# lppllppl920/SAGE-SLAM

Hardware: AMD Instinct MI355X
Metric: M residuals/sec (+ LM iters/sec), 64-keyframe feature-metric BA @128x160 (higher is better)
Workload: dtype f32; 1 GPU; 64-keyframe window, 128x160x16 feature pyramids (L=4), 32-dim depth code, dense sampling N=16128, 186 links = 372 photometric + 372 geometric directed edges; parallelism=single GPU, collective=none, accepted_steps=988

## Files before the change

### include/sage_ba.h

```cpp
#ifndef SAGE_BA_H_
#define SAGE_BA_H_

#include <stddef.h>
#include <stdint.h>

#ifdef __cplusplus
extern "C" {
#endif

#define SAGE_MAX_LEVELS 8
#define SAGE_POSE_FLOATS 12

#define SAGE_OK 0
#define SAGE_E_INVALID (-1)
#define SAGE_E_UNSUPPORTED (-2)
#define SAGE_E_NOT_PSD (-3)
#define SAGE_E_STATE (-4)
#define SAGE_E_NO_OVERLAP (-5)

typedef struct SageCamera
{
  float fx, fy, cx, cy, w, h;
} SageCamera;

// ... 9 lines not shown

const char *sage_version(void);
const char *sage_error_string(int code);

typedef struct SageWorkspace SageWorkspace;
int sage_workspace_create(void *hip_stream, SageWorkspace **out);
void sage_workspace_destroy(SageWorkspace *ws);


int sage_photometric_jac_error_calculate(
    SageWorkspace *ws, float *AtA_dev, float *Atb_dev, float *error_host, float *num_inliers_host,
    const float *R10_dev, const float *t10_dev, const float *R0_dev, const float *t0_dev,
    const float *R1_dev, const float *t1_dev,
    const float *bias0_dev, const float *basis0_dev, const float *code0_dev, const float *mask1_dev,
    const int64_t *loc1d_dev, const float *homo_dev,
    const float *feat0_dev, const float *feat1_dev, const float *grad1_dev,
    float scale0, const SagePyramid *pyr, float eps, const float *weights_host,
    int N, int FS, int CS);

int sage_photometric_error_calculate(
    SageWorkspace *ws, float *error_host, float *num_inliers_host,
    const float *R10_dev, const float *t10_dev,
    const float *bias0_dev, const float *basis0_dev, const float *code0_dev, const float *mask1_dev,
    const int64_t *loc1d_dev, const float *homo_dev,
    const float *feat0_dev, const float *feat1_dev,
    float scale0, const SagePyramid *pyr, float eps, const float *weights_host,
    int N, int FS, int CS);

int sage_tracker_photo_jac_error_calculate(
    SageWorkspace *ws, int dof, float *AtA_dev, float *Atb_dev, float *error_host, float *num_inliers_host,
    const float *R_dev, const float *t_dev, const float *mask1_dev,
    const float *dpts0_dev, const float *homo_dev, const float *feat0s_dev,
    const float *feat1_dev, const float *grad1_dev,
    const SagePyramid *pyr, float scale0, float eps, const float *weights_dev, int N, int FS);

int sage_tracker_photo_error_calculate(
    SageWorkspace *ws, float *error_host, float *num_inliers_host,
    const float *R_dev, const float *t_dev, const float *mask1_dev,
    const float *dpts0_dev, const float *homo_dev, const float *feat0s_dev, const float *feat1_dev,
    const SagePyramid *pyr, float eps, const float *weights_dev, int N, int FS);

int sage_geometric_jac_error_calculate(
    SageWorkspace *ws, float *AtA_dev, float *Atb_dev, float *error_host, float *num_inliers_host,
    const float *R10_dev, const float *t10_dev, const float *R0_dev, const float *t0_dev,
    const float *R1_dev, const float *t1_dev,
    const float *bias0_dev, const float *basis0_dev, const float *code0_dev,
    const float *dpt1_dev, const float *dpt_grad1_dev, const float *basis1_dev, const float *mask1_dev,
    const int32_t *loc1d_dev, const float *homo_dev,
    float scale0, float scale1, const SageCamera *cam, float eps, float loss_param, float weight,
    int N, int CS);

int sage_geometric_error_calculate(
    SageWorkspace *ws, float *error_host, float *num_inliers_host,
    const float *R10_dev, const float *t10_dev,
    const float *bias0_dev, const float *basis0_dev, const float *code0_dev,
    const float *dpt1_dev, const float *mask1_dev, const int32_t *loc1d_dev, const float *homo_dev,
    float scale0, const SageCamera *cam, float eps, float loss_param, float weight, int N, int CS);

int sage_depth_and_grad(SageWorkspace *ws, float *dpt_dev, float *dpt_grad_dev,
                        const float *bias_dev, const float *basis_dev, const float *code_dev,
                        float scale, int H, int W, int CS);
int sage_gaussian_pyramid_with_grad(SageWorkspace *ws, float *pyr_dev, float *grad_dev,
                                    const float *feat_dev, const float *mask_dev,
                                    const SagePyramid *pyr, int FS);

int sage_bind_thread_to_device(int device);
int sage_solver_helper_cpus(int *cpus, int n);
int sage_solver_placement_moves(void);
int sage_placement_monitor(int enable);
void sage_shutdown(void);
int sage_host_threads_running(void);

void sage_se3_exp(const float *omega, const float *v, float *R, float *t);
void sage_pose_retract(const float *pose, const float *delta6, float *out);
int sage_nearest_psd(const double *M, int n, double *out);
int sage_nearest_psd_reference(const double *M, int n, double *out);
int sage_factor_block_count(int type, int CS);
int sage_factor_hessian_blocks(int type, int CS, const float *AtA_host, const float *Atb_host, int psd_mode,
                               double *G_out, double *g_out, int32_t *dims_out, int32_t *nkeys_out);
int sage_damped_solve_qr_f32(const float *A, const float *b, int n, float damp, float *x);

int sage_block_solve(const double *packed_host, int K, int nlinks, const int32_t *links, int B, double damp,
                     const double *diag_add, const double *g_add, double *delta);
long long sage_solve_lookahead_count(void);

typedef struct SageLmConfig
{
  int max_num_iters;
  float min_grad_thresh;
  float min_param_inc_thresh;
  float init_damp;
  float min_damp, max_damp;
  float damp_dec_factor;
  float damp_inc_factor;
  float jac_update_err_inc_threshold;
  int max_inner_evals;
  float no_overlap_error;
  int linearize_at_candidate;
} SageLmConfig;
void sage_lm_config_default(SageLmConfig *cfg);

typedef int (*SageTrackLinearizeFn)(void *ctx, const float *pose12, float scale, float *AtA, float *Atb, float *error);
typedef int (*SageTrackErrorFn)(void *ctx, const float *pose12, float scale, float *error);

typedef struct SageLmTraceEntry
{
  float damp, error, candidate_error;
  int accepted, relinearized;
} SageLmTraceEntry;

int sage_track_lm(const SageLmConfig *cfg, int dof, SageTrackLinearizeFn lin, SageTrackErrorFn err, void *ctx,
                  float *pose12, float *scale, float *final_error, int *iters,
                  SageLmTraceEntry *trace, int trace_cap, int *trace_len);

typedef struct SageTrackProblem
{
  SageWorkspace *ws;
  int32_t use_photo;
  const float *mask1_dev, *dpts0_dev, *homo_dev, *feat0s_dev, *feat1_dev, *grad1_dev;
  const float *weights_dev;
  SagePyramid pyr;
  float eps;
  int32_t N, FS;
  int32_t use_keypoints, NK;
  const float *kp_dpts0_dev;
  const float *kp_homo0_dev;
  const float *kp_matched_2d_dev;
  const float *kp_matched_dpts1_dev;
  const float *kp_matched_homo1_dev;
  float kp_loss_param;
  float kp_weight;
} SageTrackProblem;
int sage_track_frame(const SageLmConfig *cfg, int dof, const SageTrackProblem *prob,
                     float *pose12, float *scale, float *final_error, int *iters,
                     SageLmTraceEntry *trace, int trace_cap, int *trace_len);

typedef struct SageWindow SageWindow;

typedef struct SageKeyframeView
{
  const float *feat_pyr;
  const float *grad_pyr;
  const float *bias;
  const float *basis;
  const int64_t *loc1d;
  const float *homo;
  int32_t N;
} SageKeyframeView;

typedef struct SageWindowConfig
{
  SagePyramid pyr;
  int32_t FS, CS;
  const float *mask_dev;
  float photo_weights[SAGE_MAX_LEVELS];
  float geo_weight, geo_loss_param, eps;
  float code_prior_weight;
  float scale_prior_weight;
  float pose_prior_weight;
  int32_t use_photo, use_geo;
} SageWindowConfig;

int sage_window_create(const SageWindowConfig *cfg, void *hip_stream, SageWindow **out);
void sage_window_destroy(SageWindow *w);
int sage_window_add_keyframe(SageWindow *w, const SageKeyframeView *view, const float *pose12,
                             const float *code, float scale);
int sage_window_add_link(SageWindow *w, int kf_a, int kf_b);
int sage_window_set_link_geo_loss(SageWindow *w, int link, float loss_param);
int sage_window_add_keypoint_link(SageWindow *w, int kf_a, int kf_b);
enum { SAGE_HOLD_POSE = 1, SAGE_HOLD_CODE = 2, SAGE_HOLD_SCALE = 4 };
int sage_window_hold(SageWindow *w, int kf, int what);
int sage_window_set_shard(SageWindow *w, int rank, int world);
int sage_window_finalize(SageWindow *w);

int sage_window_num_keyframes(const SageWindow *w);
int sage_window_num_links(const SageWindow *w);
int sage_window_block_size(const SageWindow *w);
int sage_window_solver_block_size(const SageWindow *w);
size_t sage_window_packed_count(const SageWindow *w);
double *sage_window_packed_dev(SageWindow *w);
double sage_window_residuals_per_linearize(const SageWindow *w);
double sage_window_bytes_per_linearize(const SageWindow *w);

int sage_window_linearize(SageWindow *w);
int sage_window_error(SageWindow *w, int which);
int sage_window_tune_runs(SageWindow *w, int *tpb_out, int *tpb_rule_out, float *ms_rule_out, float *ms_best_out);
int sage_window_set_runs(SageWindow *w, int tpb);
double *sage_window_error_dev(SageWindow *w);
int sage_window_solve(SageWindow *w, double damp, double *step_norm);
int sage_window_total_error(SageWindow *w, int from_linearize, double *err);
int sage_window_accept(SageWindow *w);
int sage_window_reset(SageWindow *w);
int sage_window_get_keyframe(const SageWindow *w, int kf, float *pose12, float *code, float *scale);
int sage_window_set_keyframe(SageWindow *w, int kf, const float *pose12, const float *code, float scale);
int sage_window_get_delta(const SageWindow *w, double *delta);
int sage_window_get_edge(const SageWindow *w, int type, int e, float *AtA, float *Atb, float *err, float *n_in);

enum { SAGE_KP_REPROJECTION = 0, SAGE_KP_MATCH_GEOMETRY = 1, SAGE_KP_LOOP_MG = 2 };
typedef struct SageKeypointTerm
{
  int32_t kind;
  int32_t edge;
  int32_t N;
  const int32_t *loc1d_0;
  const float *homo0;
  const float *matched_2d;
  const int32_t *matched_loc1d_1;
  const float *matched_homo1;
  float loss_param, weight;
  int32_t loss;
  const float *unscaled_dpts0, *matched_unscaled_dpts1;
} SageKeypointTerm;
int sage_window_add_keypoint_term(SageWindow *w, const SageKeypointTerm *t);
int sage_window_num_keypoint_terms(const SageWindow *w);
int sage_window_get_keypoint_term(const SageWindow *w, int term, float *AtA, float *Atb, float *err, float *n_in);

int sage_window_prepass(SageWindow *w, const float *pose12, const float *codes, const float *scales, int jacobians,
                        int *recomputed);
int sage_window_factor(const SageWindow *w, int type, int e, int psd_mode, double *G_out, double *g_out, double *f_out,
                       int *dims_out, int *nkeys_out);
int sage_window_factor_error(const SageWindow *w, int type, int e, double *err_out);
int sage_window_prepare_factors(SageWindow *w, int psd_mode, int n_threads);
int sage_factor_psd(int type, int CS, const float *AtA, int psd_mode, double *C_out);
int sage_factor_cut_blocks(int type, int CS, const double *C, const float *Atb, double *G_out, double *g_out,
                           int32_t *dims_out, int32_t *nkeys_out);

int sage_window_set_profiling(SageWindow *w, int on);
int sage_window_get_kernel_time(SageWindow *w, int which, double *total_ms, int *launches);
int sage_window_get_phase_time(SageWindow *w, double *ms4, int *iterations);

int sage_reprojection_jac_error_calculate(SageWorkspace *ws, float *AtA_dev, float *Atb_dev, float *error_host,
                                          float *num_inliers_host, const float *R10, const float *t10, const float *R0,
                                          const float *t0, const float *R1, const float *t1, const float *bias0,
                                          const float *basis0, const float *code0, const int32_t *loc1d,
                                          const float *homo, const float *matched_2d, float scale0,
                                          const SageCamera *cam, float eps, float loss_param, float weight, int N, int CS);
int sage_reprojection_error_calculate(SageWorkspace *ws, float *error_host, float *num_inliers_host, const float *R10,
                                      const float *t10, const float *bias0, const float *basis0, const float *code0,
                                      const int32_t *loc1d, const float *homo, const float *matched_2d, float scale0,
                                      const SageCamera *cam, float eps, float loss_param, float weight, int N, int CS);
int sage_tracker_reproj_jac_error_calculate(SageWorkspace *ws, float *AtA_dev, float *Atb_dev, float *error_host,
                                            float *num_inliers_host, const float *R, const float *t,
                                            const float *sampled_dpts0, const float *homo, const float *matched_2d,
                                            const SageCamera *cam, float eps, float loss_param, float weight, int N);
int sage_tracker_reproj_error_calculate(SageWorkspace *ws, float *error_host, float *num_inliers_host, const float *R,
                                        const float *t, const float *sampled_dpts0, const float *homo,
                                        const float *matched_2d, const SageCamera *cam, float eps, float loss_param,
                                        float weight, int N);

enum { SAGE_LOSS_FAIR = 0, SAGE_LOSS_L2 = 1, SAGE_LOSS_HUBER = 2, SAGE_LOSS_UNBIASED = 3 };
int sage_match_geometry_jac_error_calculate(SageWorkspace *ws, float *AtA_dev, float *Atb_dev, float *error_host,
                                            const float *R10, const float *t10, const float *R0, const float *t0,
                                            const float *R1, const float *t1, const float *bias0, const float *bias1,
                                            const float *basis0, const float *basis1, const float *code0,
                                            const float *code1, const float *homo0, const float *matched_homo1,
                                            const int32_t *loc1d_0, const int32_t *matched_loc1d_1, float scale0,
                                            float scale1, float loss_param, float weight, int loss, int N, int CS);
int sage_match_geometry_error_calculate(SageWorkspace *ws, float *error_host, const float *R10, const float *t10,
                                        const float *bias0, const float *bias1, const float *basis0, const float *basis1,
                                        const float *code0, const float *code1, const float *homo0,
                                        const float *matched_homo1, const int32_t *loc1d_0,
                                        const int32_t *matched_loc1d_1, float scale0, float scale1, float loss_param,
                                        float weight, int loss, int N, int CS);
int sage_loop_mg_jac_error_calculate(SageWorkspace *ws, float *AtA_dev, float *Atb_dev, float *error_host,
                                     const float *R10, const float *t10, const float *R0, const float *t0,
                                     const float *R1, const float *t1, const float *unscaled_dpts0,
                                     const float *matched_unscaled_dpts1, const float *homo0, const float *matched_homo1,
                                     float scale0, float scale1, float loss_param, float weight, int N);
// ... 68 lines not shown
```

### sage_slam_amd/capi.py

```python
from __future__ import annotations

import ctypes as C
import os
from typing import List, Optional, Sequence

import numpy as np

HERE = os.path.dirname(os.path.abspath(__file__))
LIB_PATH = os.path.join(HERE, "libsage_ba.so")
SAGE_MAX_LEVELS = 8


class SageError(RuntimeError):
    def __init__(self, code: int, where: str):
        self.code = code
        msg = lib().sage_error_string(code).decode() if _lib is not None else "?"
        super().__init__(f"{where}: {msg} (code {code})")


class SageCamera(C.Structure):
    _fields_ = [(n, C.c_float) for n in ("fx", "fy", "cx", "cy", "w", "h")]


class SagePyramid(C.Structure):
    _fields_ = [("levels", C.c_int32), ("P", C.c_int32), ("level_offsets", C.c_int32 * SAGE_MAX_LEVELS),
                ("cam", SageCamera * SAGE_MAX_LEVELS)]


class SageLmConfig(C.Structure):
    _fields_ = [("max_num_iters", C.c_int), ("min_grad_thresh", C.c_float), ("min_param_inc_thresh", C.c_float),
                ("init_damp", C.c_float), ("min_damp", C.c_float), ("max_damp", C.c_float),
                ("damp_dec_factor", C.c_float), ("damp_inc_factor", C.c_float),
                ("jac_update_err_inc_threshold", C.c_float), ("max_inner_evals", C.c_int),
                ("no_overlap_error", C.c_float), ("linearize_at_candidate", C.c_int)]


class SageLmTraceEntry(C.Structure):
    _fields_ = [("damp", C.c_float), ("error", C.c_float), ("candidate_error", C.c_float),
                ("accepted", C.c_int), ("relinearized", C.c_int)]


class SageTrackProblem(C.Structure):
    _fields_ = [("ws", C.c_void_p), ("use_photo", C.c_int32), ("mask1_dev", C.c_void_p), ("dpts0_dev", C.c_void_p),
                ("homo_dev", C.c_void_p), ("feat0s_dev", C.c_void_p), ("feat1_dev", C.c_void_p),
                ("grad1_dev", C.c_void_p), ("weights_dev", C.c_void_p), ("pyr", SagePyramid), ("eps", C.c_float),
                ("N", C.c_int32), ("FS", C.c_int32), ("use_keypoints", C.c_int32), ("NK", C.c_int32),
                ("kp_dpts0_dev", C.c_void_p), ("kp_homo0_dev", C.c_void_p), ("kp_matched_2d_dev", C.c_void_p),
                ("kp_matched_dpts1_dev", C.c_void_p), ("kp_matched_homo1_dev", C.c_void_p),
                ("kp_loss_param", C.c_float), ("kp_weight", C.c_float)]


class SageKeyframeView(C.Structure):
    _fields_ = [("feat_pyr", C.c_void_p), ("grad_pyr", C.c_void_p), ("bias", C.c_void_p), ("basis", C.c_void_p),
                ("loc1d", C.c_void_p), ("homo", C.c_void_p), ("N", C.c_int32)]


class SageWindowConfig(C.Structure):
    _fields_ = [("pyr", SagePyramid), ("FS", C.c_int32), ("CS", C.c_int32), ("mask_dev", C.c_void_p),
                ("photo_weights", C.c_float * SAGE_MAX_LEVELS), ("geo_weight", C.c_float),
                ("geo_loss_param", C.c_float), ("eps", C.c_float), ("code_prior_weight", C.c_float),
                ("scale_prior_weight", C.c_float), ("pose_prior_weight", C.c_float),
                ("use_photo", C.c_int32), ("use_geo", C.c_int32)]


SAGE_KP_REPROJECTION, SAGE_KP_MATCH_GEOMETRY, SAGE_KP_LOOP_MG = 0, 1, 2
SAGE_HOLD_POSE, SAGE_HOLD_CODE, SAGE_HOLD_SCALE = 1, 2, 4
KP_KINDS = {"reprojection": SAGE_KP_REPROJECTION, "match_geometry": SAGE_KP_MATCH_GEOMETRY, "loop_mg": SAGE_KP_LOOP_MG}


class SageKeypointTerm(C.Structure):
    _fields_ = [("kind", C.c_int32), ("edge", C.c_int32), ("N", C.c_int32), ("loc1d_0", C.c_void_p), ("homo0", C.c_void_p),
                ("matched_2d", C.c_void_p), ("matched_loc1d_1", C.c_void_p), ("matched_homo1", C.c_void_p),
                ("loss_param", C.c_float), ("weight", C.c_float), ("loss", C.c_int32), ("unscaled_dpts0", C.c_void_p),
                ("matched_unscaled_dpts1", C.c_void_p)]


def kp_term_dim(kind, CS: int) -> int:
    kind = KP_KINDS.get(kind, kind)
    return {SAGE_KP_REPROJECTION: 13 + CS, SAGE_KP_MATCH_GEOMETRY: 14 + 2 * CS, SAGE_KP_LOOP_MG: 14}[kind]


ALLREDUCE_FN = C.CFUNCTYPE(C.c_int, C.c_void_p, C.c_size_t, C.c_void_p)


class SageLmState(C.Structure):
    _fields_ = [("damp", C.c_double), ("error", C.c_double), ("candidate_error", C.c_double),
                ("accepted", C.c_int), ("iters", C.c_int)]


TRACK_LIN_FN = C.CFUNCTYPE(C.c_int, C.c_void_p, C.POINTER(C.c_float), C.c_float, C.POINTER(C.c_float),
                           C.POINTER(C.c_float), C.POINTER(C.c_float))
TRACK_ERR_FN = C.CFUNCTYPE(C.c_int, C.c_void_p, C.POINTER(C.c_float), C.c_float, C.POINTER(C.c_float))

_lib = None

SYMBOLS = [
    "sage_camera_pyramid", "sage_version", "sage_error_string", "sage_workspace_create", "sage_workspace_destroy",
    "sage_photometric_jac_error_calculate", "sage_photometric_error_calculate",
    "sage_tracker_photo_jac_error_calculate", "sage_tracker_photo_error_calculate",
    "sage_geometric_jac_error_calculate", "sage_geometric_error_calculate", "sage_depth_and_grad",
    "sage_gaussian_pyramid_with_grad", "sage_se3_exp", "sage_pose_retract", "sage_nearest_psd", "sage_nearest_psd_reference", "sage_factor_block_count", "sage_factor_hessian_blocks",
    "sage_damped_solve_qr_f32", "sage_block_solve", "sage_solve_lookahead_count", "sage_lm_config_default", "sage_track_lm", "sage_track_frame",
    "sage_window_create", "sage_window_destroy", "sage_window_add_keyframe", "sage_window_add_link", "sage_window_add_keypoint_link", "sage_window_hold", "sage_window_set_link_geo_loss",
    "sage_window_set_shard", "sage_window_finalize", "sage_window_num_keyframes", "sage_window_num_links",
    "sage_window_block_size", "sage_window_solver_block_size", "sage_window_packed_count", "sage_window_packed_dev",
    "sage_window_residuals_per_linearize", "sage_window_bytes_per_linearize", "sage_window_linearize",
    "sage_window_error", "sage_window_tune_runs", "sage_window_set_runs", "sage_window_error_dev", "sage_window_solve", "sage_window_total_error",
    "sage_window_accept", "sage_window_reset", "sage_window_get_keyframe", "sage_window_set_keyframe", "sage_window_get_delta",
    "sage_window_get_edge", "sage_window_add_keypoint_term", "sage_window_num_keypoint_terms", "sage_window_get_keypoint_term", "sage_window_prepass", "sage_window_factor", "sage_window_factor_error", "sage_window_prepare_factors", "sage_factor_psd", "sage_factor_cut_blocks", "sage_window_set_profiling", "sage_window_get_kernel_time", "sage_window_get_phase_time", "sage_window_lm_step", "sage_window_lm_run", "sage_window_lm_run_timed", "sage_window_sync_variables", "sage_window_set_allreduce", "sage_shard_plan_create", "sage_shard_plan_create_domains", "sage_block_solve_domains", "sage_shard_plan_destroy", "sage_shard_sep_count", "sage_shard_num_separators", "sage_shard_num_interior", "sage_shard_keyframe_owner", "sage_shard_keyframe_is_local", "sage_shard_eliminate", "sage_shard_solve", "sage_rccl_unique_id", "sage_rccl_comm_create", "sage_rccl_comm_destroy", "sage_rccl_comm_info", "sage_window_use_rccl", "sage_window_emulate_peers", "sage_sort_locations", "sage_bind_thread_to_device", "sage_solver_helper_cpus", "sage_solver_placement_moves", "sage_placement_monitor", "sage_shutdown", "sage_host_threads_running",
    "sage_valid_locations", "sage_shuffle_indices", "sage_sample_locations",
    "sage_reprojection_jac_error_calculate", "sage_reprojection_error_calculate",
    "sage_tracker_reproj_jac_error_calculate", "sage_tracker_reproj_error_calculate",
    "sage_match_geometry_jac_error_calculate", "sage_match_geometry_error_calculate",
    "sage_loop_mg_jac_error_calculate", "sage_loop_mg_error_calculate",
    "sage_tracker_match_geom_jac_error_calculate", "sage_tracker_match_geom_error_calculate", "sage_cycle_match",
]


def lib():
    global _lib
    if _lib is None:
        LIB_PATH = os.environ.get("SAGE_BA_LIB", globals()["LIB_PATH"])
        if not os.path.exists(LIB_PATH):
            raise ImportError(f"{LIB_PATH} is missing: run `python -m sage_slam_amd.build` "
                              "(the HIP engine has no fallback path)")
        import torch
        L = C.CDLL(LIB_PATH)
        L.sage_version.restype = C.c_char_p
        L.sage_error_string.restype = C.c_char_p
        L.sage_window_packed_count.restype = C.c_size_t
        L.sage_shutdown.restype = None
        L.sage_window_packed_dev.restype = C.c_void_p
        L.sage_window_error_dev.restype = C.c_void_p
        L.sage_window_residuals_per_linearize.restype = C.c_double
        L.sage_window_bytes_per_linearize.restype = C.c_double
        for name in ("sage_window_packed_count", "sage_window_packed_dev", "sage_window_error_dev",
                     "sage_window_residuals_per_linearize", "sage_window_bytes_per_linearize",
                     "sage_window_num_keyframes", "sage_window_num_links", "sage_window_block_size",
                     "sage_window_solver_block_size"):
            getattr(L, name).argtypes = [C.c_void_p]
        _lib = L
    return _lib


def _chk(code: int, where: str):
    if code != 0:
        raise SageError(code, where)


def _f32(a) -> np.ndarray:
    return np.ascontiguousarray(a, dtype=np.float32)


def _fp(a: np.ndarray):
    return a.ctypes.data_as(C.POINTER(C.c_float))


def dptr(t) -> C.c_void_p:
    if t is None:
        return C.c_void_p(0)
    assert t.is_contiguous(), "device buffers handed to the C ABI must be contiguous"
    return C.c_void_p(t.data_ptr())


def make_pyramid(cam, levels: int) -> SagePyramid:
    base = SageCamera(*[float(v) for v in (cam.fx, cam.fy, cam.cx, cam.cy, cam.w, cam.h)])
    out = SagePyramid()
    _chk(lib().sage_camera_pyramid(C.byref(base), levels, C.byref(out)), "sage_camera_pyramid")
    return out


def se3_exp(omega, v):
    omega = _f32(omega); v = _f32(v)
    R = np.zeros(9, np.float32); t = np.zeros(3, np.float32)
    lib().sage_se3_exp(_fp(omega), _fp(v), _fp(R), _fp(t))
    return R.reshape(3, 3), t


def pose_retract(pose12, delta6):
    pose12 = _f32(pose12).reshape(12); delta6 = _f32(delta6)
    out = np.zeros(12, np.float32)
    lib().sage_pose_retract(_fp(pose12), _fp(delta6), _fp(out))
    return out


def nearest_psd(M):
    M = np.ascontiguousarray(M, dtype=np.float64)
    out = np.zeros_like(M)
    _chk(lib().sage_nearest_psd(M.ctypes.data_as(C.POINTER(C.c_double)), M.shape[0],
                                out.ctypes.data_as(C.POINTER(C.c_double))), "sage_nearest_psd")
    return out


def nearest_psd_reference(M):
    M = np.ascontiguousarray(M, np.float64)
    out = np.zeros_like(M)
    _chk(lib().sage_nearest_psd_reference(M.ctypes.data_as(C.POINTER(C.c_double)), M.shape[0],
                                          out.ctypes.data_as(C.POINTER(C.c_double))), "sage_nearest_psd_reference")
    return out


def factor_hessian_blocks(type_: int, CS: int, AtA, Atb, psd_mode: int = 1):
    L = lib()
    A = _f32(AtA); b = _f32(Atb)
    n = L.sage_factor_block_count(type_, CS)
    if n < 0:
        raise SageError(n, "sage_factor_block_count")
    G = np.zeros(n, np.float64); g = np.zeros(b.size, np.float64)
    dims = (C.c_int32 * 6)(); nk = C.c_int32()
    _chk(L.sage_factor_hessian_blocks(type_, CS, _fp(A), _fp(b), psd_mode, G.ctypes.data_as(C.POINTER(C.c_double)),
                                      g.ctypes.data_as(C.POINTER(C.c_double)), dims, C.byref(nk)),
         "sage_factor_hessian_blocks")
    dims = [int(dims[i]) for i in range(nk.value)]
    blocks, o = {}, 0
    for i in range(nk.value):
        for j in range(i, nk.value):
            blocks[(i, j)] = G[o:o + dims[i] * dims[j]].reshape(dims[i], dims[j]); o += dims[i] * dims[j]
    offs = np.concatenate([[0], np.cumsum(dims)])
    return blocks, [g[offs[i]:offs[i + 1]] for i in range(nk.value)], dims


def damped_solve_qr_f32(A, b, damp):
    A = _f32(A); b = _f32(b)
    x = np.zeros(b.shape[0], np.float32)
    _chk(lib().sage_damped_solve_qr_f32(_fp(A), _fp(b), b.shape[0], C.c_float(damp), _fp(x)), "sage_damped_solve_qr_f32")
# ... 295 lines not shown
                raise SageError(r, "sage_window_add_keypoint_link")
        self.links = [(min(a, b), max(a, b)) for a, b in list(win.links) + kp_links]
        for kf, what in sorted((holds or {}).items()):
            _chk(self.hold(kf, what), "sage_window_hold")
        self.keypoint_terms = list(keypoint_terms or [])
        for t in self.keypoint_terms:
            r = self.add_keypoint_term(t)
            if r < 0:
                raise SageError(r, "sage_window_add_keypoint_term")
        _chk(L.sage_window_set_shard(self.h, rank, world), "sage_window_set_shard")
        _chk(L.sage_window_finalize(self.h), "sage_window_finalize")
        self.K = L.sage_window_num_keyframes(self.h)
        self.B = L.sage_window_block_size(self.h)
        self.Bs = L.sage_window_solver_block_size(self.h)
        self.nlinks = L.sage_window_num_links(self.h)
        self.packed_count = L.sage_window_packed_count(self.h)
        self.residuals_per_linearize = L.sage_window_residuals_per_linearize(self.h)
        self.bytes_per_linearize = L.sage_window_bytes_per_linearize(self.h)

    def add_keypoint_link(self, a, b) -> int:
        return int(lib().sage_window_add_keypoint_link(self.h, int(a), int(b)))

    def hold(self, kf, what) -> int:
        return int(lib().sage_window_hold(self.h, int(kf), int(what)))

    def add_keypoint_term(self, t) -> int:
        import torch
        kind = KP_KINDS.get(t["kind"], t["kind"])
        lmg = kind == SAGE_KP_LOOP_MG
        mg = "loc1" in t and not lmg
        N = int(np.asarray(t["homo0"]).shape[0])
        dev = dict(homo0=_dev(t["homo0"], np.float32))
        kt = SageKeypointTerm()
        kt.kind = int(kind)
        kt.edge, kt.N = int(t["edge"]), N
        kt.homo0 = dev["homo0"].data_ptr()
        if not lmg:
            dev["loc0"] = _dev(t["loc0"], np.int32)
            kt.loc1d_0 = dev["loc0"].data_ptr()
        if lmg:
            for key, field in (("homo1", "matched_homo1"), ("u0", "unscaled_dpts0"), ("u1", "matched_unscaled_dpts1")):
                if t.get(key) is not None:
                    dev[key] = _dev(t[key], np.float32)
                    setattr(kt, field, dev[key].data_ptr())
        elif mg:
            dev["loc1"] = _dev(t["loc1"], np.int32); dev["homo1"] = _dev(t["homo1"], np.float32)
            kt.matched_loc1d_1, kt.matched_homo1 = dev["loc1"].data_ptr(), dev["homo1"].data_ptr()
            loss = t.get("loss", "fair")
            kt.loss = MG_LOSS[loss] if isinstance(loss, str) else int(loss)
        else:
            dev["m2d"] = _dev(t["matched_2d"], np.float32)
            kt.matched_2d = dev["m2d"].data_ptr()
        kt.loss_param, kt.weight = float(t["loss_param"]), float(t["weight"])
        torch.cuda.synchronize()
        return int(lib().sage_window_add_keypoint_term(self.h, C.byref(kt)))

    def num_keypoint_terms(self) -> int:
        return int(lib().sage_window_num_keypoint_terms(self.h))

    def get_keypoint_term(self, i, check=True):
        kind = self.keypoint_terms[i]["kind"] if 0 <= i < len(self.keypoint_terms) else "reprojection"
        D = kp_term_dim(kind, self.win.CS)
        A = np.zeros((D, D), np.float32); b = np.zeros(D, np.float32)
        err = C.c_float(); nin = C.c_float()
        rc = lib().sage_window_get_keypoint_term(self.h, int(i), _fp(A), _fp(b), C.byref(err), C.byref(nin))
        out = dict(AtA=A, Atb=b, error=err.value, num_inliers=nin.value)
        if not check:
            return rc, out
        _chk(rc, "sage_window_get_keypoint_term")
        return out

    def packed_tensor(self):
        return _tensor_from_ptr(lib().sage_window_packed_dev(self.h), self.packed_count)

    def error_tensor(self):
        return _tensor_from_ptr(lib().sage_window_error_dev(self.h), 4)

    def linearize(self):
        _chk(lib().sage_window_linearize(self.h), "sage_window_linearize")

    def error(self, which=1):
        _chk(lib().sage_window_error(self.h, which), "sage_window_error")

    def tune_runs(self):
        tpb, rule = C.c_int(0), C.c_int(0)
        ms_rule, ms_best = C.c_float(0), C.c_float(0)
        _chk(lib().sage_window_tune_runs(self.h, C.byref(tpb), C.byref(rule), C.byref(ms_rule), C.byref(ms_best)),
             "sage_window_tune_runs")
        return dict(tpb=tpb.value, tpb_rule=rule.value, ms_rule=ms_rule.value, ms_best=ms_best.value)

    def set_runs(self, tpb):
        _chk(lib().sage_window_set_runs(self.h, int(tpb)), "sage_window_set_runs")

    def solve(self, damp, want_norm=True):
        if not want_norm:
            _chk(lib().sage_window_solve(self.h, C.c_double(damp), None), "sage_window_solve")
            return None
        sn = C.c_double()
        _chk(lib().sage_window_solve(self.h, C.c_double(damp), C.byref(sn)), "sage_window_solve")
        return sn.value

    def total_error(self, from_linearize: bool):
        e = C.c_double()
        _chk(lib().sage_window_total_error(self.h, int(from_linearize), C.byref(e)), "sage_window_total_error")
        return e.value

    def accept(self):
        _chk(lib().sage_window_accept(self.h), "sage_window_accept")

    def reset(self):
        _chk(lib().sage_window_reset(self.h), "sage_window_reset")

    def set_allreduce(self, dist_module, group=None):
        tensors = {}
        for t in (self.packed_tensor(), self.error_tensor()):
            tensors[(t.data_ptr(), t.numel())] = t

        def hook(ptr, n, _user):
            try:
                t = tensors.get((ptr, n))
                if t is None:
                    t = tensors[(ptr, n)] = _tensor_from_ptr(ptr, n)
                dist_module.all_reduce(t, group=group)
                return 0
            except Exception:
                import traceback
                traceback.print_exc()
                return 1

        self._allreduce_cb = ALLREDUCE_FN(hook)
        _chk(lib().sage_window_set_allreduce(self.h, self._allreduce_cb, None), "sage_window_set_allreduce")

    def sync_variables(self):
        _chk(lib().sage_window_sync_variables(self.h), "sage_window_sync_variables")

    def use_rccl(self, comm):
        _chk(lib().sage_window_use_rccl(self.h, C.c_void_p(comm)), "sage_window_use_rccl")

    def emulate_peers(self, rest):
        if rest is None:
            self._emu_rest = None
            _chk(lib().sage_window_emulate_peers(self.h, None, 0), "sage_window_emulate_peers")
            return
        assert rest.is_cuda and rest.dim() == 2 and rest.shape[1] == self.packed_count and rest.is_contiguous()
        self._emu_rest = rest
        _chk(lib().sage_window_emulate_peers(self.h, C.c_void_p(rest.data_ptr()), int(rest.shape[0])),
             "sage_window_emulate_peers")

    def lm_step(self, state: SageLmState, cfg: SageLmConfig):
        _chk(lib().sage_window_lm_step(self.h, C.byref(state), C.byref(cfg)), "sage_window_lm_step")
        return state

    def lm_run(self, state: SageLmState, cfg: SageLmConfig, n: int):
        tr = np.zeros((n, 4), np.float64)
        done = C.c_int()
        _chk(lib().sage_window_lm_run(self.h, C.byref(state), C.byref(cfg), n, tr.ctypes.data_as(C.POINTER(C.c_double)),
                                      C.byref(done)), "sage_window_lm_run")
        return tr[:done.value]

    def lm_run_timed(self, state: SageLmState, cfg: SageLmConfig, n: int):
        tr = np.zeros((n, 4), np.float64); sec = np.zeros(n, np.float64)
        done = C.c_int()
        _chk(lib().sage_window_lm_run_timed(self.h, C.byref(state), C.byref(cfg), n, tr.ctypes.data_as(C.POINTER(C.c_double)),
                                            C.byref(done), sec.ctypes.data_as(C.POINTER(C.c_double))), "sage_window_lm_run_timed")
        return tr[:done.value], sec[:done.value]

# ... 435 lines not shown
```

### sage_slam_amd/csrc/block_solver.cpp

```cpp
#include <algorithm>
#include <atomic>
#include <chrono>
#include <cmath>
#include <cstdio>
#include <cstdlib>
#include <cstring>
#include <sched.h>
#include <thread>
#include <vector>

#include "block_solver.h"
#include "damped_system.h"
#include "host_math.h"
#include "sage_ba.h"

namespace sage
{
namespace
{
typedef double v8d __attribute__((vector_size(64), aligned(8)));

#define SAGE_LOADU(dst, p) __builtin_memcpy(&(dst), (p), sizeof(v8d))
#define SAGE_STOREU(p, v) __builtin_memcpy((p), &(v), sizeof(v8d))

struct RowPrefetch
{
  const char *p, *end;
  const char *p2 = nullptr, *end2 = nullptr, *p3 = nullptr, *end3 = nullptr;
  inline __attribute__((always_inline)) void step()
  {
    if (p < end)
    {
      __builtin_prefetch(p, 0, 3);
      __builtin_prefetch(p + 64, 0, 3);
      p += 128;
    }
    else if (p2 < end2)
    {
      __builtin_prefetch(p2, 0, 3);
      __builtin_prefetch(p2 + 64, 0, 3);
      p2 += 128;
    }
    else if (p3 < end3)
    {
      __builtin_prefetch(p3, 0, 3);
      __builtin_prefetch(p3 + 64, 0, 3);
      p3 += 128;
    }
  }
};

template <int NV, int V0>
static inline __attribute__((always_inline)) void tn_sub_rows4(double *CT, const double *Tj, const double *Ti, int c0,
                                                               RowPrefetch &pf)
{
  constexpr int BP = NV * 8;
  v8d acc[4][NV];
  for (int u = 0; u < 4; ++u)
    for (int v = V0; v < NV; ++v)
      acc[u][v] = v8d{0, 0, 0, 0, 0, 0, 0, 0};
  for (int t = 0; t < BP; ++t)
  {
    const double *ti = Ti + t * BP, *tj = Tj + t * BP + c0;
    pf.step();
    v8d b[NV];
    for (int v = V0; v < NV; ++v)
      SAGE_LOADU(b[v], ti + 8 * v);
    for (int u = 0; u < 4; ++u)
    {
      const double sc = tj[u];
      const v8d s = {sc, sc, sc, sc, sc, sc, sc, sc};
      for (int v = V0; v < NV; ++v)
        acc[u][v] += s * b[v];
    }
  }
  for (int u = 0; u < 4; ++u)
    for (int v = V0; v < NV; ++v)
    {
      v8d c;
      SAGE_LOADU(c, CT + (c0 + u) * BP + 8 * v);
      c -= acc[u][v];
      SAGE_STOREU(CT + (c0 + u) * BP + 8 * v, c);
    }
}

template <int NV>
static inline __attribute__((always_inline)) void tn_sub(double *CT, const double *Tj, const double *Ti, bool upper_only,
                                                         RowPrefetch &pf)
{
  constexpr int BP = NV * 8;
  for (int c0 = 0; c0 < BP; c0 += 4)
  {
    const int v0 = upper_only ? c0 / 8 : 0;
    switch (v0)
// ... 1500 lines not shown
}

BlockEnvelope envelope_of(const BlockPlan &plan, int Bp)
{
  BlockEnvelope env;
  env.K = (int)plan.row_first.size(); env.Bp = Bp; env.n1 = plan.n1; env.n2 = plan.n2;
  env.row_first = plan.row_first.data(); env.row_off = plan.row_off.data();
  env.a_first = plan.a_first.data(); env.a_cnt = plan.a_cnt.data(); env.a_off = plan.a_off.data();
  env.col_ptr = plan.col_ptr.data(); env.col_rows = plan.col_rows.data();
  return env;
}
}

extern "C" long long sage_solve_lookahead_count(void) { return sage::g_lookahead_count.load(); }

extern "C" int sage_block_solve(const double *packed, int K, int nlinks, const int32_t *links, int B, double damp,
                                const double *diag_add, const double *g_add, double *delta)
{
  if (!packed || K < 1 || B < 1 || nlinks < 0 || (nlinks > 0 && !links) || !delta)
    return SAGE_E_INVALID;
  const int Bp = sage::padded_block(B);
  if (Bp == 0)
    return SAGE_E_UNSUPPORTED;
  const int BB = B * B, BBp = Bp * Bp;
  const double *diag = packed;
  const double *lnk = diag + (size_t)K * BB;
  const double *g = lnk + (size_t)nlinks * BB;
  std::vector<std::pair<int, int>> lk(nlinks);
  for (int l = 0; l < nlinks; ++l)
    lk[l] = {links[2 * l], links[2 * l + 1]};
  sage::BlockPlan bp;
  int rcp = sage::plan_blocks(K, lk, !sage::env_flag("SAGE_SOLVE_NO_SPLIT"), bp);
  if (rcp == SAGE_E_UNSUPPORTED)
  {
    std::sort(lk.begin(), lk.end());
    lk.erase(std::unique(lk.begin(), lk.end()), lk.end());
    rcp = sage::plan_blocks(K, lk, !sage::env_flag("SAGE_SOLVE_NO_SPLIT"), bp);
  }
  if (rcp != SAGE_OK)
    return rcp;
  const int nblk = bp.nblk;
  std::vector<double> T((size_t)nblk * BBp, 0.0), X((size_t)K * BBp), y((size_t)K * Bp, 0.0);
  for (int q = 0; q < K; ++q)
  {
    const int k = bp.perm[q];
    double *D = T.data() + (size_t)bp.index(q, q) * BBp;
    for (int r = 0; r < Bp; ++r)
      for (int c = 0; c < Bp; ++c)
        D[sage::stored_slot(r, c, Bp)] =
            (r < B && c < B) ? sage::damped_diag_elem(diag + (size_t)k * BB, B, r, c, diag_add ? diag_add[k * B + r] : 0.0, damp)
                             : sage::damped_pad_elem(r, c, damp);
    for (int r = 0; r < B; ++r)
      y[(size_t)q * Bp + r] = sage::damped_rhs_elem(g[(size_t)k * B + r], g_add ? g_add[k * B + r] : 0.0);
  }
  for (int l = 0; l < nlinks; ++l)
  {
    const int a = links[2 * l], b = links[2 * l + 1];
    const int qi = std::max(bp.pos[a], bp.pos[b]), qj = std::min(bp.pos[a], bp.pos[b]);
    double *D = T.data() + (size_t)bp.index(qi, qj) * BBp;
    const bool row_is_a = bp.perm[qi] == a;
    for (int r = 0; r < B; ++r)
      for (int c = 0; c < B; ++c)
        D[sage::stored_slot(r, c, Bp)] += lnk[(size_t)l * BB + sage::link_elem(row_is_a, r, c, B)];
  }
  static const bool dbg = sage::env_flag("SAGE_DEBUG_TIMING");
  const auto t0 = std::chrono::steady_clock::now();
  sage::BlockEnvelope env = sage::envelope_of(bp, Bp);
  int rcf;
  {
    sage::SolveLease lease;
    if (bp.n1 > 0)
      env.no_lookahead = sage::block_chol_arm(sage::block_plan_has_arrow_rows(env), sage::block_plan_long_arrow_chains(env));
    rcf = sage::block_chol_solve_tr(env, T.data(), X.data(), y.data());
  }
  if (dbg)
    fprintf(stderr, "[sage block_solve] fixed-block Cholesky + substitution %.3f ms\n",
            std::chrono::duration<double, std::milli>(std::chrono::steady_clock::now() - t0).count());
  if (rcf != 0)
    return SAGE_E_NOT_PSD;
  for (int k = 0; k < K; ++k)
    std::memcpy(delta + (size_t)k * B, y.data() + (size_t)bp.pos[k] * Bp, sizeof(double) * B);
  return SAGE_OK;
}
```

### sage_slam_amd/csrc/photo_kernels.hip

```cpp
#include <type_traits>

#include "sage_device.h"
#include "sage_internal.h"
#include "finalize_bodies.h"

namespace sage
{

struct PhotoParams
{
  PhotoEdge single;
  const PhotoEdge *table;
  const WorkItem *work;
  float *partials;
  SagePyramid pyr;
  float w[SAGE_MAX_LEVELS];
  float eps;
  int tiles_per_block;
  int width, height;
  float rx[SAGE_MAX_LEVELS], ry[SAGE_MAX_LEVELS];
  int lw[SAGE_MAX_LEVELS], lh[SAGE_MAX_LEVELS];
  float geo_loss_param;
  int n_work;
  const int32_t *rec_first;
// ... 1301 lines not shown
                                 const LaunchCommon &lc, const SagePyramid &pyr, const float *wh, float eps,
                                 const EdgeOut &out)
{
  float wsum;
  PhotoParams p = make_params(single, table, lc, pyr, wh, eps, &wsum);
  if (lc.stage != 2)
  {
    if (lc.ev_start)
      (void)hipEventRecord(lc.ev_start, s);
    if (lc.packed && lc.merge_geo_weight > 0.f)
      hipLaunchKernelGGL((photo_kernel<CS, FS, true, 2>), dim3(lc.n_work), dim3(kBlock), 0, s, p);
    else if (lc.packed)
      hipLaunchKernelGGL((photo_kernel<CS, FS, true, 1>), dim3(lc.n_work), dim3(kBlock), 0, s, p);
    else
      hipLaunchKernelGGL((photo_kernel<CS, FS, true, 0>), dim3(lc.n_work), dim3(kBlock), 0, s, p);
    if (lc.ev_stop)
      (void)hipEventRecord(lc.ev_stop, s);
  }
  if (lc.stage == 1)
    return hipGetLastError();
  PhotoFinalizeParams f{};
  if (single)
    f.single = *single;
  f.table = table;
  f.edge_first = lc.edge_first;
  f.edge_tiles = lc.edge_tiles;
  f.partials = lc.partials;
  f.AtA = out.AtA;
  f.Atb = out.Atb;
  f.stats = out.stats;
  f.wide = out.wide;
  f.wsum = wsum;
  f.edge_base = lc.stage == 2 ? lc.edge_base : 0;
  const int n_fin = lc.stage == 2 ? lc.edge_count : lc.n_edges;
  if (n_fin > 0)
    hipLaunchKernelGGL((photo_finalize_kernel<CS>), dim3(n_fin), dim3(lc.fin_block), 0, s, f);
  return hipGetLastError();
}

template <int CS, int FS>
static hipError_t photo_err_impl(hipStream_t s, const PhotoEdge *single, const PhotoEdge *table,
                                 const LaunchCommon &lc, const SagePyramid &pyr, const float *wh, float eps,
                                 float *stats)
{
  float wsum;
  PhotoParams p = make_params(single, table, lc, pyr, wh, eps, &wsum);
  if (lc.ev_start)
    (void)hipEventRecord(lc.ev_start, s);
  if (lc.packed)
    hipLaunchKernelGGL((photo_kernel<CS, FS, false, 1>), dim3(lc.n_work), dim3(kBlock), 0, s, p);
  else
    hipLaunchKernelGGL((photo_kernel<CS, FS, false, 0>), dim3(lc.n_work), dim3(kBlock), 0, s, p);
  if (lc.ev_stop)
    (void)hipEventRecord(lc.ev_stop, s);
  if (lc.stage == 1)
    return hipGetLastError();
  return launch_stats_finalize(s, lc, stats, 10.0f * wsum, 1.0f);
}

template <class F>
static hipError_t dispatch_cs_fs(int CS, int FS, F &&f)
{
  using std::integral_constant;
  if (CS == 32 && FS == 16)
    return f(integral_constant<int, 32>{}, integral_constant<int, 16>{});
  if (CS == 16 && FS == 16)
    return f(integral_constant<int, 16>{}, integral_constant<int, 16>{});
  if (CS == 32 && FS == 32)
    return f(integral_constant<int, 32>{}, integral_constant<int, 32>{});
  if (CS == 16 && FS == 32)
    return f(integral_constant<int, 16>{}, integral_constant<int, 32>{});
  return hipErrorInvalidValue;
}

hipError_t launch_photo_linearize(hipStream_t s, int CS, int FS, const PhotoEdge *single, const PhotoEdge *table,
                                  const LaunchCommon &lc, const SagePyramid &pyr, const float *weights_host,
                                  float eps, const EdgeOut &out)
{
  return dispatch_cs_fs(CS, FS, [&](auto cs, auto fs) {
    return photo_lin_impl<decltype(cs)::value, decltype(fs)::value>(s, single, table, lc, pyr, weights_host, eps, out);
  });
}

hipError_t launch_photo_error(hipStream_t s, int CS, int FS, const PhotoEdge *single, const PhotoEdge *table,
                              const LaunchCommon &lc, const SagePyramid &pyr, const float *weights_host,
                              float eps, float *stats)
{
  return dispatch_cs_fs(CS, FS, [&](auto cs, auto fs) {
    return photo_err_impl<decltype(cs)::value, decltype(fs)::value>(s, single, table, lc, pyr, weights_host, eps, stats);
  });
}

}

#ifdef SAGE_PHOTO_TRACE
extern "C" int sage_debug_photo_trace(void *dst, size_t bytes)
{
  const size_t all = sizeof(unsigned long long) * (size_t)sage::kTraceMaxWg * 4 * sage::kTraceSubs * sage::kTraceMarks;
  if (bytes > all)
    bytes = all;
  return (int)hipMemcpyFromSymbol(dst, HIP_SYMBOL(sage::g_photo_trace), bytes, 0, hipMemcpyDeviceToHost);
}
extern "C" int sage_debug_photo_trace_clear()
{
  void *p = nullptr;
  if (hipGetSymbolAddress(&p, HIP_SYMBOL(sage::g_photo_trace)) != hipSuccess)
    return 1;
  return (int)hipMemset(p, 0, sizeof(unsigned long long) * (size_t)sage::kTraceMaxWg * 4 * sage::kTraceSubs * sage::kTraceMarks);
}
#endif
```

### sage_slam_amd/csrc/runtime_internal.h

```cpp
#pragma once

#include <hip/hip_runtime.h>

#include <algorithm>
#include <atomic>
#include <cctype>
#include <sched.h>
#include <chrono>
#include <cmath>
#include <cstdlib>
#include <cstdio>
#include <cstring>
#include <thread>
#include <vector>

#include <dlfcn.h>
#if __has_include(<rccl/rccl.h>)
#include <rccl/rccl.h>
#else
extern "C"
{
  typedef struct ncclComm *ncclComm_t;
  typedef struct
  {
// ... 190 lines not shown
  int stride, err_off, cnt_off;
};

}

#include "window_state.h"

struct SageWindow
{
  SageWindowConfig cfg;
  hipStream_t stream = nullptr;
  bool finalized = false;
  int rank = 0, world = 1;
  int K = 0, B = 0, VS = 0;
  std::vector<SageKeyframeView> views;
  HostVars hv;
  std::vector<float> link_geo_loss;
  std::vector<std::pair<int, int>> links;
  std::vector<char> link_dense;
  std::vector<uint8_t> hold;
  sage::plan::SolverRows rows;
  std::vector<int> local_links;
  std::vector<int> owned_edges;
  std::vector<int> local_edges;
  int n_edges = 0;
  DevBuf vars[2];
  DevBuf sorted_loc, sorted_homo;
  std::vector<std::pair<const int64_t *, const float *>> user_samples;
  std::vector<int> user_n;
  DevBuf dpt, dgrad, depth_items[2];
  int n_depth = 0;
  int dpt_set = -1;
  bool dgrad_valid = false;
  DevBuf geo_px;
  bool merge_ok = false;
  DevBuf pk;
  DevBuf f0s;
  DenseSide dense[2];
  PhotoRecordPlan photo_rec;
  std::vector<int> Nedge;
  int tpb_heur = 1;
  DevBuf adj_start, adj, link_edges, packed, errbuf;
  TotalsMirror mirror;
  WindowDist dist;
  std::vector<double> host_packed;
  std::vector<double> delta;
  sage::DeviceSolver *solver = nullptr;
  bool cand_pending = false;
  double residuals_per_lin = 0, bytes_per_lin = 0;
  bool have_lin = false;
  uint64_t vars_epoch = 1, lin_epoch = 0;
  bool spec_err_valid = false;
  double spec_error = 0.0;
  DevBuf packed_save;
  struct KeypointTermHost
  {
    int32_t kind, edge, N, loss;
    float loss_param, weight;
    std::vector<int32_t> loc0, loc1;
    std::vector<float> homo0, second;
    std::vector<float> dpts0, dpts1;
  };
  std::vector<KeypointTermHost> kp_added;
  std::vector<int> kp_local;
  int n_kr = 0, n_km = 0, n_kl = 0;
  int n_terms() const { return n_kr + n_km + n_kl; }
  unsigned kp_kinds() const { return (n_kr > 0 ? 1u : 0u) | (n_km > 0 ? 2u : 0u) | (n_kl > 0 ? 4u : 0u); }
  bool kp_lin = false;
  DevBuf kp_pool, kp_table, kp_link_start, kp_link;
  DevBuf AtA_kr, Atb_kr, AtA_km, Atb_km, AtA_kl, Atb_kl;
  DevBuf stats_k;
  struct FactorCache
  {
    bool lin = false, err = false;
    std::vector<float> pose, code, scale;
    struct Side
    {
      std::vector<float> A, b, s;
      std::vector<double> C;
    } side[2];
    int psd_mode = -1;
  } fc;
  WindowProfiler prof;

  bool kernels_mirror_totals() const { return world == 1 && !dist.allreduce && mirror.h; }
};


template <class T>
static int upload(DevBuf &b, const std::vector<T> &v, hipStream_t s)
{
  int rc = b.reserve(std::max<size_t>(v.size(), 1) * sizeof(T));
  if (rc)
    return rc;
  if (!v.empty())
    SAGE_HIP(hipMemcpyAsync(b.p, v.data(), v.size() * sizeof(T), hipMemcpyHostToDevice, s));
  return 0;
}
int window_upload_vars(SageWindow *w, int set);
int window_local_edge(const SageWindow *w, int global_edge);
bool window_owns_edge(const SageWindow *w, int global_edge);
bool window_has_holds(const SageWindow *w);
std::vector<int32_t> window_link_pairs(const SageWindow *w);
int window_linearize_set(SageWindow *w, int set, double *dst = nullptr, bool local_blocks = false, bool merge = false);
int window_error_pass(SageWindow *w, int which, bool speculate_gradients);
int window_collective(SageWindow *w, double *buf, size_t n);
int window_allreduce(SageWindow *w, double *buf, size_t n, int iterate);
int window_allreduce_into(SageWindow *w, const double *send, double *recv, size_t n, int iterate);
int window_mirror_totals(SageWindow *w, bool with_err, const double *system = nullptr);
bool window_wait_error_totals(SageWindow *w);
bool window_wait_reduced_totals(SageWindow *w);
int window_wait_mirror(SageWindow *w, bool *not_psd);
double mirrored_error(const SageWindow *w, int at, int set);
int window_total_error(SageWindow *w, int from_linearize, double *err, bool stream_idle);
int window_copy_floats(SageWindow *w, const float *src, float *dst, int n);
void window_add_to_double(SageWindow *w, double *p, double v);
double window_prior_error(const SageWindow *w, int set, bool owned_only = false);
int window_sync_candidate(SageWindow *w, bool stream_idle = false);
int window_schur_solve(SageWindow *w, double damp, double *lin_error);
void prof_attach(SageWindow *w, int which, LaunchCommon &lc);
void window_phase_mark(SageWindow *w, int which);
```

### sage_slam_amd/csrc/sage_internal.h

```cpp
#pragma once

#include <hip/hip_runtime.h>
#include <stdint.h>

#include <cmath>
#include <utility>
#include <vector>

#include "sage_ba.h"

static inline bool pyramid_is_dyadic(const SagePyramid &pyr)
{
  for (int l = 0; l < pyr.levels && l < SAGE_MAX_LEVELS; ++l)
  {
    int e;
    const float rx = pyr.cam[l].fx / pyr.cam[0].fx, ry = pyr.cam[l].fy / pyr.cam[0].fy;
    if (!(rx > 0.f) || !(ry > 0.f) || std::frexp(rx, &e) != 0.5f || std::frexp(ry, &e) != 0.5f)
      return false;
  }
  return true;
}


namespace sage
{

constexpr int kBlock = 256;
constexpr int kFinalizeBlock = 1024;
constexpr int kWaves = kBlock / 64;
constexpr int kTile = 256;

struct PhotoEdge
{
  const float *feat0;
  const float *feat1;
  const float *grad1;
  const float *feat0_pk, *feat1_pk;
  const float *f0s;
  const float *dpt0;
  const float *dpt1_geo;
  float geo_loss;
  const float *geo_px;
  const float *bias0;
  const float *basis0;
  const float *mask1;
  const float *homo;
  const void *loc;
  const float *R0, *t0;
  const float *R1, *t1;
  const float *R10, *t10;
  const float *code0;
  const float *scale0;
  float scale0_val;
  int32_t N;
  int32_t loc_is_i64;
};

struct GeoEdge
{
  const float *dpt0;
  const float *bias0;
  const float *basis0;
  const float *dpt1;
  const float *dgrad1;
  const float *basis1;
  const float *mask1;
  const float *homo;
  const void *loc;
  const float *R0, *t0, *R1, *t1, *R10, *t10;
  const float *code0;
  const float *scale0, *scale1;
  float scale0_val, scale1_val;
  int32_t N;
  int32_t loc_is_i64;
  float loss_param;
  float *px_out;
};

struct TrackEdge
{
  const float *feat0s;
  const float *feat1;
  const float *grad1;
  const float *mask1;
  const float *homo;
  const float *dpts0;
  const float *R, *t;
  const float *weights;
  float scale0;
  int32_t N;
};

struct WorkItem
{
  int32_t edge;
  int32_t tile;
};

constexpr int kPhotoScalars = 40;
constexpr int kGeoScalars = 48;
__host__ __device__ constexpr int photo_tiles(int CS) { return CS == 32 ? 5 : 2; }
__host__ __device__ constexpr int photo_cc_tiles(int CS) { return CS == 32 ? 3 : 1; }
__host__ __device__ constexpr int photo_partial_double_offset(int CS) { return kPhotoScalars + photo_tiles(CS) * 256; }
__host__ __device__ constexpr int photo_partial_doubles(int CS) { return kPhotoScalars + (photo_tiles(CS) - photo_cc_tiles(CS)) * 256; }
__host__ __device__ constexpr int photo_partial_floats(int CS) { return photo_partial_double_offset(CS) + 2 * photo_partial_doubles(CS); }
__host__ __device__ constexpr int geo_n16(int CS) { return 2 * CS / 16; }
__host__ __device__ constexpr int geo_tiles(int CS) { return geo_n16(CS) * (geo_n16(CS) + 1) / 2 + geo_n16(CS); }
__host__ __device__ constexpr int geo_partial_floats(int CS) { return kGeoScalars + geo_tiles(CS) * 256; }
constexpr int kTrackScalars = 40;

struct LaunchCommon
{
  const WorkItem *work;
  const int32_t *edge_first;
  const int32_t *edge_tiles;
  int32_t n_work;
  int32_t n_edges;
  float *partials;
  int32_t tiles_per_block;
  hipEvent_t ev_start = nullptr, ev_stop = nullptr;
  bool packed = false;
  int32_t stage = 0, edge_base = 0, edge_count = 0;
  int32_t fin_block = kFinalizeBlock;
  float fused_geo_loss_param = 0.f;
  int32_t flush = 0;
  float merge_geo_weight = 0.f;
  const float *merge_photo_partials = nullptr;
  const int32_t *merge_photo_rec_first = nullptr, *merge_photo_rec_count = nullptr;
};

struct EdgeOut
{
  float *AtA;
  float *Atb;
  float *stats;
  double *wide = nullptr;
};

hipError_t launch_photo_linearize(hipStream_t s, int CS, int FS, const PhotoEdge *single, const PhotoEdge *table,
                                  const LaunchCommon &lc, const SagePyramid &pyr, const float *weights_host,
                                  float eps, const EdgeOut &out);
hipError_t launch_photo_error(hipStream_t s, int CS, int FS, const PhotoEdge *single, const PhotoEdge *table,
                              const LaunchCommon &lc, const SagePyramid &pyr, const float *weights_host,
                              float eps, float *stats );
hipError_t launch_geo_linearize(hipStream_t s, int CS, const GeoEdge *single, const GeoEdge *table,
                                const LaunchCommon &lc, const SageCamera &cam, float eps, float loss_param,
                                float weight, const EdgeOut &out);
hipError_t launch_geo_error(hipStream_t s, int CS, const GeoEdge *single, const GeoEdge *table,
                            const LaunchCommon &lc, const SageCamera &cam, float eps, float loss_param,
                            float weight, float *stats);
hipError_t launch_track_linearize(hipStream_t s, int dof, int FS, const TrackEdge &edge, const LaunchCommon &lc,
                                  const SagePyramid &pyr, float eps, const EdgeOut &out);
hipError_t launch_track_error(hipStream_t s, int FS, const TrackEdge &edge, const LaunchCommon &lc,
                              const SagePyramid &pyr, float eps, float *stats);
hipError_t launch_depth_and_grad(hipStream_t s, int CS, float *dpt, float *grad, const float *bias,
                                 const float *basis, const float *code, const float *scale_dev, float scale,
                                 int H, int W);
struct DepthItem
{
  const float *bias, *basis, *code, *scale;
  float *dpt, *grad;
};
hipError_t launch_presample_source(hipStream_t s, float *f0s, const float *feat_pk, const float *homo, int N, int FS,
                                   const SagePyramid &pyr);
struct RepackScale
{
  int on;
  float s[SAGE_MAX_LEVELS];
};
hipError_t launch_repack_groups(hipStream_t s, float *dst, const float *src, int C, int P, int axis = 0,
                                const SagePyramid *pyr = nullptr, const float *level_scale = nullptr);
struct SortItem
{
  const long long *loc;
  const float *homo;
  long long *loc_out;
  float *homo_out;
  int n;
};
hipError_t launch_sort_locations(hipStream_t s, const SortItem *items_dev, int K, int max_n, int HW, int *mark_dev,
                                 int *status_dev, int W = 0, int tile_w = 0, int tile_h = 0, const int *pad_flags_dev = nullptr,
                                 int *tiles_out_dev = nullptr, bool keep_marks = false);
hipError_t launch_depth_batch(hipStream_t s, int CS, const DepthItem *items_dev, int K, int H, int W, bool with_depth,
                              bool with_grad);
hipError_t launch_stats_finalize(hipStream_t s, const LaunchCommon &lc, float *stats, float fallback, float scale);
size_t reproj_scratch_floats(int N, int D);
hipError_t launch_reproj(hipStream_t s, int CS, bool tracker, bool jac, const float *R10, const float *t10, const float *R0,
                         const float *t0, const float *R1, const float *t1, const float *bias0, const float *basis0,
                         const float *code0, const int32_t *loc, const float *dpts0, const float *homo,
                         const float *matched, float scale0, const SageCamera &cam, float eps, float loss_param,
                         float weight, int N, float *scratch, float *AtA, float *Atb, float *stats);
hipError_t launch_cycle_match(hipStream_t s, const float *desc0, const float *desc1, const long long *kp_loc0, int K,
                              int C, int H, int W, float cyc_thresh, long long *raw_matched1, long long *cyc_matched0,
                              int32_t *inlier, int *n_inliers_dev);
size_t mg_scratch_floats(int N, int D);
hipError_t launch_match_geom(hipStream_t s, int mode, int loss, int CS, bool jac, const float *R10, const float *t10,
                             const float *R0, const float *t0, const float *R1, const float *t1, const float *bias0,
                             const float *bias1, const float *basis0, const float *basis1, const float *code0,
                             const float *code1, const float *dpts0, const float *dpts1, const float *homo0,
                             const float *homo1, const int32_t *loc0, const int32_t *loc1, float scale0, float scale1,
                             float loss_param, float weight, int N, float *scratch, float *AtA, float *Atb, float *stats);
hipError_t launch_valid_locations(hipStream_t s, const float *mask, const SageCamera &cam, long long *loc1d, float *homo,
                                  int *n_out_dev);
hipError_t launch_gather_locations(hipStream_t s, const long long *vloc, const float *vhomo, const long long *index_dev,
                                   int n, long long *loc1d, float *homo);
hipError_t launch_depth_samples(hipStream_t s, int CS, float *dpt, const float *bias, const float *basis,
                                const float *code, float scale, const void *loc, int loc_is_i64, int N, int HW);
hipError_t launch_scale_array(hipStream_t s, float *out, const float *in, float mult, int n);
hipError_t launch_gaussian_pyramid_with_grad(hipStream_t s, float *pyr, float *grad, const float *feat,
                                             const float *mask, const SagePyramid &p, int FS, float *scratch_mask);


struct DeviceSolver;
struct SolvePriors;
namespace plan
{
struct SolverRows;
}
int solver_create(DeviceSolver **out, int K, const plan::SolverRows &rows, int VS,
                  const std::vector<std::pair<int, int>> &links, hipStream_t stream);
void solver_destroy(DeviceSolver *S);
int solver_set_holds(DeviceSolver *S, const std::vector<uint8_t> &hold, hipStream_t stream);
int solver_run(DeviceSolver *S, hipStream_t stream, const double *packed_dev, const float *vars0, float *vars1, int CS,
               double damp, const SolvePriors &pri);
const float *solver_host_vars(const DeviceSolver *S);
const double *solver_host_delta(const DeviceSolver *S);
double solver_host_step_norm2(const DeviceSolver *S);
int solver_host_status(const DeviceSolver *S);

}
```

### sage_slam_amd/csrc/solve_kernels.hip

```cpp
#include <algorithm>
#include <atomic>
#include <chrono>
#include <cstdio>
#include <cstring>
#include <memory>
#include <vector>

#include "block_solver.h"
#include "damped_system.h"
#include "host_math.h"
#include "sage_device.h"
#include "sage_internal.h"
#include "window_plan.h"

namespace sage
{

struct SolvePlan
{
  int K, B, Bs, Bp, nblk, nlinks;
  const int32_t *row_first;
  const int32_t *row_off;
  const int32_t *blk_row, *blk_col, *blk_src;
  const int32_t *perm, *pos;
  const int32_t *hold;
  const int32_t *to_block, *to_solver;
};

struct SolveResult
{
  double step_norm2;
  int status;
  unsigned go;
};
static size_t result_vars_offset() { return sizeof(SolveResult); }
static size_t result_delta_offset(int K, int VS) { return (sizeof(SolveResult) + (size_t)K * VS * sizeof(float) + 15) / 16 * 16; }

constexpr int kScatterWorkgroups = 32;

__global__ __launch_bounds__(256) void solve_scatter_kernel(const SolvePlan P, const double *__restrict__ packed,
                                                            const float *__restrict__ vars0, int VS, int CS,
                                                            const SolvePriors pri, double damp,
                                                            double *__restrict__ L, double *__restrict__ y,
                                                            const int32_t *__restrict__ order, unsigned *flags,
                                                            unsigned epoch)
{
  const int tid = threadIdx.x;
  const int B = P.B, Bs = P.Bs, Bp = P.Bp, BB = B * B;
  __shared__ double s_dadd[64], s_gadd[64];
  __shared__ int s_row[64];
  if (tid < Bs)
    s_row[tid] = P.to_block[tid];
  __syncthreads();
  for (int it = blockIdx.x; it < P.nblk; it += gridDim.x)
  {
    const int b = order[it];
    const int i = P.blk_row[b], j = P.blk_col[b], srcf = P.blk_src[b];
    const int src = srcf < 0 ? -1 : (srcf & 0x3fffffff);
    const bool row_is_a = srcf >= 0 && (srcf & 0x40000000);
    if (src < 0 && i != j)
      continue;
    const int kf = P.perm[i];
    const int hold_r = P.hold ? P.hold[kf] : 0, hold_c = P.hold ? P.hold[P.perm[j]] : 0;
    const double *diag = packed + (size_t)kf * BB;
    const double *lnk = packed + (size_t)P.K * BB + (size_t)(src < 0 ? 0 : src) * BB;
    const double *g = packed + (size_t)P.K * BB + (size_t)P.nlinks * BB + (size_t)kf * B;
    double *out = L + (size_t)b * Bp * Bp;
    if (i == j)
    {
      const float *var = vars0 + (size_t)kf * VS;
      if (tid < Bs)
      {
        double da, ga;
        prior_row(pri, kf, s_row[tid], CS, var, var[12], var + 13, da, ga, hold_r);
        s_dadd[tid] = da;
        s_gadd[tid] = ga;
      }
      __syncthreads();
    }
    for (int o = tid; o < Bp * Bp; o += blockDim.x)
    {
      const int c = o / Bp, r = o - c * Bp;
      double v = 0.0;
      const bool in = r < Bs && c < Bs;
      const bool held = in && solver_elem_held(hold_r, hold_c, s_row, r, c, CS);
      if (i == j)
        v = in ? (held ? held_diag_elem(r, c) : solver_diag_elem(diag, B, s_row, r, c, s_dadd[r], damp))
               : damped_pad_elem(r, c, damp);
      else if (in && !held)
        v = lnk[solver_link_elem(row_is_a, s_row, r, c, B)];
      out[o] = v;
    }
    if (i == j)
      for (int r = tid; r < Bp; r += blockDim.x)
        y[(size_t)i * Bp + r] =
            (r < Bs && !(hold_r && row_held(hold_r, s_row[r], CS))) ? damped_rhs_elem(g[s_row[r]], s_gadd[r]) : 0.0;
    __syncthreads();
    if (tid == 0)
    {
      __threadfence_system();
      *reinterpret_cast<volatile unsigned *>(flags + b) = epoch;
    }
  }
}

__global__ __launch_bounds__(1024) void solve_retract_kernel(const double *__restrict__ x, int K, int B, int Bp, int CS,
                                                            int VS, const int32_t *__restrict__ pos,
                                                            const int32_t *__restrict__ hold,
                                                            const int32_t *__restrict__ to_solver,
                                                            const float *__restrict__ vars0,
                                                            float *__restrict__ vars1, float *__restrict__ h_vars,
                                                            double *__restrict__ h_delta, SolveResult *h_res,
                                                            unsigned epoch)
{
  const int tid = threadIdx.x;
  const volatile unsigned *go = &h_res->go;
  __shared__ int s_go;
  if (tid == 0)
  {
    const unsigned long long t0 = wall_clock64();
    unsigned v;
    bool timed_out = false;
    for (;;)
    {
      v = *go;
      const unsigned d = ((v & 0x7fffffffu) - epoch) & 0x7fffffffu;
      if (d == 0u)
        break;
      if (d < 0x40000000u && (v & 0x7fffffffu) != 0u)
      {
        v = 0x80000000u;
        break;
      }
      __builtin_amdgcn_s_sleep(4);
      if (wall_clock64() - t0 > 200000000ull)
      {
        v = 0x80000000u;
// ... 42 lines not shown
      pose_retract(v0, d6, o);
    }
    for (int i = 0; i < 12; ++i)
      h_vars[(size_t)k * VS + i] = o[i];
  }
  __shared__ double s_n[16];
  for (int off = 32; off > 0; off >>= 1)
    nrm += __shfl_down(nrm, off);
  if ((tid & 63) == 0)
    s_n[tid >> 6] = nrm;
  __syncthreads();
  if (tid == 0)
  {
    double tot = 0.0;
    for (int w = 0; w < (int)(blockDim.x >> 6); ++w)
      tot += s_n[w];
    h_res->step_norm2 = tot;
  }
}

struct DeviceSolver
{
  int K = 0, B = 0, Bs = 0, Bp = 0, nblk = 0, nlinks = 0, VS = 0;
  void *d_int = nullptr;
  void *d_hold = nullptr;
  void *h_pinned = nullptr;
  void *h_T = nullptr;
  double *h_y = nullptr;
  unsigned *h_flags = nullptr;
  unsigned epoch = 0, go_epoch = 0;
  SolvePlan plan{};
  const int32_t *d_order = nullptr;
  std::vector<double> h_X;
  BlockPlan host_plan;
  std::vector<uint8_t> h_fill;

  DeviceSolver() = default;
  DeviceSolver(const DeviceSolver &) = delete;
  DeviceSolver &operator=(const DeviceSolver &) = delete;
  ~DeviceSolver()
  {
    if (d_int)
      (void)hipFree(d_int);
    if (d_hold)
      (void)hipFree(d_hold);
    if (h_pinned)
      (void)hipHostFree(h_pinned);
    if (h_T)
      (void)hipHostFree(h_T);
  }
  SolveResult *result() const { return reinterpret_cast<SolveResult *>(h_pinned); }
  float *host_vars() const { return reinterpret_cast<float *>(reinterpret_cast<char *>(h_pinned) + result_vars_offset()); }
  double *host_delta() const { return reinterpret_cast<double *>(reinterpret_cast<char *>(h_pinned) + result_delta_offset(K, VS)); }
};

int solver_create(DeviceSolver **out, int K, const plan::SolverRows &rows, int VS,
                  const std::vector<std::pair<int, int>> &links, hipStream_t stream)
{
  *out = nullptr;
  const int B = rows.B, Bs = rows.Bs;
  const int Bp = sage::padded_block(Bs);
  if (Bp == 0 || K < 1)
    return SAGE_E_UNSUPPORTED;
  BlockPlan bp;
  const int rcp = plan_blocks(K, links, !sage::env_flag("SAGE_SOLVE_NO_SPLIT"), bp);
  if (rcp != SAGE_OK)
    return rcp;
  const int n1 = bp.n1, n2 = bp.n2, nblk = bp.nblk;
  const std::vector<int32_t> &perm = bp.perm, &pos = bp.pos, &row_first = bp.row_first, &row_off = bp.row_off,
                             &a_cnt = bp.a_cnt, &a_off = bp.a_off, &blk_row = bp.blk_row, &blk_col = bp.blk_col,
                             &blk_src = bp.blk_src;
  std::unique_ptr<DeviceSolver> S(new DeviceSolver);
  S->K = K; S->B = B; S->Bs = Bs; S->Bp = Bp; S->nblk = nblk; S->nlinks = (int)links.size(); S->VS = VS;
  std::vector<int32_t> all;
  auto put = [&](const std::vector<int32_t> &v) {
    const size_t off = all.size();
    all.insert(all.end(), v.begin(), v.end());
    while (all.size() % 4)
      all.push_back(0);
    return off;
  };
  const size_t o_rf = put(row_first), o_ro = put(row_off), o_br = put(blk_row), o_bc = put(blk_col),
               o_bs = put(blk_src), o_pm = put(perm), o_ps = put(pos);
  std::vector<int32_t> order;
  auto push_row = [&](int i) {
    for (int q = 0; q < a_cnt[i]; ++q)
      order.push_back(a_off[i] + q);
    for (int q = 0; q <= i - row_first[i]; ++q)
      order.push_back(row_off[i] + q);
  };
  if (n1 > 0)
  {
    for (int t = 0; t < std::max(n1, n2); ++t)
    {
      if (t < n1)
        push_row(t);
      if (t < n2)
        push_row(n1 + t);
    }
    for (int i = n1 + n2; i < K; ++i)
      push_row(i);
  }
  else
    for (int i = 0; i < K; ++i)
      push_row(i);
  const size_t o_ord = put(order);
  const size_t o_tb = put(rows.to_block), o_ts = put(rows.to_solver);
  if (hipMalloc(&S->d_int, all.size() * sizeof(int32_t)) != hipSuccess)
    return (int)hipErrorOutOfMemory;
  if (hipMemcpyAsync(S->d_int, all.data(), all.size() * sizeof(int32_t), hipMemcpyHostToDevice, stream) != hipSuccess)
    return (int)hipErrorUnknown;
  if (hipStreamSynchronize(stream) != hipSuccess)
    return (int)hipErrorUnknown;
  const size_t ty_doubles = (size_t)nblk * Bp * Bp + (size_t)K * Bp;
  if (hipHostMalloc(&S->h_T, ty_doubles * sizeof(double) + (size_t)nblk * sizeof(unsigned), hipHostMallocDefault) !=
      hipSuccess)
    return (int)hipErrorOutOfMemory;
  S->h_y = reinterpret_cast<double *>(S->h_T) + (size_t)nblk * Bp * Bp;
  S->h_flags = reinterpret_cast<unsigned *>(reinterpret_cast<double *>(S->h_T) + ty_doubles);
  std::memset(S->h_flags, 0, (size_t)nblk * sizeof(unsigned));
  S->h_X.assign((size_t)K * Bp * Bp, 0.0);
  const size_t h_bytes = result_delta_offset(K, VS) + (size_t)K * B * sizeof(double);
  if (hipHostMalloc(&S->h_pinned, h_bytes, hipHostMallocDefault) != hipSuccess)
    return (int)hipErrorOutOfMemory;
  std::memset(S->h_pinned, 0, h_bytes);
  const int32_t *base = reinterpret_cast<const int32_t *>(S->d_int);
  SolvePlan &P = S->plan;
  P.K = K; P.B = B; P.Bs = Bs; P.Bp = Bp; P.nblk = nblk; P.nlinks = (int)links.size();
  P.row_first = base + o_rf; P.row_off = base + o_ro;
  P.blk_row = base + o_br; P.blk_col = base + o_bc; P.blk_src = base + o_bs; P.perm = base + o_pm; P.pos = base + o_ps;
  P.to_block = base + o_tb; P.to_solver = base + o_ts;
  S->d_order = base + o_ord;
  S->h_fill.assign((size_t)nblk, 0);
  for (int b = 0; b < nblk; ++b)
    S->h_fill[b] = (blk_src[b] < 0 && blk_row[b] != blk_col[b]) ? 1 : 0;
  S->host_plan = std::move(bp);
  *out = S.release();
  return SAGE_OK;
}

void solver_destroy(DeviceSolver *S) { delete S; }

int solver_set_holds(DeviceSolver *S, const std::vector<uint8_t> &hold, hipStream_t stream)
{
  if ((int)hold.size() != S->K)
    return SAGE_E_INVALID;
  const std::vector<int32_t> masks(hold.begin(), hold.end());
  if (!S->d_hold && hipMalloc(&S->d_hold, masks.size() * sizeof(int32_t)) != hipSuccess)
    return (int)hipErrorOutOfMemory;
  if (hipMemcpyAsync(S->d_hold, masks.data(), masks.size() * sizeof(int32_t), hipMemcpyHostToDevice, stream) != hipSuccess ||
      hipStreamSynchronize(stream) != hipSuccess)
    return (int)hipErrorUnknown;
  S->plan.hold = reinterpret_cast<const int32_t *>(S->d_hold);
  return SAGE_OK;
}

int solver_run(DeviceSolver *S, hipStream_t stream, const double *packed_dev, const float *vars0, float *vars1,
               int CS, double damp, const SolvePriors &pri)
{
  static const bool dbgt = sage::env_flag("SAGE_DEBUG_TIMING");
  hipError_t eh;
  SolveLease lease;
  BlockEnvelope env = envelope_of(S->host_plan, S->Bp);
  if (env.n1 > 0)
    env.no_lookahead = block_chol_arm(block_plan_has_arrow_rows(env), block_plan_long_arrow_chains(env));
  S->epoch += 1;
  if (S->epoch == 0)
    S->epoch = 1;
  hipLaunchKernelGGL(solve_scatter_kernel, dim3(std::min(kScatterWorkgroups, S->nblk)), dim3(256), 0, stream, S->plan,
                     packed_dev, vars0, S->VS, CS, pri, damp, reinterpret_cast<double *>(S->h_T), S->h_y, S->d_order,
                     S->h_flags, S->epoch);
  if ((eh = hipGetLastError()) != hipSuccess)
    return (int)eh;
  volatile unsigned *go = &S->result()->go;
  S->go_epoch = (S->go_epoch + 1) & 0x7fffffffu;
  if (S->go_epoch == 0)
    S->go_epoch = 1;
  hipLaunchKernelGGL(solve_retract_kernel, dim3(1), dim3(1024), 0, stream, S->h_y, S->K, S->B, S->Bp, CS, S->VS,
                     S->plan.pos, S->plan.hold, S->plan.to_solver, vars0, vars1, S->host_vars(), S->host_delta(),
                     S->result(), S->go_epoch);
  if ((eh = hipGetLastError()) != hipSuccess)
    return (int)eh;
  struct GoGuard
  {
    volatile unsigned *go;
    unsigned word;
    ~GoGuard()
    {
      std::atomic_thread_fence(std::memory_order_release);
      *go = word;
    }
  } guard{go, S->go_epoch | 0x80000000u};
  const auto t1 = std::chrono::steady_clock::now();
  env.ready = S->h_flags; env.epoch = S->epoch;
  env.fill = S->h_fill.data();
  const int bad = block_chol_solve_tr(env, reinterpret_cast<double *>(S->h_T), S->h_X.data(), S->h_y);
  const auto t2 = std::chrono::steady_clock::now();
  if (dbgt)
    fprintf(stderr, "[sage hybrid solve] wait for the system + host cholesky %.3f ms\n",
            std::chrono::duration<double, std::milli>(t2 - t1).count());
  if (bad == -2)
    return SAGE_E_STATE;
  if (bad)
    return SAGE_E_NOT_PSD;
  guard.word = S->go_epoch;
  return SAGE_OK;
}

const float *solver_host_vars(const DeviceSolver *S) { return S->host_vars(); }
const double *solver_host_delta(const DeviceSolver *S) { return S->host_delta(); }
double solver_host_step_norm2(const DeviceSolver *S) { return S->result()->step_norm2; }
int solver_host_status(const DeviceSolver *S) { return S->result()->status; }

}
```

### sage_slam_amd/csrc/window.hip

```cpp
#include "runtime_internal.h"

extern "C" int sage_window_num_keyframes(const SageWindow *w) { return w ? w->K : 0; }
extern "C" int sage_window_num_links(const SageWindow *w) { return w ? (int)w->links.size() : 0; }
extern "C" int sage_window_block_size(const SageWindow *w) { return w ? w->B : 0; }
extern "C" int sage_window_solver_block_size(const SageWindow *w) { return w && w->finalized ? w->rows.Bs : 0; }
extern "C" size_t sage_window_packed_count(const SageWindow *w)
{
  if (!w)
    return 0;
  const size_t BB = (size_t)w->B * w->B;
  return (size_t)w->K * BB + w->links.size() * BB + (size_t)w->K * w->B + 4;
}
extern "C" double *sage_window_packed_dev(SageWindow *w) { return w ? w->packed.as<double>() : nullptr; }
extern "C" double *sage_window_error_dev(SageWindow *w) { return w ? w->errbuf.as<double>() : nullptr; }
extern "C" double sage_window_residuals_per_linearize(const SageWindow *w) { return w ? w->residuals_per_lin : 0; }
extern "C" double sage_window_bytes_per_linearize(const SageWindow *w) { return w ? w->bytes_per_lin : 0; }

std::vector<int32_t> window_link_pairs(const SageWindow *w)
{
  std::vector<int32_t> lk;
  for (const auto &l : w->links)
    lk.insert(lk.end(), {l.first, l.second});
  return lk;
}

int window_local_edge(const SageWindow *w, int global_edge)
{
  const auto it = std::lower_bound(w->local_edges.begin(), w->local_edges.end(), global_edge);
  return it != w->local_edges.end() && *it == global_edge ? (int)(it - w->local_edges.begin()) : -1;
}

bool window_owns_edge(const SageWindow *w, int global_edge)
{
  return std::binary_search(w->owned_edges.begin(), w->owned_edges.end(), global_edge);
}

bool window_has_holds(const SageWindow *w)
{
  return std::any_of(w->hold.begin(), w->hold.end(), [](uint8_t h) { return h != 0; });
}

int window_upload_vars(SageWindow *w, int set)
{
  if (w->dpt_set == set)
    w->dpt_set = -1;
  if (set == 0)
    ++w->vars_epoch;
  std::vector<float> buf((size_t)w->K * w->VS, 0.f);
  for (int k = 0; k < w->K; ++k)
    w->hv.pack(set, k, w->cfg.CS, &buf[(size_t)k * w->VS]);
  SAGE_HIP(hipMemcpyAsync(w->vars[set].p, buf.data(), buf.size() * sizeof(float), hipMemcpyHostToDevice, w->stream));
  SAGE_HIP(hipStreamSynchronize(w->stream));
  return SAGE_OK;
}

extern "C" int sage_window_get_keyframe(const SageWindow *w, int kf, float *pose12, float *code, float *scale)
{
  if (!w || kf < 0 || kf >= w->K)
    return SAGE_E_INVALID;
  if (pose12)
    std::memcpy(pose12, &w->hv.pose[0][(size_t)kf * 12], 12 * sizeof(float));
  if (code)
    std::memcpy(code, &w->hv.code[0][(size_t)kf * w->cfg.CS], w->cfg.CS * sizeof(float));
  if (scale)
    *scale = w->hv.scale[0][kf];
  return SAGE_OK;
}

extern "C" int sage_window_set_keyframe(SageWindow *w, int kf, const float *pose12, const float *code, float scale)
{
  if (!w || kf < 0 || kf >= w->K || !pose12 || !code)
    return SAGE_E_INVALID;
  (void)window_sync_candidate(w);
  for (int s = 0; s < 2; ++s)
  {
    std::memcpy(&w->hv.pose[s][(size_t)kf * 12], pose12, 12 * sizeof(float));
    std::memcpy(&w->hv.code[s][(size_t)kf * w->cfg.CS], code, w->cfg.CS * sizeof(float));
    w->hv.scale[s][kf] = scale;
  }
  if (w->finalized)
  {
    int rc;
    if ((rc = window_upload_vars(w, 0)) || (rc = window_upload_vars(w, 1)))
      return rc;
  }
  return SAGE_OK;
}
```

### sage_slam_amd/csrc/window_build.hip

```cpp
#include "runtime_internal.h"
#include "window_plan.h"

static std::atomic<int> g_live_windows{0};

extern "C" int sage_window_create(const SageWindowConfig *cfg, void *hip_stream, SageWindow **out)
{
  if (!cfg || !out || !cfg->mask_dev)
    return SAGE_E_INVALID;
  if (!supported(cfg->CS, cfg->FS) || cfg->pyr.levels < 1 || cfg->pyr.levels > SAGE_MAX_LEVELS)
    return SAGE_E_UNSUPPORTED;
  int ndev = 0;
  SAGE_HIP(hipGetDeviceCount(&ndev));
  if (ndev < 1)
    return (int)hipErrorNoDevice;
  SageWindow *w = new SageWindow();
  w->cfg = *cfg;
  w->stream = reinterpret_cast<hipStream_t>(hip_stream);
  w->B = 7 + cfg->CS;
  w->VS = ((13 + cfg->CS + 3) / 4) * 4;
  *out = w;
  g_live_windows.fetch_add(1, std::memory_order_acq_rel);
  return SAGE_OK;
}

extern "C" void sage_window_destroy(SageWindow *w)
{
  if (!w)
    return;
  struct LastOut
  {
    ~LastOut()
    {
      if (g_live_windows.fetch_sub(1, std::memory_order_acq_rel) == 1)
        sage::host_threads_shutdown();
    }
  } last_out;
  std::free(w->dist.rccl_hook);
  sage_shard_plan_destroy(w->dist.shard);
  solver_destroy(w->solver);
  delete w;
}

extern "C" int sage_window_add_keyframe(SageWindow *w, const SageKeyframeView *v, const float *pose12,
                                        const float *code, float scale)
{
  if (!w || !v || !pose12 || !code || w->finalized)
    return SAGE_E_INVALID;
  if (!v->feat_pyr || !v->grad_pyr || !v->bias || !v->basis || !v->loc1d || !v->homo || v->N < 0)
    return SAGE_E_INVALID;
  w->views.push_back(*v);
  for (int s = 0; s < 2; ++s)
  {
    w->hv.pose[s].insert(w->hv.pose[s].end(), pose12, pose12 + 12);
    w->hv.code[s].insert(w->hv.code[s].end(), code, code + w->cfg.CS);
    w->hv.scale[s].push_back(scale);
  }
  w->hv.pose_init.insert(w->hv.pose_init.end(), pose12, pose12 + 12);
  w->hv.code_added.insert(w->hv.code_added.end(), code, code + w->cfg.CS);
  w->hv.scale_init.push_back(scale);
  return w->K++;
}

extern "C" int sage_window_add_link(SageWindow *w, int a, int b)
{
  if (!w || w->finalized || a == b || a < 0 || b < 0 || a >= w->K || b >= w->K)
    return SAGE_E_INVALID;
  w->links.emplace_back(std::min(a, b), std::max(a, b));
  w->link_geo_loss.push_back(0.f);
  w->link_dense.push_back(1);
  return (int)w->links.size() - 1;
}

extern "C" int sage_window_add_keypoint_link(SageWindow *w, int a, int b)
{
  if (!w)
    return SAGE_E_INVALID;
  if (w->finalized)
    return SAGE_E_STATE;
  if (a == b || a < 0 || b < 0 || a >= w->K || b >= w->K)
    return SAGE_E_INVALID;
  w->links.emplace_back(std::min(a, b), std::max(a, b));
  w->link_geo_loss.push_back(0.f);
  w->link_dense.push_back(0);
// ... 150 lines not shown
    offs[t].dpts1 = h.dpts1.empty() ? 0 : put(h.dpts1.data(), h.dpts1.size());
  }
  int rc;
  if ((rc = upload(w->kp_pool, pool, w->stream)))
    return rc;
  const uint32_t *base = w->kp_pool.as<uint32_t>();
  std::vector<KpTerm> table(nloc);
  std::vector<std::vector<AdjEntry>> per_link(w->links.size());
  for (int t = 0; t < nloc; ++t)
  {
    const SageWindow::KeypointTermHost &h = w->kp_added[order[t]];
    const int l = h.edge / 2, dir = h.edge % 2;
    const int k0 = dir == 0 ? w->links[l].first : w->links[l].second, k1 = dir == 0 ? w->links[l].second : w->links[l].first;
    KpTerm kt{};
    kt.kind = h.kind; kt.loss = h.loss; kt.N = h.N;
    kt.out = t - (h.kind >= 1 ? w->n_kr : 0) - (h.kind >= 2 ? w->n_km : 0);
    kt.stat = t;
    kt.k0 = k0; kt.k1 = k1;
    kt.loss_param = h.loss_param; kt.weight = h.weight;
    if (h.kind != SAGE_KP_LOOP_MG)
      kt.loc0 = reinterpret_cast<const int32_t *>(base + offs[t].loc0);
    kt.homo0 = reinterpret_cast<const float *>(base + offs[t].homo0);
    if (h.kind == 0)
      kt.matched = reinterpret_cast<const float *>(base + offs[t].second);
    else
      kt.homo1 = reinterpret_cast<const float *>(base + offs[t].second);
    if (h.kind == SAGE_KP_MATCH_GEOMETRY)
      kt.loc1 = reinterpret_cast<const int32_t *>(base + offs[t].loc1);
    if (h.kind == SAGE_KP_LOOP_MG)
    {
      kt.dpts0 = reinterpret_cast<const float *>(base + offs[t].dpts0);
      kt.dpts1 = reinterpret_cast<const float *>(base + offs[t].dpts1);
    }
    kt.bias0 = w->views[k0].bias; kt.basis0 = w->views[k0].basis;
    kt.bias1 = w->views[k1].bias; kt.basis1 = w->views[k1].basis;
    table[t] = kt;
    adjv[k0].push_back(AdjEntry{2 + h.kind, kt.out, 0});
    adjv[k1].push_back(AdjEntry{2 + h.kind, kt.out, 1});
    per_link[l].push_back(AdjEntry{2 + h.kind, kt.out, dir});
    link_terms[l] = 1;
    *residuals += (double)kp_kind_rows(h.kind) * h.N;
  }
  std::vector<int32_t> lstart(w->links.size() + 1, 0);
  std::vector<AdjEntry> lkp;
  for (size_t l = 0; l < w->links.size(); ++l)
  {
    lstart[l] = (int32_t)lkp.size();
    lkp.insert(lkp.end(), per_link[l].begin(), per_link[l].end());
  }
  lstart[w->links.size()] = (int32_t)lkp.size();
  const size_t Dp = kp_kind_dim(0, CS), Dg = kp_kind_dim(1, CS), Dl = kp_kind_dim(2, CS);
  if ((rc = upload(w->kp_table, table, w->stream)) || (rc = upload(w->kp_link_start, lstart, w->stream)) ||
      (rc = upload(w->kp_link, lkp, w->stream)) ||
      (rc = w->AtA_kr.reserve(std::max<size_t>(1, w->n_kr) * Dp * Dp * sizeof(float))) ||
      (rc = w->Atb_kr.reserve(std::max<size_t>(1, w->n_kr) * Dp * sizeof(float))) ||
      (rc = w->AtA_km.reserve(std::max<size_t>(1, w->n_km) * Dg * Dg * sizeof(float))) ||
      (rc = w->Atb_km.reserve(std::max<size_t>(1, w->n_km) * Dg * sizeof(float))) ||
      (rc = w->AtA_kl.reserve(std::max<size_t>(1, w->n_kl) * Dl * Dl * sizeof(float))) ||
      (rc = w->Atb_kl.reserve(std::max<size_t>(1, w->n_kl) * Dl * sizeof(float))) ||
      (rc = w->stats_k.reserve((size_t)2 * nloc * 2 * sizeof(float))))
    return rc;
  SAGE_HIP(hipMemsetAsync(w->stats_k.p, 0, (size_t)2 * nloc * 2 * sizeof(float), w->stream));
  SAGE_HIP(hipStreamSynchronize(w->stream));
  return SAGE_OK;
}

static int photo_flush_for_runs(int tpb)
{
  if (const char *e = getenv("SAGE_PHOTO_FLUSH"))
    return std::max(0, atoi(e));
  return plan::record_cadence(tpb);
}

static int upload_work_list(DenseSide &sd, const WorkList &wl, hipStream_t s)
{
  int rc;
  sd.n_work = (int)wl.work.size();
  sd.tpb = wl.tiles_per_block;
  if ((rc = upload(sd.work, wl.work, s)) || (rc = upload(sd.first, wl.edge_first, s)) || (rc = upload(sd.tiles, wl.edge_tiles, s)))
    return rc;
  return SAGE_OK;
}

static int window_plan_photo_runs(SageWindow *w, int tpb, int flush)
{
  WorkList wp;
  wp.build(w->Nedge, tpb, nullptr, flush);
  int rc;
  w->photo_rec.flush = wp.flush;
  w->photo_rec.n = wp.n_records;
  DenseSide &ph = w->dense[kPhoto];
  if ((rc = upload_work_list(ph, wp, w->stream)) || (rc = upload(w->photo_rec.first, wp.rec_first, w->stream)) ||
      (rc = upload(w->photo_rec.count, wp.rec_count, w->stream)))
    return rc;
  SAGE_HIP(hipStreamSynchronize(w->stream));
  return ph.part.reserve(std::max<size_t>(1, std::max(ph.n_work, w->photo_rec.n)) * photo_partial_floats(w->cfg.CS) * sizeof(float));
}

static std::vector<int> edge_tiles(const std::vector<int> &Nedge)
{
  std::vector<int> tiles;
  for (int n : Nedge)
    tiles.push_back((n + kTile - 1) / kTile);
  return tiles;
}

struct FinalizeState
{
  bool domain_solve = false;
  std::vector<char> needed;
  std::vector<size_t> f0s_off;
  std::vector<size_t> px_off;
  std::vector<int> Nedge;
  std::vector<std::vector<AdjEntry>> adjv;
  std::vector<LinkEdges> le;
  std::vector<char> link_terms;
  double residuals = 0, bytes = 0;
};

static int image_pixels(const SageWindow *w) { return (int)w->cfg.pyr.cam[0].h * (int)w->cfg.pyr.cam[0].w; }

static int finalize_variables(SageWindow *w)
{
  const int K = w->K, HW = image_pixels(w);
  int rc;
  for (int s = 0; s < 2; ++s)
  {
    if ((rc = w->vars[s].reserve((size_t)K * w->VS * sizeof(float))))
      return rc;
    if ((rc = window_upload_vars(w, s)))
      return rc;
  }
  if ((rc = w->dpt.reserve((size_t)K * HW * sizeof(float))) || (rc = w->dgrad.reserve((size_t)K * 2 * HW * sizeof(float))))
    return rc;
  return SAGE_OK;
}

static int finalize_ownership(SageWindow *w, FinalizeState &fs)
{
  const int K = w->K, HW = image_pixels(w);
  int rc;
  const bool by_link = sage::env_flag("SAGE_SHARD_BY_LINK") || fs.domain_solve;
  plan::Ownership own = plan::owned_edges((int)w->links.size(), w->rank, w->world, by_link);
  w->owned_edges = std::move(own.edges);
  w->local_links = std::move(own.links);
  w->local_edges = plan::dense_edges(w->owned_edges, w->link_dense);
  fs.needed.assign(K, 0);
  for (int ge : w->local_edges)
    fs.needed[w->links[ge / 2].first] = fs.needed[w->links[ge / 2].second] = 1;
  w->n_depth = 0;
  for (int k = 0; k < K; ++k)
    w->n_depth += fs.needed[k];
  for (int s = 0; s < 2; ++s)
  {
    std::vector<DepthItem> items;
    for (int k = 0; k < K; ++k)
    {
      if (!fs.needed[k])
        continue;
      const float *vp = w->vars[s].as<float>() + (size_t)k * w->VS;
      items.push_back(DepthItem{w->views[k].bias, w->views[k].basis, vp + 13, vp + 12,
                                w->dpt.as<float>() + (size_t)k * HW, w->dgrad.as<float>() + (size_t)k * 2 * HW});
    }
    if ((rc = upload(w->depth_items[s], items, w->stream)))
      return rc;
    SAGE_HIP(hipStreamSynchronize(w->stream));
  }
  return SAGE_OK;
}

static int finalize_pyramids(SageWindow *w)
{
  const SageWindowConfig &c = w->cfg;
  const int FS = c.FS, K = w->K;
  int rc;
  const size_t plane_f = (size_t)FS * c.pyr.P;
  if ((rc = w->pk.reserve((size_t)K * 3 * plane_f * sizeof(float))))
    return rc;
  float lvl_scale[SAGE_MAX_LEVELS] = {};
// ... 246 lines not shown
  const size_t ne = std::max(1, w->n_edges);
  DenseSide &ph = w->dense[kPhoto], &ge = w->dense[kGeo];
  if ((rc = ph.reserve_results(ne, dense_dim(kPhoto, CS), std::max(ph.n_work, w->photo_rec.n), photo_partial_floats(CS))) ||
      (rc = ge.reserve_results(ne, dense_dim(kGeo, CS), ge.n_work, geo_partial_floats(CS))))
    return rc;
  std::vector<int32_t> adj_start(K + 1, 0);
  std::vector<AdjEntry> adj;
  for (int k = 0; k < K; ++k)
  {
    adj_start[k] = (int32_t)adj.size();
    adj.insert(adj.end(), fs.adjv[k].begin(), fs.adjv[k].end());
  }
  adj_start[K] = (int32_t)adj.size();
  if ((rc = upload(w->adj_start, adj_start, w->stream)) || (rc = upload(w->adj, adj, w->stream)) ||
      (rc = upload(w->link_edges, fs.le, w->stream)))
    return rc;
  SAGE_HIP(hipStreamSynchronize(w->stream));
  if ((rc = w->packed.reserve(sage_window_packed_count(w) * sizeof(double))) || (rc = w->errbuf.reserve(4 * sizeof(double))))
    return rc;
  {
    std::vector<int32_t> ids;
    for (int k = 0; k < K; ++k)
      if (!fs.adjv[k].empty())
        ids.push_back(k);
    for (size_t l = 0; l < fs.le.size(); ++l)
      if (fs.le[l].e_ab >= 0 || fs.le[l].e_ba >= 0 || fs.link_terms[l])
        ids.push_back(K + (int32_t)l);
    ids.push_back(K + (int32_t)w->links.size());
    w->dist.n_asm_blocks = (int)ids.size();
    if ((rc = upload(w->dist.asm_blocks, ids, w->stream)))
      return rc;
    SAGE_HIP(hipStreamSynchronize(w->stream));
  }
  SAGE_HIP(hipMemsetAsync(w->packed.p, 0, sage_window_packed_count(w) * sizeof(double), w->stream));
  SAGE_HIP(hipMemsetAsync(w->errbuf.p, 0, 4 * sizeof(double), w->stream));
  if (!w->mirror.h)
  {
    SAGE_HIP(hipHostMalloc(reinterpret_cast<void **>(&w->mirror.h), TotalsMirror::kDoubles * sizeof(double), hipHostMallocDefault));
    std::memset(w->mirror.h, 0, TotalsMirror::kDoubles * sizeof(double));
  }
  w->host_packed.assign(sage_window_packed_count(w), 0.0);
  w->delta.assign((size_t)K * w->B, 0.0);
  return SAGE_OK;
}

static int finalize_solver(SageWindow *w, const FinalizeState &fs)
{
  int rc = solver_create(&w->solver, w->K, w->rows, w->VS, w->links, w->stream);
  if (rc != SAGE_OK && rc != SAGE_E_UNSUPPORTED)
    return rc;
  if (w->solver && window_has_holds(w) && (rc = solver_set_holds(w->solver, w->hold, w->stream)))
    return rc;
  if (!fs.domain_solve)
    return SAGE_OK;
  const std::vector<int32_t> lk = window_link_pairs(w);
  if ((rc = sage_shard_plan_create(w->K, (int)w->links.size(), lk.data(), w->B, w->rank, w->world, &w->dist.shard)))
    return rc;
  const size_t ns = sage_shard_sep_count(w->dist.shard);
  w->dist.h_sep.assign(ns, 0.0);
  if ((rc = w->dist.sepbuf.reserve(ns * sizeof(double))))
    return rc;
  w->host_packed.resize(sage_window_packed_count(w));
  return SAGE_OK;
}

extern "C" int sage_window_finalize(SageWindow *w)
{
  if (!w || w->finalized || w->K < 1)
    return SAGE_E_INVALID;
  FinalizeState fs;
  const char *schur = getenv("SAGE_SHARD_SCHUR");
  fs.domain_solve = plan::uses_domain_solve(w->world, w->K, schur ? atoi(schur) != 0 : -1);
  w->hold.resize(w->K, 0);
  if (fs.domain_solve && window_has_holds(w))
    return SAGE_E_UNSUPPORTED;
  w->rows = plan::solver_rows(w->hold.data(), w->K, w->cfg.CS);
  int rc;
  if ((rc = finalize_variables(w)) || (rc = finalize_ownership(w, fs)) || (rc = finalize_pyramids(w)) ||
      (rc = finalize_samples(w)) || (rc = finalize_source_features(w, fs)) || (rc = finalize_edge_tables(w, fs)) ||
      (rc = window_finalize_keypoints(w, fs.adjv, fs.link_terms, &fs.residuals)))
    return rc;
  w->residuals_per_lin = fs.residuals;
  w->bytes_per_lin = fs.bytes;
  if ((rc = finalize_work_lists(w, fs)) || (rc = finalize_results(w, fs)) || (rc = finalize_solver(w, fs)))
    return rc;
  w->finalized = true;
  if (const char *e = getenv("SAGE_AUTOTUNE"))
    if (atoi(e) != 0)
      return sage_window_tune_runs(w, nullptr, nullptr, nullptr, nullptr);
  return SAGE_OK;
}

extern "C" int sage_window_set_runs(SageWindow *w, int tpb)
{
  if (!w || !w->finalized)
    return SAGE_E_STATE;
  if (tpb < 1 || tpb > 64)
    return SAGE_E_INVALID;
  return window_plan_photo_runs(w, tpb, photo_flush_for_runs(tpb));
}

extern "C" int sage_window_tune_runs(SageWindow *w, int *tpb_out, int *tpb_rule_out, float *ms_rule_out, float *ms_best_out)
{
  if (!w || !w->finalized)
    return SAGE_E_STATE;
  const int rule = w->tpb_heur;
  if (tpb_out)
    *tpb_out = w->dense[kPhoto].tpb;
  if (tpb_rule_out)
    *tpb_rule_out = rule;
  if (ms_rule_out)
    *ms_rule_out = 0.f;
  if (ms_best_out)
    *ms_best_out = 0.f;
  if (getenv("SAGE_PHOTO_TPB") || w->world > 1 || w->dist.allreduce || w->n_edges == 0 || !(w->cfg.use_photo))
    return SAGE_OK;
  const std::vector<int> cand = plan::tune_candidates(rule, plan::typical_edge(edge_tiles(w->Nedge)));
  const bool prof_was = w->prof.profiling;
  const int level_was = w->prof.prof_level;
  int rc = sage_window_set_profiling(w, 1);
  double best_ms = 0.0, rule_ms = 0.0;
  int best = rule;
  auto measure = [&](int t, double &ms) -> int {
    int r = window_plan_photo_runs(w, t, photo_flush_for_runs(t));
    for (int rep = 0; rep < 4 && !r; ++rep)
    {
      if ((r = sage_window_linearize(w)) || (r = sage_window_error(w, 1)))
        break;
      double lin = 0.0, err = 0.0;
      int nl = 0, ne = 0;
      if ((r = sage_window_get_kernel_time(w, 0, &lin, &nl)) || (r = sage_window_get_kernel_time(w, 2, &err, &ne)))
        break;
      const double tt = lin / std::max(1, nl) + err / std::max(1, ne);
      if (rep > 0)
        ms = rep == 1 ? tt : std::min(ms, tt);
    }
    return r;
  };
  for (int i = 0; i < 8 && !rc; ++i)
    if ((rc = sage_window_linearize(w)) || (rc = sage_window_error(w, 1)))
      break;
  (void)sage_window_get_kernel_time(w, 0, nullptr, nullptr);
  (void)sage_window_get_kernel_time(w, 2, nullptr, nullptr);
  if (!rc)
    rc = measure(rule, rule_ms);
  best_ms = rule_ms;
  for (size_t c = 1; c < cand.size() && !rc; ++c)
  {
    double ms = 0.0;
    if ((rc = measure(cand[c], ms)))
      break;
    if (ms < best_ms)
    {
      best_ms = ms;
      best = cand[c];
    }
  }
  if (!rc && best != rule)
  {
    double again = 0.0;
    if (!(rc = measure(rule, again)))
      rule_ms = std::min(rule_ms, again);
  }
  (void)sage_window_get_kernel_time(w, 1, nullptr, nullptr);
  (void)sage_window_get_kernel_time(w, 3, nullptr, nullptr);
  (void)sage_window_set_profiling(w, prof_was ? level_was : 0);
  if (!rc && !(best_ms < 0.96 * rule_ms))
// ... 11 lines not shown
```

### sage_slam_amd/csrc/window_eval.hip

```cpp
#include "runtime_internal.h"
#include "finalize_bodies.h"

namespace sage
{

__device__ __forceinline__ int edge_col(int type, int role, int bi, int CS)
{
  if (bi < 6)
    return role * 6 + bi;
  if (type == 2)
    return bi == 6 + CS ? 12 + role : -1;
  if (type == 0)
  {
    if (role == 1)
      return -1;
    return bi < 6 + CS ? 12 + (bi - 6) : 12 + CS;
  }
  if (bi < 6 + CS)
    return 12 + role * CS + (bi - 6);
  return 12 + 2 * CS + role;
}

__device__ __forceinline__ int adj_col_map(int type) { return type == 4 ? 2 : (type & 1); }
__device__ __forceinline__ const float *kp_AtA(const AssembleParams &p, int lt) { return lt == 0 ? p.AtA_kr : (lt == 1 ? p.AtA_km : p.AtA_kl); }
__device__ __forceinline__ const float *kp_Atb(const AssembleParams &p, int lt) { return lt == 0 ? p.Atb_kr : (lt == 1 ? p.Atb_km : p.Atb_kl); }

template <bool KP>
__global__ __launch_bounds__(1024) void assemble_kernel(const AssembleParams p)
{
  const int B = 7 + p.CS, BB = B * B;
  const int Dp = 13 + p.CS, Dg = 14 + 2 * p.CS;
  const int split = p.split > 1 ? p.split : 1;
  const int part = (int)blockIdx.x % split, bslot = (int)blockIdx.x / split;
  const int blk = p.blocks ? p.blocks[bslot] : bslot;
  const int tstride = (int)blockDim.x * split, tfirst = part * (int)blockDim.x + (int)threadIdx.x;
  double *diag = p.packed;
  double *lnk = diag + (size_t)p.K * BB;
  double *g = lnk + (size_t)p.nlinks * BB;
  double *tail = g + (size_t)p.K * B;
  if (blk < p.K)
  {
    const int k = blk;
    const int a0 = p.adj_start[k], a1 = p.adj_start[k + 1];
    constexpr int S = 2;
    for (int base = 0; base < BB + B; base += S * tstride)
    {
    double acc[S] = {0.0, 0.0};
    int bi[S], bj[S];
    bool isg[S], valid[S];
#pragma unroll
    for (int s = 0; s < S; ++s)
    {
      const int idx = base + tfirst + s * tstride;
      valid[s] = idx < BB + B;
      isg[s] = idx >= BB;
      bi[s] = isg[s] ? idx - BB : idx / B;
      bj[s] = isg[s] ? 0 : idx % B;
    }
#pragma unroll 4
    for (int a = a0; a < a1; ++a)
    {
      const AdjEntry ae = p.adj[a];
      const int lt = KP ? adj_col_map(ae.type) : ae.type;
      const bool kp = KP && ae.type >= 2;
      const int D = lt == 0 ? Dp : (lt == 1 ? Dg : 14);
      const float *A = kp ? kp_AtA(p, lt) : (lt == 0 ? p.AtA_p : p.AtA_g);
      const float *b = kp ? kp_Atb(p, lt) : (lt == 0 ? p.Atb_p : p.Atb_g);
#pragma unroll
      for (int s = 0; s < S; ++s)
      {
        if (!valid[s])
          continue;
        const int ci = edge_col(lt, ae.role, bi[s], p.CS);
        const int cj = isg[s] ? 0 : edge_col(lt, ae.role, bj[s], p.CS);
        if (ci < 0 || cj < 0)
          continue;
        const double *Wd = kp ? nullptr : (lt == 0 ? p.wide_p : p.wide_g);
        if (Wd)
          acc[s] += Wd[(size_t)ae.edge * (D * D + D) + (isg[s] ? (size_t)D * D + ci : (size_t)ci * D + cj)];
        else
          acc[s] += isg[s] ? (double)b[(size_t)ae.edge * D + ci] : (double)A[(size_t)ae.edge * D * D + (size_t)ci * D + cj];
      }
// ... 6 lines not shown
        continue;
      if (isg[s])
        g[(size_t)k * B + bi[s]] = acc[s];
      else
        diag[(size_t)k * BB + idx] = acc[s];
    }
    }
  }
  else if (blk < p.K + p.nlinks)
  {
    const int l = blk - p.K;
    const LinkEdges le = p.links[l];
    for (int idx = tfirst; idx < BB; idx += tstride)
    {
      const int bi = idx / B, bj = idx % B;
      double acc = 0.0;
      {
        for (int type = 0; type < 2; ++type)
        {
          if ((type == 0 && !p.AtA_p) || (type == 1 && !p.AtA_g))
            continue;
          const int D = type == 0 ? Dp : Dg;
          const float *A = type == 0 ? p.AtA_p : p.AtA_g;
          const double *Wd = type == 0 ? p.wide_p : p.wide_g;
          const size_t ws = (size_t)D * D + D;
          int ci = edge_col(type, 0, bi, p.CS), cj = edge_col(type, 1, bj, p.CS);
          if (le.e_ab >= 0 && ci >= 0 && cj >= 0)
            acc += Wd ? Wd[(size_t)le.e_ab * ws + (size_t)ci * D + cj] : (double)A[(size_t)le.e_ab * D * D + (size_t)ci * D + cj];
          ci = edge_col(type, 1, bi, p.CS);
          cj = edge_col(type, 0, bj, p.CS);
          if (le.e_ba >= 0 && ci >= 0 && cj >= 0)
            acc += Wd ? Wd[(size_t)le.e_ba * ws + (size_t)ci * D + cj] : (double)A[(size_t)le.e_ba * D * D + (size_t)ci * D + cj];
        }
      }
      if (KP && p.link_kp_start)
        for (int a = p.link_kp_start[l]; a < p.link_kp_start[l + 1]; ++a)
        {
          const AdjEntry ae = p.link_kp[a];
          const int lt = adj_col_map(ae.type), D = lt == 0 ? Dp : (lt == 1 ? Dg : 14);
          const float *A = kp_AtA(p, lt);
          const int ci = edge_col(lt, ae.role, bi, p.CS), cj = edge_col(lt, 1 - ae.role, bj, p.CS);
          if (ci >= 0 && cj >= 0)
            acc += (double)A[(size_t)ae.edge * D * D + (size_t)ci * D + cj];
        }
      lnk[(size_t)l * BB + idx] = acc;
    }
  }
  else
  {
    if (part != 0)
      return;
    const int wave = threadIdx.x >> 6, lane = threadIdx.x & 63;
    const bool photo = (wave & 1) == 0;
    const int which = wave >> 1;
    const float *st = photo ? p.stats_p : p.stats_g;
    const int n = photo ? p.n_edges_p : p.n_edges_g;
    double acc = 0.0;
    if (st && wave < 4)
      for (int e = lane; e < n; e += 64)
        acc += (double)st[2 * e + which];
    if (KP && p.stats_k && wave < 2)
    {
      const float *sk = p.stats_k + (photo ? 0 : 2 * (size_t)p.n_kr);
      const int nk = photo ? p.n_kr : p.n_km + p.n_kl;
      for (int t = lane; t < nk; t += 64)
        acc += (double)sk[2 * t];
    }
    for (int off = 32; off > 0; off >>= 1)
      acc += __shfl_down(acc, off);
    if (lane == 0 && wave < 4)
    {
      tail[which * 2 + (photo ? 0 : 1)] = acc;
      if (p.tail_mirror)
        p.tail_mirror[which * 2 + (photo ? 0 : 1)] = acc;
    }
  }
}

struct WindowFinalizeParams
{
  PhotoFinalizeParams ph;
  GeoFinalizeParams ge;
  int n_p, n_g;
};

template <int CS>
__global__ __launch_bounds__(kFinalizeBlock) void window_finalize_kernel(const WindowFinalizeParams prm)
{
  constexpr int LDS = photo_finalize_lds_doubles(CS) > geo_finalize_lds_doubles(CS) ? photo_finalize_lds_doubles(CS)
                                                                                    : geo_finalize_lds_doubles(CS);
  __shared__ double s[LDS];
  const int bid = (int)blockIdx.x;
  if (bid < prm.n_g)
    geo_finalize_body<CS>(prm.ge, bid, s);
  else
    photo_finalize_body<CS>(prm.ph, bid - prm.n_g, s);
}

template <bool KP>
__global__ __launch_bounds__(1024) void error_totals_kernel(const ErrorTotalsSide ph, const ErrorTotalsSide ge, double *out,
                                                            double *mirror, double epoch, const KpTotals kp)
{
  for (int idx = threadIdx.x; idx < ph.n_edges + ge.n_edges; idx += blockDim.x)
  {
    const bool photo = idx < ph.n_edges;
    const ErrorTotalsSide &sd = photo ? ph : ge;
    const int e = photo ? idx : idx - ph.n_edges;
    const int first = sd.edge_first[e], nt = sd.edge_tiles[e];
    float se = 0.f, sn = 0.f;
    for (int t0 = 0; t0 < nt; t0 += 8)
    {
      float ve[8], vn[8];
#pragma unroll
      for (int u = 0; u < 8; ++u)
      {
        const int t = t0 + u < nt ? t0 + u : nt - 1;
        ve[u] = sd.partials[(size_t)(first + t) * sd.stride + sd.err_off];
        vn[u] = sd.partials[(size_t)(first + t) * sd.stride + sd.cnt_off];
      }
#pragma unroll
      for (int u = 0; u < 8; ++u)
        if (t0 + u < nt)
        {
          se += ve[u];
          sn += vn[u];
        }
    }
    sd.stats[2 * e + 0] = sn > 0.f ? sd.scale * se / sn : sd.fallback;
    sd.stats[2 * e + 1] = sn;
  }
  __threadfence_block();
  __syncthreads();
  const int wave = threadIdx.x >> 6, lane = threadIdx.x & 63;
  if (wave >= 4)
    return;
  const bool photo = (wave & 1) == 0;
  const int which = wave >> 1;
  const ErrorTotalsSide &sd = photo ? ph : ge;
  double acc = 0.0;
  for (int e0 = lane; e0 < sd.n_edges; e0 += 64 * 8)
  {
    float v[8];
#pragma unroll
    for (int u = 0; u < 8; ++u)
    {
      const int e = e0 + 64 * u;
      v[u] = sd.stats[2 * (e < sd.n_edges ? e : lane) + which];
    }
#pragma unroll
    for (int u = 0; u < 8; ++u)
      if (e0 + 64 * u < sd.n_edges)
        acc += (double)v[u];
  }
  if (KP && kp.stats && which == 0)
  {
    const float *sk = kp.stats + (photo ? 0 : 2 * (size_t)kp.n_kr);
    const int nk = photo ? kp.n_kr : kp.n_km + kp.n_kl;
    for (int t = lane; t < nk; t += 64)
      acc += (double)sk[2 * t];
  }
  for (int off = 32; off > 0; off >>= 1)
    acc += __shfl_down(acc, off);
  if (lane == 0)
  {
    out[which * 2 + (photo ? 0 : 1)] = acc;
    if (mirror)
    {
      mirror[which * 2 + (photo ? 0 : 1)] = acc;
      __threadfence_system();
      *reinterpret_cast<volatile double *>(mirror + 4 + which * 2 + (photo ? 0 : 1)) = epoch;
    }
  }
}

}

static LaunchCommon window_lc(SageWindow *w, int type, bool photo_linearize = false)
{
  const DenseSide &sd = w->dense[type];
  LaunchCommon lc{};
  lc.work = sd.work.as<WorkItem>();
  lc.edge_first = sd.first.as<int32_t>();
  lc.edge_tiles = sd.tiles.as<int32_t>();
  lc.n_work = sd.n_work;
  lc.n_edges = w->n_edges;
  lc.partials = sd.part.as<float>();
  lc.tiles_per_block = sd.tpb;
  lc.packed = type == kPhoto;
  if (photo_linearize && w->photo_rec.flush > 0)
  {
    lc.edge_first = w->photo_rec.first.as<int32_t>();
    lc.edge_tiles = w->photo_rec.count.as<int32_t>();
    lc.flush = w->photo_rec.flush;
  }
  return lc;
}

template <class E, class P>
static void finalize_side(P &fp, const DenseSide &sd, int set, const LaunchCommon &lc)
{
  const EdgeOut out = sd.out();
  fp.table = sd.tab[set].as<E>();
  fp.edge_first = lc.edge_first; fp.edge_tiles = lc.edge_tiles; fp.partials = lc.partials;
  fp.AtA = out.AtA; fp.Atb = out.Atb; fp.stats = out.stats; fp.wide = out.wide;
}

static float photo_weight_sum(const SageWindowConfig &c)
{
  float wsum = 0.f;
  for (int l = 0; l < c.pyr.levels; ++l)
    wsum += c.photo_weights[l];
  return wsum;
}

static AssembleParams window_assemble_params(SageWindow *w)
{
  const SageWindowConfig &c = w->cfg;
  AssembleParams ap{};
  const bool has = w->n_edges > 0;
  const EdgeOut op = w->dense[kPhoto].out(), og = w->dense[kGeo].out();
  ap.AtA_p = (has && c.use_photo) ? op.AtA : nullptr;
  ap.Atb_p = op.Atb;
  ap.stats_p = (has && c.use_photo) ? op.stats : nullptr;
  ap.wide_p = (has && c.use_photo) ? op.wide : nullptr;
  ap.AtA_g = (has && c.use_geo) ? og.AtA : nullptr;
  ap.Atb_g = og.Atb;
  ap.stats_g = (has && c.use_geo) ? og.stats : nullptr;
  ap.wide_g = (has && c.use_geo) ? og.wide : nullptr;
  ap.adj_start = w->adj_start.as<int32_t>();
  ap.adj = w->adj.as<AdjEntry>();
  ap.links = w->link_edges.as<LinkEdges>();
  ap.packed = w->packed.as<double>();
  ap.tail_mirror = w->kernels_mirror_totals() ? w->mirror.h + TotalsMirror::kTail : nullptr;
  ap.K = w->K;
  ap.nlinks = (int)w->links.size();
  ap.CS = c.CS;
  ap.n_edges_p = w->n_edges;
  ap.n_edges_g = w->n_edges;
  ap.split = 1;
  ap.blocks = nullptr;
  if (w->n_terms() > 0)
  {
    ap.AtA_kr = w->AtA_kr.as<float>(); ap.Atb_kr = w->Atb_kr.as<float>();
    ap.AtA_km = w->AtA_km.as<float>(); ap.Atb_km = w->Atb_km.as<float>();
    ap.AtA_kl = w->AtA_kl.as<float>(); ap.Atb_kl = w->Atb_kl.as<float>();
    ap.n_kl = w->n_kl;
    ap.stats_k = w->stats_k.as<float>();
    ap.link_kp_start = w->kp_link_start.as<int32_t>();
    ap.link_kp = w->kp_link.as<AdjEntry>();
    ap.n_kr = w->n_kr;
    ap.n_km = w->n_km;
  }
  return ap;
}

static int window_launch_keypoints(SageWindow *w, int set, bool jac)
{
  const int nloc = w->n_terms();
  if (nloc == 0)
    return SAGE_OK;
  KpBatchParams kp{};
  kp.terms = w->kp_table.as<KpTerm>();
  kp.vars = w->vars[set].as<float>();
  kp.VS = w->VS;
  kp.cam = w->cfg.pyr.cam[0];
  kp.eps = w->cfg.eps;
  kp.AtA_r = w->AtA_kr.as<float>(); kp.Atb_r = w->Atb_kr.as<float>();
  kp.AtA_m = w->AtA_km.as<float>(); kp.Atb_m = w->Atb_km.as<float>();
  kp.AtA_l = w->AtA_kl.as<float>(); kp.Atb_l = w->Atb_kl.as<float>();
  kp.stats = w->stats_k.as<float>() + (jac ? 0 : (size_t)2 * nloc);
  LaunchCommon lc{};
  prof_attach(w, jac ? 4 : 5, lc);
  if (lc.ev_start)
    (void)hipEventRecord(lc.ev_start, w->stream);
  SAGE_HIP(launch_keypoint_batch(w->stream, w->cfg.CS, jac, nloc, w->kp_kinds(), kp));
  if (lc.ev_stop)
    (void)hipEventRecord(lc.ev_stop, w->stream);
  if (jac)
    w->kp_lin = true;
  return SAGE_OK;
}

int window_linearize_set(SageWindow *w, int set, double *dst, bool local_blocks, bool merge)
{
  if (!w || !w->finalized)
    return SAGE_E_STATE;
  const SageWindowConfig &c = w->cfg;
  const int H = (int)c.pyr.cam[0].h, W = (int)c.pyr.cam[0].w;
  const bool dense = w->n_edges > 0;
  LaunchCommon lcg{}, lcp{};
  merge = merge && w->merge_ok;
  if (dense)
  {
    const bool have_depth = w->dpt_set == set;
    SAGE_HIP(launch_depth_batch(w->stream, c.CS, w->depth_items[set].as<DepthItem>(), w->n_depth, H, W, !have_depth,
                                !(have_depth && w->dgrad_valid)));
    w->dpt_set = set;
    w->dgrad_valid = true;
    lcg = window_lc(w, kGeo);
    lcp = window_lc(w, kPhoto, true);
    lcg.stage = 1;
    lcp.stage = 1;
    lcg.merge_geo_weight = lcp.merge_geo_weight = merge ? c.geo_weight : 0.f;
    if (c.use_geo)
    {
      prof_attach(w, 1, lcg);
      SAGE_HIP(launch_geo_linearize(w->stream, c.CS, nullptr, w->dense[kGeo].tab[set].as<GeoEdge>(), lcg, c.pyr.cam[0], c.eps,
                                    c.geo_loss_param, c.geo_weight, w->dense[kGeo].out()));
    }
    if (c.use_photo)
    {
      prof_attach(w, 0, lcp);
      SAGE_HIP(launch_photo_linearize(w->stream, c.CS, c.FS, nullptr, w->dense[kPhoto].tab[set].as<PhotoEdge>(), lcp, c.pyr,
                                      c.photo_weights, c.eps, w->dense[kPhoto].out()));
    }
  }
  {
    const int rck = window_launch_keypoints(w, set, true);
    if (rck)
      return rck;
  }
  if (dense)
  {
    WindowFinalizeParams fp{};
    fp.n_p = c.use_photo ? w->n_edges : 0;
    fp.n_g = c.use_geo ? w->n_edges : 0;
    finalize_side<PhotoEdge>(fp.ph, w->dense[kPhoto], set, lcp);
    fp.ph.wsum = photo_weight_sum(c);
    finalize_side<GeoEdge>(fp.ge, w->dense[kGeo], set, lcg);
    fp.ge.weight = c.geo_weight;
    if (merge)
    {
      fp.ge.photo_partials = lcp.partials;
      fp.ge.photo_rec_first = lcp.edge_first;
      fp.ge.photo_rec_count = lcp.edge_tiles;
    }
    if (c.CS == 32)
      hipLaunchKernelGGL((window_finalize_kernel<32>), dim3(fp.n_p + fp.n_g), dim3(kFinalizeBlock), 0, w->stream, fp);
    else
      hipLaunchKernelGGL((window_finalize_kernel<16>), dim3(fp.n_p + fp.n_g), dim3(kFinalizeBlock), 0, w->stream, fp);
    SAGE_HIP(hipGetLastError());
  }
  AssembleParams ap = window_assemble_params(w);
  if (dst)
    ap.packed = dst;
  ap.split = 4;
  int nblocks = w->K + ap.nlinks + 1;
  if (local_blocks && w->dist.n_asm_blocks > 0)
  {
    ap.blocks = w->dist.asm_blocks.as<int32_t>();
    nblocks = w->dist.n_asm_blocks;
  }
  if (w->n_terms() > 0)
    hipLaunchKernelGGL(assemble_kernel<true>, dim3(nblocks * ap.split), dim3(512), 0, w->stream, ap);
  else
    hipLaunchKernelGGL(assemble_kernel<false>, dim3(nblocks * ap.split), dim3(512), 0, w->stream, ap);
  SAGE_HIP(hipGetLastError());
  window_phase_mark(w, 1);
  if (ap.packed == w->packed.as<double>())
  {
    w->have_lin = true;
    w->lin_epoch = set == 0 ? w->vars_epoch : 0;
    w->spec_err_valid = false;
    w->dist.packed_reduced = false;
  }
  return SAGE_OK;
}

extern "C" int sage_window_linearize(SageWindow *w)
{
  if (w)
    window_phase_mark(w, 0);
  return window_linearize_set(w, 0);
}

struct PartialRecord
{
  int stride, err_slot, cnt_slot;
};
constexpr PartialRecord kOwnRecord{2, 0, 1};
constexpr PartialRecord kFusedPhoto{4, 0, 1}, kFusedGeo{4, 2, 3};

static ErrorTotalsSide error_totals_side(const LaunchCommon &lc, float *stats, float fallback, float scale, int n_edges,
                                         PartialRecord rec)
{
  ErrorTotalsSide sd{};
  sd.edge_first = lc.edge_first; sd.edge_tiles = lc.edge_tiles; sd.partials = lc.partials;
  sd.stats = stats;
  sd.fallback = fallback; sd.scale = scale;
  sd.n_edges = n_edges;
  sd.stride = rec.stride; sd.err_off = rec.err_slot; sd.cnt_off = rec.cnt_slot;
  return sd;
}

int window_error_pass(SageWindow *w, int which, bool speculate_gradients)
{
  if (!w || !w->finalized || which < 0 || which > 1)
    return SAGE_E_STATE;
  const SageWindowConfig &c = w->cfg;
  const int H = (int)c.pyr.cam[0].h, W = (int)c.pyr.cam[0].w;
  const bool has = w->n_edges > 0;
  if (has && w->dpt_set != which)
  {
    SAGE_HIP(launch_depth_batch(w->stream, c.CS, w->depth_items[which].as<DepthItem>(), w->n_depth, H, W, true, false));
    w->dpt_set = which;
    w->dgrad_valid = false;
  }
  ErrorTotalsSide ph{}, ge{};
  const bool fused = has && c.use_photo && c.use_geo;
  if (has && c.use_photo)
  {
    LaunchCommon lc = window_lc(w, kPhoto);
    prof_attach(w, 2, lc);
    lc.stage = 1;
    lc.fused_geo_loss_param = fused ? c.geo_loss_param : 0.f;
    SAGE_HIP(launch_photo_error(w->stream, c.CS, c.FS, nullptr, w->dense[kPhoto].tab[which].as<PhotoEdge>(), lc, c.pyr,
                                c.photo_weights, c.eps, w->dense[kPhoto].stats.as<float>()));
    ph = error_totals_side(lc, w->dense[kPhoto].stats.as<float>(), 10.0f * photo_weight_sum(c), 1.0f, w->n_edges,
                           fused ? kFusedPhoto : kOwnRecord);
    if (fused)
      ge = error_totals_side(lc, w->dense[kGeo].stats.as<float>(), 10.0f * c.geo_weight, c.geo_weight, w->n_edges, kFusedGeo);
  }
  if (has && c.use_geo && !fused)
  {
    LaunchCommon lc = window_lc(w, kGeo);
    prof_attach(w, 3, lc);
    lc.stage = 1;
    SAGE_HIP(launch_geo_error(w->stream, c.CS, nullptr, w->dense[kGeo].tab[which].as<GeoEdge>(), lc, c.pyr.cam[0], c.eps,
                              c.geo_loss_param, c.geo_weight, w->dense[kGeo].stats.as<float>()));
    ge = error_totals_side(lc, w->dense[kGeo].stats.as<float>(), 10.0f * c.geo_weight, c.geo_weight, w->n_edges, kOwnRecord);
  }
  KpTotals kpt{};
  if (w->n_terms() > 0)
  {
    const int rck = window_launch_keypoints(w, which, false);
    if (rck)
      return rck;
    kpt = KpTotals{w->stats_k.as<float>() + (size_t)2 * w->n_terms(), w->n_kr, w->n_km, w->n_kl};
  }
  w->mirror.err_epoch += 1;
  double *const mirror = w->kernels_mirror_totals() ? w->mirror.h + TotalsMirror::kError : nullptr;
  if (kpt.stats)
    hipLaunchKernelGGL(error_totals_kernel<true>, dim3(1), dim3(1024), 0, w->stream, ph, ge, w->errbuf.as<double>(), mirror,
                       (double)w->mirror.err_epoch, kpt);
  else
    hipLaunchKernelGGL(error_totals_kernel<false>, dim3(1), dim3(1024), 0, w->stream, ph, ge, w->errbuf.as<double>(), mirror,
                       (double)w->mirror.err_epoch, kpt);
  SAGE_HIP(hipGetLastError());
// ... 11 lines not shown
```

### sage_slam_amd/csrc/window_lm.hip

```cpp
#include "runtime_internal.h"

enum class LmSeq { classic, schur, at_candidate };

static LmSeq lm_sequence_for(const SageWindow *w, const SageLmConfig *cfg)
{
  const bool sharded = w->dist.allreduce != nullptr;
  if (sharded && w->dist.shard)
    return LmSeq::schur;
  const bool at_candidate = cfg->linearize_at_candidate > 0 || (cfg->linearize_at_candidate == 0 && sharded);
  return at_candidate && !w->links.empty() ? LmSeq::at_candidate : LmSeq::classic;
}

struct LmEval
{
  double cur_tot[4];
  bool have_cur_tot;
};

static int window_form_system(SageWindow *w, int set, double *dst, int it)
{
  int rc;
  if (!w->dist.allreduce)
    return (rc = window_linearize_set(w, set, dst, false, true)) ? rc : window_mirror_totals(w, false, dst);
  if ((rc = window_linearize_set(w, set, w->dist.packed_loc.as<double>(), true, true)) ||
      (rc = window_allreduce_into(w, w->dist.packed_loc.as<double>(), dst, sage_window_packed_count(w), it)))
    return rc;
  window_phase_mark(w, 2);
  return window_mirror_totals(w, false, dst);
}

static int lm_prepare(LmSeq seq, SageWindow *w, SageLmState *st)
{
  int rc;
  const bool sharded = w->dist.allreduce != nullptr;
  const size_t np = sage_window_packed_count(w);
  if (seq != LmSeq::at_candidate)
  {
    if ((rc = window_linearize_set(w, 0, nullptr, false, true)) ||
        (seq == LmSeq::classic && sharded && (rc = window_allreduce(w, w->packed.as<double>(), np, w->dist.emu_cur))))
      return rc;
    window_phase_mark(w, 2);
    return SAGE_OK;
  }
  if ((rc = w->packed_save.reserve(np * sizeof(double))))
    return rc;
  if (sharded && !w->dist.packed_loc.p)
  {
    if ((rc = w->dist.packed_loc.reserve(np * sizeof(double))))
      return rc;
    SAGE_HIP(hipMemsetAsync(w->dist.packed_loc.p, 0, np * sizeof(double), w->stream));
  }
  bool mirrored_now = false;
  if (!(w->have_lin && w->lin_epoch == w->vars_epoch && (!sharded || w->dist.packed_reduced)))
  {
    if ((rc = window_form_system(w, 0, w->packed.as<double>(), w->dist.emu_cur)))
      return rc;
    w->have_lin = true;
    w->lin_epoch = w->vars_epoch;
    w->dist.packed_reduced = true;
    w->spec_err_valid = false;
    mirrored_now = true;
  }
  if (!w->spec_err_valid)
  {
    if (!mirrored_now && (rc = window_mirror_totals(w, false)))
      return rc;
    if (!window_wait_reduced_totals(w))
      SAGE_HIP(hipStreamSynchronize(w->stream));
    w->spec_error = mirrored_error(w, TotalsMirror::kTail, 0);
    w->spec_err_valid = true;
  }
  st->error = w->spec_error;
  return SAGE_OK;
}

static int evaluate_schur(SageWindow *w, SageLmState *st, bool first)
{
  int rc;
  double lin_error = 0;
  if ((rc = window_schur_solve(w, st->damp, &lin_error)) && rc != SAGE_E_NOT_PSD)
    return rc;
  window_phase_mark(w, 3);
  if (first)
    st->error = lin_error;
  st->candidate_error = INFINITY;
  if (rc == SAGE_E_NOT_PSD)
    return SAGE_OK;
  if ((rc = sage_window_error(w, 1)))
    return rc;
  window_add_to_double(w, w->errbuf.as<double>(), window_prior_error(w, 1, true));
  if ((rc = window_collective(w, w->errbuf.as<double>(), 4)))
    return rc;
  double t4[4];
  SAGE_HIP(hipMemcpyAsync(t4, w->errbuf.p, sizeof(t4), hipMemcpyDeviceToHost, w->stream));
  SAGE_HIP(hipStreamSynchronize(w->stream));
  st->candidate_error = t4[0] + t4[1];
  return SAGE_OK;
}

static int evaluate_at_candidate(SageWindow *w, SageLmState *st, LmEval &ev)
{
  int rc;
  std::memcpy(ev.cur_tot, w->mirror.h, sizeof(ev.cur_tot));
  ev.have_cur_tot = true;
  bool not_psd;
  if ((rc = window_form_system(w, 1, w->packed_save.as<double>(), w->dist.emu_cur + 1)) ||
      (rc = window_wait_mirror(w, &not_psd)))
    return rc;
  st->candidate_error = not_psd ? INFINITY : mirrored_error(w, TotalsMirror::kTail, 1);
  return SAGE_OK;
}

static int evaluate_classic(SageWindow *w, SageLmState *st, bool first)
{
  int rc;
  const bool sharded = w->dist.allreduce != nullptr;
  if ((rc = window_error_pass(w, 1, !sharded)))
    return rc;
  if (!sharded)
  {
    const bool idle = window_wait_error_totals(w);
    if (first && (rc = window_total_error(w, 1, &st->error, idle)))
      return rc;
    if ((rc = window_total_error(w, 0, &st->candidate_error, idle)) == SAGE_E_NOT_PSD)
      st->candidate_error = INFINITY;
    return rc == SAGE_E_NOT_PSD ? SAGE_OK : rc;
  }
  bool not_psd;
  if ((rc = window_allreduce(w, w->errbuf.as<double>(), 4, w->dist.emu_cur + 1)) || (rc = window_mirror_totals(w, true)) ||
      (rc = window_wait_mirror(w, &not_psd)))
    return rc;
  if (first)
    st->error = mirrored_error(w, TotalsMirror::kTail, 0);
  st->candidate_error = not_psd ? INFINITY : mirrored_error(w, TotalsMirror::kError, 1);
  return SAGE_OK;
}

static int lm_evaluate(LmSeq seq, SageWindow *w, SageLmState *st, bool first, LmEval &ev)
{
  if (seq == LmSeq::schur)
    return evaluate_schur(w, st, first);
  const int rc = sage_window_solve(w, st->damp, nullptr);
  if (rc == SAGE_E_NOT_PSD)
  {
    st->candidate_error = INFINITY;
    return first && seq == LmSeq::classic ? sage_window_total_error(w, 1, &st->error) : SAGE_OK;
  }
  if (rc)
    return rc;
  return seq == LmSeq::at_candidate ? evaluate_at_candidate(w, st, ev) : evaluate_classic(w, st, first);
}

static int lm_accept(LmSeq seq, SageWindow *w, const SageLmState *st)
{
  const int rc = sage_window_accept(w);
  if (rc || seq != LmSeq::at_candidate)
    return rc;
  w->packed.swap(w->packed_save);
  w->lin_epoch = w->vars_epoch;
  w->dist.packed_reduced = true;
  w->spec_error = st->candidate_error;
  return SAGE_OK;
}

static void lm_reject(SageWindow *w, const LmEval &ev)
{
  if (ev.have_cur_tot)
    std::memcpy(w->mirror.h, ev.cur_tot, sizeof(ev.cur_tot));
}

extern "C" int sage_window_lm_step(SageWindow *w, SageLmState *st, const SageLmConfig *cfg)
{
  if (!w || !st || !cfg)
    return SAGE_E_INVALID;
  if (w->world > 1 && !w->dist.allreduce)
    return SAGE_E_STATE;
  const LmSeq seq = lm_sequence_for(w, cfg);
  auto clampd = [&](double d) { return std::min(std::max((double)cfg->min_damp, d), (double)cfg->max_damp); };
  if (st->iters == 0 && st->damp <= 0)
    st->damp = cfg->init_damp;
  window_phase_mark(w, 0);
  int rc = lm_prepare(seq, w, st);
  if (rc)
    return rc;
  st->accepted = 0;
  for (int evals = 1;; ++evals)
  {
    LmEval ev{};
    if ((rc = lm_evaluate(seq, w, st, evals == 1, ev)))
      return rc;
    if (st->candidate_error < st->error)
    {
      st->accepted = 1;
      if ((rc = lm_accept(seq, w, st)))
        return rc;
      st->damp = clampd(st->damp / cfg->damp_dec_factor);
      break;
    }
    lm_reject(w, ev);
    const bool give_up = st->damp >= cfg->max_damp || (cfg->max_inner_evals > 0 && evals >= cfg->max_inner_evals);
    st->damp = clampd(st->damp * cfg->damp_inc_factor);
    if (give_up)
      break;
  }
  st->iters += 1;
  return SAGE_OK;
}

static int window_lm_run(SageWindow *w, SageLmState *st, const SageLmConfig *cfg, int n, double *trace, int *done,
                         double *step_seconds)
{
  if (!w || !st || !cfg || n < 0)
    return SAGE_E_INVALID;
  int i = 0, rc = SAGE_OK;
  auto t_prev = std::chrono::steady_clock::now();
  for (; i < n; ++i)
  {
    if ((rc = sage_window_lm_step(w, st, cfg)))
      break;
    if (trace)
    {
      trace[4 * i + 0] = st->error;
      trace[4 * i + 1] = st->candidate_error;
      trace[4 * i + 2] = (double)st->accepted;
      trace[4 * i + 3] = st->damp;
    }
    if (step_seconds)
    {
      const auto t = std::chrono::steady_clock::now();
      step_seconds[i] = std::chrono::duration<double>(t - t_prev).count();
      t_prev = t;
    }
  }
  if (done)
    *done = i;
  return rc;
}

extern "C" int sage_window_lm_run(SageWindow *w, SageLmState *st, const SageLmConfig *cfg, int n, double *trace, int *done)
{
  return window_lm_run(w, st, cfg, n, trace, done, nullptr);
}

extern "C" int sage_window_lm_run_timed(SageWindow *w, SageLmState *st, const SageLmConfig *cfg, int n, double *trace,
                                        int *done, double *step_seconds)
{
  return window_lm_run(w, st, cfg, n, trace, done, step_seconds);
}
```

### sage_slam_amd/csrc/window_plan.h

```cpp
#pragma once

#include <algorithm>
#include <vector>

namespace sage
{
namespace plan
{

struct Ownership
{
  std::vector<int> edges;
  std::vector<int> links;
};

inline Ownership owned_edges(int nlinks, int rank, int world, bool by_link)
{
  Ownership o;
  const long long nl = nlinks;
  if (by_link)
  {
    const int lo = (int)(nl * rank / world), hi = (int)(nl * (rank + 1) / world);
    for (int l = lo; l < hi; ++l)
    {
      o.edges.push_back(2 * l);
      o.edges.push_back(2 * l + 1);
    }
  }
  else
  {
    const int lo = (int)(2 * nl * rank / world), hi = (int)(2 * nl * (rank + 1) / world);
    for (int ge = lo; ge < hi; ++ge)
      o.edges.push_back(ge);
  }
  for (int ge : o.edges)
    if (o.links.empty() || o.links.back() != ge / 2)
      o.links.push_back(ge / 2);
  return o;
}

inline std::vector<int> dense_edges(const std::vector<int> &owned, const std::vector<char> &link_is_dense)
{
  std::vector<int> out;
  for (int ge : owned)
    if (ge >= 0 && (size_t)(ge / 2) < link_is_dense.size() && link_is_dense[ge / 2])
      out.push_back(ge);
  return out;
}

inline bool uses_domain_solve(int world, int K, int requested)
{
  return world > 1 && (requested >= 0 ? requested != 0 : K >= 256);
}

struct SolverRows
{
  int B = 0, Bs = 0;
  int kept = 7;
  std::vector<int> to_block;
  std::vector<int> to_solver;
  bool compact() const { return Bs != B; }
};

inline SolverRows solver_rows(const unsigned char *hold, int K, int CS)
{
  const int first[3] = {0, 6, 6 + CS}, size[3] = {6, CS, 1};
  SolverRows s;
  s.B = 7 + CS;
  int all = K > 0 ? 7 : 0;
  for (int k = 0; k < K; ++k)
    all &= hold ? hold[k] : 0;
  s.kept = (all == 7) ? 7 : (7 & ~all);
  s.to_solver.assign(s.B, -1);
  for (int grp = 0; grp < 3; ++grp)
    if (s.kept & (1 << grp))
      for (int r = first[grp]; r < first[grp] + size[grp]; ++r)
      {
        s.to_solver[r] = (int)s.to_block.size();
        s.to_block.push_back(r);
      }
  s.Bs = (int)s.to_block.size();
  return s;
}

inline long long total_tiles(const std::vector<int> &tiles)
{
  long long total = 0;
  for (int t : tiles)
    total += t;
  return total;
}

inline int typical_edge(std::vector<int> tiles)
{
  if (tiles.empty())
    return 1;
  std::nth_element(tiles.begin(), tiles.begin() + tiles.size() / 2, tiles.end());
  return std::max(1, tiles[tiles.size() / 2]);
}

inline int geo_run(long long total)
{
  return total >= 8192 ? 16 : (total >= 4096 ? 8 : (total >= 512 ? 4 : 2));
}

inline int photo_run(const std::vector<int> &tiles, int FS)
{
  const long long total = total_tiles(tiles);
  const int T = typical_edge(tiles);
  int tpb = total >= 4096 ? 8 : (total >= 1536 ? 4 : (total >= 768 ? 2 : 1));
  if (FS == 32 && total >= 1536 && total < 4096)
    tpb = 6;
  {
    const int nwg = (T + tpb - 1) / tpb, rem = T % tpb;
    if (rem != 0 && 4 * rem < 3 * tpb)
      tpb = (T + nwg - 1) / nwg;
  }
  if (T >= 48 && ((T + tpb - 1) / tpb) % 8 != 0)
    for (int mod : {8, 4})
      for (int t : {8, 9, 10, 12, 6, 15, 16, 20})
        if (((T + t - 1) / t) % mod == 0)
          return t;
  return tpb;
}

inline int record_cadence(int tpb)
{
  if (tpb < 6)
    return 0;
  return tpb % 4 == 0 ? 4 : (tpb % 5 == 0 ? 5 : (tpb % 3 == 0 ? 3 : 0));
}

inline std::vector<int> tune_candidates(int rule, int typical)
{
  std::vector<int> cand{rule};
  for (int t : {4, 6, 8, 9, 10, 12, 16})
    if (t != rule && t <= typical && 2 * t >= std::min(rule, 8))
      cand.push_back(t);
  return cand;
}

}
}
```

### sage_slam_amd/csrc/window_profile.hip

```cpp
#include "runtime_internal.h"

WindowProfiler::~WindowProfiler()
{
  for (auto &pm : phase_pending)
    for (auto &m : pm.ev)
      (void)hipEventDestroy(m.second);
  for (auto &m : phase_cur.ev)
    (void)hipEventDestroy(m.second);
  for (auto &pend : pending)
    for (auto &pr : pend)
    {
      (void)hipEventDestroy(pr.first);
      (void)hipEventDestroy(pr.second);
    }
  for (hipEvent_t e : ev_free)
    (void)hipEventDestroy(e);
}

static bool ev_get(WindowProfiler &pf, hipEvent_t *e)
{
  if (!pf.ev_free.empty())
  {
    *e = pf.ev_free.back();
    pf.ev_free.pop_back();
    return true;
  }
  return hipEventCreate(e) == hipSuccess;
}
static void ev_put(WindowProfiler &pf, hipEvent_t e)
{
  if (e)
    pf.ev_free.push_back(e);
}

void prof_attach(SageWindow *w, int which, LaunchCommon &lc)
{
  WindowProfiler &pf = w->prof;
  if (!pf.profiling || (pf.prof_level == 2 && which != 0))
    return;
  hipEvent_t a, b;
  if (!ev_get(pf, &a))
    return;
  if (!ev_get(pf, &b))
  {
    ev_put(pf, a);
    return;
  }
  lc.ev_start = a;
  lc.ev_stop = b;
  pf.pending[which].emplace_back(a, b);
}

void window_phase_mark(SageWindow *w, int which)
{
  WindowProfiler &pf = w->prof;
  if (!pf.profiling || pf.prof_level == 2)
    return;
  if (which == 0)
  {
    if (pf.phase_cur.ev.size() >= 2)
    {
      if (pf.phase_pending.size() >= 1024)
      {
        for (auto &m : pf.phase_pending.front().ev)
          ev_put(pf, m.second);
        pf.phase_pending.erase(pf.phase_pending.begin());
      }
      pf.phase_pending.push_back(std::move(pf.phase_cur));
    }
    else
      for (auto &m : pf.phase_cur.ev)
        ev_put(pf, m.second);
    pf.phase_cur = WindowProfiler::PhaseMarks{};
  }
  else if (pf.phase_cur.ev.empty())
    return;
  hipEvent_t e;
  if (pf.phase_cur.ev.size() >= 64 || !ev_get(pf, &e))
    return;
  (void)hipEventRecord(e, w->stream);
  pf.phase_cur.ev.emplace_back(which, e);
}

extern "C" int sage_window_get_phase_time(SageWindow *w, double *ms4, int *iterations)
{
  if (!w || !ms4)
    return SAGE_E_INVALID;
  WindowProfiler &pf = w->prof;
  SAGE_HIP(hipStreamSynchronize(w->stream));
  window_phase_mark(w, 0);
  for (auto &m : pf.phase_cur.ev)
    ev_put(pf, m.second);
  pf.phase_cur = WindowProfiler::PhaseMarks{};
  for (auto &pm : pf.phase_pending)
  {
    double d4[4] = {0, 0, 0, 0};
    bool ok = true;
    for (size_t i = 1; i < pm.ev.size() && ok; ++i)
    {
      float d = 0.f;
      ok = hipEventElapsedTime(&d, pm.ev[i - 1].second, pm.ev[i].second) == hipSuccess;
      const int ph = pm.ev[i].first;
      if (ok && ph >= 1 && ph <= 4)
        d4[ph - 1] += d;
    }
    if (ok)
    {
      for (int i = 0; i < 4; ++i)
        pf.phase_ms[i] += d4[i];
      pf.phase_n += 1;
    }
    for (auto &m : pm.ev)
      ev_put(pf, m.second);
  }
  pf.phase_pending.clear();
  for (int i = 0; i < 4; ++i)
  {
    ms4[i] = pf.phase_ms[i];
    pf.phase_ms[i] = 0;
  }
  if (iterations)
    *iterations = pf.phase_n;
  pf.phase_n = 0;
  return SAGE_OK;
}

extern "C" int sage_window_set_profiling(SageWindow *w, int on)
{
  if (!w)
    return SAGE_E_INVALID;
  WindowProfiler &pf = w->prof;
  pf.profiling = on != 0;
  pf.prof_level = on;
  while (pf.profiling && pf.ev_free.size() < 512)
  {
    hipEvent_t e;
    if (hipEventCreate(&e) != hipSuccess)
      break;
    pf.ev_free.push_back(e);
  }
  return SAGE_OK;
}

extern "C" int sage_window_get_kernel_time(SageWindow *w, int which, double *total_ms, int *launches)
{
  if (!w || which < 0 || which > 5)
    return SAGE_E_INVALID;
  WindowProfiler &pf = w->prof;
  SAGE_HIP(hipStreamSynchronize(w->stream));
  for (auto &pr : pf.pending[which])
  {
    float ms = 0.f;
    if (hipEventElapsedTime(&ms, pr.first, pr.second) == hipSuccess)
    {
      pf.prof_ms[which] += ms;
      pf.prof_n[which] += 1;
    }
    ev_put(pf, pr.first);
    ev_put(pf, pr.second);
  }
  pf.pending[which].clear();
  if (total_ms)
    *total_ms = pf.prof_ms[which];
  if (launches)
    *launches = pf.prof_n[which];
  pf.prof_ms[which] = 0;
  pf.prof_n[which] = 0;
  return SAGE_OK;
}
```

### sage_slam_amd/csrc/window_solve.hip

```cpp
#include "damped_system.h"
#include "runtime_internal.h"

double window_prior_error(const SageWindow *w, int set, bool owned_only)
{
  const SageWindowConfig &c = w->cfg;
  double e = 0;
  auto keyframe0_terms = [&] {
    if (c.scale_prior_weight > 0)
    {
      const double d = std::log((double)w->hv.scale_init[0]) - std::log((double)w->hv.scale[set][0]);
      e += c.scale_prior_weight * d * d;
    }
    if (c.pose_prior_weight > 0)
    {
      double loc[6];
      sage::pose_local(&w->hv.pose[set][0], &w->hv.pose_init[0], loc);
      for (int i = 0; i < 6; ++i)
        e += c.pose_prior_weight * loc[i] * loc[i];
    }
  };
  for (int k = 0; k < w->K; ++k)
  {
    if (owned_only && sage_shard_keyframe_owner(w->dist.shard, k) != w->rank)
      continue;
    double s = 0;
    for (int i = 0; i < c.CS; ++i)
      s += (double)w->hv.code[set][(size_t)k * c.CS + i] * w->hv.code[set][(size_t)k * c.CS + i];
    e += c.code_prior_weight * s / c.CS;
    if (owned_only && k == 0)
      keyframe0_terms();
  }
  if (!owned_only)
    keyframe0_terms();
  return e;
}

static sage::SolvePriors window_solve_priors(const SageWindow *w)
{
  const SageWindowConfig &c = w->cfg;
  sage::SolvePriors pri{};
  pri.code_w = c.code_prior_weight; pri.scale_w = c.scale_prior_weight; pri.pose_w = c.pose_prior_weight;
  pri.scale_init0 = w->hv.scale_init[0];
  std::copy_n(&w->hv.pose_init[0], 12, pri.pose_init0);
  return pri;
}

static void window_priors(const SageWindow *w, std::vector<double> &dadd, std::vector<double> &gadd)
{
  const int K = w->K, B = w->B, CS = w->cfg.CS;
  const sage::SolvePriors pri = window_solve_priors(w);
  dadd.assign((size_t)K * B, 0.0);
  gadd.assign((size_t)K * B, 0.0);
  for (int k = 0; k < K; ++k)
    for (int r = 0; r < B; ++r)
      sage::prior_row(pri, k, r, CS, &w->hv.pose[0][(size_t)k * 12], w->hv.scale[0][k], &w->hv.code[0][(size_t)k * CS],
                      dadd[(size_t)k * B + r], gadd[(size_t)k * B + r], w->hold.empty() ? 0 : w->hold[k]);
}

static void window_retract_candidate(SageWindow *w, bool local_only)
{
  const int K = w->K, B = w->B, CS = w->cfg.CS;
  if (local_only)
    w->hv.copy_set(1, 0);
  for (int k = 0; k < K; ++k)
  {
    if (local_only && !sage_shard_keyframe_is_local(w->dist.shard, k))
      continue;
    const int hold = w->hold.empty() ? 0 : w->hold[k];
    float d6[6];
    for (int i = 0; i < 6; ++i)
      d6[i] = (float)w->delta[(size_t)k * B + i];
    if (hold & sage::kHoldPose)
      std::copy_n(&w->hv.pose[0][(size_t)k * 12], 12, &w->hv.pose[1][(size_t)k * 12]);
    else
      sage_pose_retract(&w->hv.pose[0][(size_t)k * 12], d6, &w->hv.pose[1][(size_t)k * 12]);
    for (int i = 0; i < CS; ++i)
      w->hv.code[1][(size_t)k * CS + i] =
          (hold & sage::kHoldCode) ? w->hv.code[0][(size_t)k * CS + i]
                                   : w->hv.code[0][(size_t)k * CS + i] + (float)w->delta[(size_t)k * B + 6 + i];
    w->hv.scale[1][k] = (hold & sage::kHoldScale) ? w->hv.scale[0][k] : w->hv.scale[0][k] + (float)w->delta[(size_t)k * B + 6 + CS];
  }
}

int window_sync_candidate(SageWindow *w, bool stream_idle)
{
  if (!w->cand_pending)
    return SAGE_OK;
  if (!stream_idle)
    SAGE_HIP(hipStreamSynchronize(w->stream));
  w->cand_pending = false;
  const DeviceSolver *S = w->solver;
  if (solver_host_status(S) != 0)
    return SAGE_E_NOT_PSD;
  const float *v = solver_host_vars(S);
  for (int k = 0; k < w->K; ++k)
    w->hv.unpack(1, k, w->cfg.CS, v + (size_t)k * w->VS);
  std::memcpy(w->delta.data(), solver_host_delta(S), w->delta.size() * sizeof(double));
  return SAGE_OK;
}

extern "C" int sage_window_solve(SageWindow *w, double damp, double *step_norm)
{
  if (!w || !w->finalized || !w->have_lin)
    return SAGE_E_STATE;
  const SageWindowConfig &c = w->cfg;
  const int K = w->K, B = w->B, CS = c.CS;
  if (w->solver)
  {
    int rc = window_sync_candidate(w);
    if (rc && rc != SAGE_E_NOT_PSD)
      return rc;
    if (w->dpt_set == 1)
      w->dpt_set = -1;
    rc = solver_run(w->solver, w->stream, w->packed.as<double>(), w->vars[0].as<float>(), w->vars[1].as<float>(), CS,
                    damp, window_solve_priors(w));
    if (rc)
      return rc;
    window_phase_mark(w, 3);
    w->cand_pending = true;
    if (step_norm)
// ... 174 lines not shown
```

### sage_slam_amd/csrc/window_state.h

```cpp
#pragma once

namespace sage_rt
{

enum : int { kPhoto = 0, kGeo = 1 };

static inline size_t dense_dim(int type, int CS) { return type == kPhoto ? 13 + (size_t)CS : 14 + 2 * (size_t)CS; }

struct HostVars
{
  std::vector<float> pose[2], code[2], scale[2];
  std::vector<float> code_init, scale_init, pose_init;
  std::vector<float> code_added;
  void copy_set(int dst, int src) { pose[dst] = pose[src], code[dst] = code[src], scale[dst] = scale[src]; }

  template <class T>
  void pack(int set, int k, int CS, T *rec) const
  {
    for (int i = 0; i < 12; ++i)
      rec[i] = pose[set][(size_t)k * 12 + i];
    rec[12] = scale[set][k];
    for (int i = 0; i < CS; ++i)
      rec[13 + i] = code[set][(size_t)k * CS + i];
  }
  template <class T>
  void unpack(int set, int k, int CS, const T *rec)
  {
    for (int i = 0; i < 12; ++i)
      pose[set][(size_t)k * 12 + i] = (float)rec[i];
    scale[set][k] = (float)rec[12];
    for (int i = 0; i < CS; ++i)
      code[set][(size_t)k * CS + i] = (float)rec[13 + i];
  }
};

struct DenseSide
{
  DevBuf tab[2];
  DevBuf work, first, tiles;
  DevBuf part;
  DevBuf AtA, Atb, stats;
  DevBuf wide;
  int n_work = 0, tpb = 1;
  EdgeOut out() const { return EdgeOut{AtA.as<float>(), Atb.as<float>(), stats.as<float>(), wide.as<double>()}; }
  int reserve_results(size_t ne, size_t D, size_t records, size_t partial_floats)
  {
    int rc;
    if ((rc = part.reserve(std::max<size_t>(1, records) * partial_floats * sizeof(float))) ||
        (rc = AtA.reserve(ne * D * D * sizeof(float))) || (rc = Atb.reserve(ne * D * sizeof(float))) ||
        (rc = stats.reserve(ne * 2 * sizeof(float))) || (rc = wide.reserve(ne * (D * D + D) * sizeof(double))))
      return rc;
    return 0;
  }
};

struct PhotoRecordPlan
{
  DevBuf first, count;
  int flush = 0, n = 0;
};

struct TotalsMirror
{
  enum : int { kTail = 0, kError = 4, kErrorTickets = 8, kMirrorTickets = 12, kDoubles = 16 };
  double *h = nullptr;
  uint64_t err_epoch = 0;
  uint64_t mirror_epoch = 0;
  TotalsMirror() = default;
  TotalsMirror(const TotalsMirror &) = delete;
  TotalsMirror &operator=(const TotalsMirror &) = delete;
  ~TotalsMirror()
  {
    if (h)
      (void)hipHostFree(h);
  }
  bool wait(int ticket_group, uint64_t epoch) const
  {
    const double *t = h + ticket_group;
    const double want = (double)epoch;
    auto ticket = [t](int i) {
      double v;
      __atomic_load(t + i, &v, __ATOMIC_ACQUIRE);
      return v;
    };
    const auto t0 = std::chrono::steady_clock::now();
    unsigned spins = 0;
    while (!(ticket(0) == want && ticket(1) == want && ticket(2) == want && ticket(3) == want))
    {
      __builtin_ia32_pause();
      if ((++spins & 0x3ff) == 0 &&
          std::chrono::duration<double>(std::chrono::steady_clock::now() - t0).count() > 0.05)
        return false;
    }
    std::atomic_thread_fence(std::memory_order_acquire);
    return true;
  }
};

struct WindowDist
{
  SageAllReduceFn allreduce = nullptr;
  int (*allreduce2)(const double *send, double *recv, size_t n, void *user) = nullptr;
  void *allreduce_user = nullptr;
  void *rccl_hook = nullptr;
  SageShardPlan *shard = nullptr;
  DevBuf sepbuf;
  std::vector<double> h_sep;
  const double *emu_rest = nullptr;
  int emu_n = 0, emu_cur = 0;
  DevBuf packed_loc;
  DevBuf asm_blocks;
  int n_asm_blocks = 0;
  bool packed_reduced = false;
};

struct WindowProfiler
{
  struct PhaseMarks
  {
    std::vector<std::pair<int, hipEvent_t>> ev;
  };
  std::vector<PhaseMarks> phase_pending;
  PhaseMarks phase_cur;
  double phase_ms[4] = {0, 0, 0, 0};
  int phase_n = 0;
  bool profiling = false;
  int prof_level = 0;
  std::vector<std::pair<hipEvent_t, hipEvent_t>> pending[6];
  std::vector<hipEvent_t> ev_free;
  double prof_ms[6] = {0, 0, 0, 0, 0, 0};
  int prof_n[6] = {0, 0, 0, 0, 0, 0};
  WindowProfiler() = default;
  WindowProfiler(const WindowProfiler &) = delete;
  WindowProfiler &operator=(const WindowProfiler &) = delete;
  ~WindowProfiler();
};

}
```

Before: 261,900 Mresiduals/s.

## Overlap early block-Cholesky rows with late linearization via split solve

Adds a split plan that divides keyframes into early rows, whose edges do not touch a late zone, and late rows. Linearization of early edges is issued first, and the scatter and factorisation of early solver rows start on a side stream while the late photometric edges are still being linearized. This aims to hide solve latency behind linearize work in the classic LM sequence. It adds stream and event synchronisation, more kernel launches and a more complex plan, and it only applies when the block plan has the expected permutation and no arrow rows.

```diff
diff --git a/include/sage_ba.h b/include/sage_ba.h
--- a/include/sage_ba.h
+++ b/include/sage_ba.h
@@ -115,6 +115,9 @@
 
 int sage_block_solve(const double *packed_host, int K, int nlinks, const int32_t *links, int B, double damp,
                      const double *diag_add, const double *g_add, double *delta);
+int sage_solve_split_plan(int K, int nlinks, const int32_t *links, const int32_t *runs, int slots, int rounds,
+                          int32_t *head, int32_t *perm, int32_t *late_edge, int32_t *late_link, int32_t *late_kf,
+                          int32_t *order, int32_t *blk_row, int32_t *blk_col, int32_t *blk_src, int cap);
 long long sage_solve_lookahead_count(void);
 
 typedef struct SageLmConfig
@@ -217,6 +220,7 @@
 
 int sage_window_linearize(SageWindow *w);
 int sage_window_error(SageWindow *w, int which);
+int sage_window_early_solve_info(const SageWindow *w, long long *info8);
 int sage_window_tune_runs(SageWindow *w, int *tpb_out, int *tpb_rule_out, float *ms_rule_out, float *ms_best_out);
 int sage_window_set_runs(SageWindow *w, int tpb);
 double *sage_window_error_dev(SageWindow *w);
diff --git a/sage_slam_amd/capi.py b/sage_slam_amd/capi.py
--- a/sage_slam_amd/capi.py
+++ b/sage_slam_amd/capi.py
@@ -100,12 +100,12 @@
     "sage_tracker_photo_jac_error_calculate", "sage_tracker_photo_error_calculate",
     "sage_geometric_jac_error_calculate", "sage_geometric_error_calculate", "sage_depth_and_grad",
     "sage_gaussian_pyramid_with_grad", "sage_se3_exp", "sage_pose_retract", "sage_nearest_psd", "sage_nearest_psd_reference", "sage_factor_block_count", "sage_factor_hessian_blocks",
-    "sage_damped_solve_qr_f32", "sage_block_solve", "sage_solve_lookahead_count", "sage_lm_config_default", "sage_track_lm", "sage_track_frame",
+    "sage_damped_solve_qr_f32", "sage_block_solve", "sage_solve_split_plan", "sage_solve_lookahead_count", "sage_lm_config_default", "sage_track_lm", "sage_track_frame",
     "sage_window_create", "sage_window_destroy", "sage_window_add_keyframe", "sage_window_add_link", "sage_window_add_keypoint_link", "sage_window_hold", "sage_window_set_link_geo_loss",
     "sage_window_set_shard", "sage_window_finalize", "sage_window_num_keyframes", "sage_window_num_links",
     "sage_window_block_size", "sage_window_solver_block_size", "sage_window_packed_count", "sage_window_packed_dev",
     "sage_window_residuals_per_linearize", "sage_window_bytes_per_linearize", "sage_window_linearize",
-    "sage_window_error", "sage_window_tune_runs", "sage_window_set_runs", "sage_window_error_dev", "sage_window_solve", "sage_window_total_error",
+    "sage_window_error", "sage_window_early_solve_info", "sage_window_tune_runs", "sage_window_set_runs", "sage_window_error_dev", "sage_window_solve", "sage_window_total_error",
     "sage_window_accept", "sage_window_reset", "sage_window_get_keyframe", "sage_window_set_keyframe", "sage_window_get_delta",
     "sage_window_get_edge", "sage_window_add_keypoint_term", "sage_window_num_keypoint_terms", "sage_window_get_keypoint_term", "sage_window_prepass", "sage_window_factor", "sage_window_factor_error", "sage_window_prepare_factors", "sage_factor_psd", "sage_factor_cut_blocks", "sage_window_set_profiling", "sage_window_get_kernel_time", "sage_window_get_phase_time", "sage_window_lm_step", "sage_window_lm_run", "sage_window_lm_run_timed", "sage_window_sync_variables", "sage_window_set_allreduce", "sage_shard_plan_create", "sage_shard_plan_create_domains", "sage_block_solve_domains", "sage_shard_plan_destroy", "sage_shard_sep_count", "sage_shard_num_separators", "sage_shard_num_interior", "sage_shard_keyframe_owner", "sage_shard_keyframe_is_local", "sage_shard_eliminate", "sage_shard_solve", "sage_rccl_unique_id", "sage_rccl_comm_create", "sage_rccl_comm_destroy", "sage_rccl_comm_info", "sage_window_use_rccl", "sage_window_emulate_peers", "sage_sort_locations", "sage_bind_thread_to_device", "sage_solver_helper_cpus", "sage_solver_placement_moves", "sage_placement_monitor", "sage_shutdown", "sage_host_threads_running",
     "sage_valid_locations", "sage_shuffle_indices", "sage_sample_locations",
@@ -141,6 +141,28 @@
             getattr(L, name).argtypes = [C.c_void_p]
         _lib = L
     return _lib
+
+
+def solve_split_plan(K, links, runs, slots, rounds=1):
+    nl = len(links)
+    lk = np.ascontiguousarray(np.asarray(links, dtype=np.int32).reshape(-1))
+    rn = np.ascontiguousarray(np.full(2 * nl, runs, dtype=np.int32) if np.isscalar(runs) else np.asarray(runs, dtype=np.int32))
+    cap = K * (K + 1) // 2 + 8
+    ip = lambda a: a.ctypes.data_as(C.POINTER(C.c_int32))
+    out = {k: np.zeros(n, dtype=np.int32) for k, n in (("head", 8), ("perm", K), ("late_edge", max(1, 2 * nl)),
+                                                         ("late_link", max(1, nl)), ("late_kf", K), ("order", cap),
+                                                         ("blk_row", cap), ("blk_col", cap), ("blk_src", cap))}
+    _chk(lib().sage_solve_split_plan(K, nl, ip(lk), ip(rn), int(slots), int(rounds), ip(out["head"]), ip(out["perm"]),
+                                     ip(out["late_edge"]), ip(out["late_link"]), ip(out["late_kf"]), ip(out["order"]),
+                                     ip(out["blk_row"]), ip(out["blk_col"]), ip(out["blk_src"]), cap), "sage_solve_split_plan")
+    h = out.pop("head")
+    nblk = int(h[2])
+    res = dict(n1=int(h[0]), n2=int(h[1]), nblk=nblk, early_rows=int(h[3]), zone=(int(h[4]), int(h[5])),
+               n_order_early=int(h[6]), arrow=bool(h[7]), perm=out["perm"].tolist(), late_edge=out["late_edge"][:2 * nl].tolist(),
+               late_link=out["late_link"][:nl].tolist(), late_kf=out["late_kf"].tolist())
+    for k in ("order", "blk_row", "blk_col", "blk_src"):
+        res[k] = out[k][:nblk].tolist()
+    return res
 
 
 def _chk(code: int, where: str):
@@ -602,6 +624,12 @@
     def error(self, which=1):
         _chk(lib().sage_window_error(self.h, which), "sage_window_error")
 
+    def early_solve_info(self):
+        v = (C.c_longlong * 8)()
+        _chk(lib().sage_window_early_solve_info(self.h, v), "sage_window_early_solve_info")
+        keys = ("on", "early_rows", "zone_lo", "zone_hi", "early_items", "late_items", "fused_evals", "photo_launches")
+        return dict(zip(keys, (int(x) for x in v)))
+
     def tune_runs(self):
         tpb, rule = C.c_int(0), C.c_int(0)
         ms_rule, ms_best = C.c_float(0), C.c_float(0)
diff --git a/sage_slam_amd/csrc/block_solver.cpp b/sage_slam_amd/csrc/block_solver.cpp
--- a/sage_slam_amd/csrc/block_solver.cpp
+++ b/sage_slam_amd/csrc/block_solver.cpp
@@ -10,6 +10,7 @@
 #include <vector>
 
 #include "block_solver.h"
+#include "window_plan.h"
 #include "damped_system.h"
 #include "host_math.h"
 #include "sage_ba.h"
@@ -1676,3 +1677,43 @@
     std::memcpy(delta + (size_t)k * B, y.data() + (size_t)bp.pos[k] * Bp, sizeof(double) * B);
   return SAGE_OK;
 }
+
+extern "C" int sage_solve_split_plan(int K, int nlinks, const int32_t *links, const int32_t *runs, int slots, int rounds,
+                                     int32_t *head, int32_t *perm, int32_t *late_edge, int32_t *late_link, int32_t *late_kf,
+                                     int32_t *order, int32_t *blk_row, int32_t *blk_col, int32_t *blk_src, int cap)
+{
+  if (K < 1 || nlinks < 0 || (nlinks > 0 && (!links || !runs)) || !head || !perm || !late_edge || !late_link || !late_kf ||
+      !order || !blk_row || !blk_col || !blk_src)
+    return SAGE_E_INVALID;
+  std::vector<std::pair<int, int>> lk(nlinks);
+  for (int l = 0; l < nlinks; ++l)
+    lk[l] = {links[2 * l], links[2 * l + 1]};
+  sage::BlockPlan bp;
+  const int rcp = sage::plan_blocks(K, lk, !sage::env_flag("SAGE_SOLVE_NO_SPLIT"), bp);
+  if (rcp != SAGE_OK)
+    return rcp;
+  if (bp.nblk > cap)
+    return SAGE_E_INVALID;
+  const bool arrow = sage::block_plan_has_arrow_rows(sage::envelope_of(bp, 40));
+  sage::plan::SolveSplit sp;
+  if (!arrow)
+    sp = sage::plan::solve_split(K, lk, bp.perm.data(), bp.n1, bp.n2, std::vector<int>(runs, runs + 2 * (size_t)nlinks), slots,
+                                 rounds);
+  const std::vector<int> ord =
+      sage::plan::scatter_order(K, bp.n1, bp.n2, bp.row_first.data(), bp.row_off.data(), bp.a_cnt.data(), bp.a_off.data());
+  head[0] = bp.n1; head[1] = bp.n2; head[2] = bp.nblk; head[3] = sp.early_rows; head[4] = sp.zone_lo; head[5] = sp.zone_hi;
+  head[6] = sp.split() ? sage::plan::scatter_order_prefix(sp.early_rows, bp.n1, bp.row_first.data(), bp.a_cnt.data()) : 0;
+  head[7] = arrow ? 1 : 0;
+  std::copy(bp.perm.begin(), bp.perm.end(), perm);
+  for (int e = 0; e < 2 * nlinks; ++e)
+    late_edge[e] = sp.split() ? sp.late_edge[e] : 0;
+  for (int l = 0; l < nlinks; ++l)
+    late_link[l] = sp.split() ? sp.late_link[l] : 0;
+  for (int k = 0; k < K; ++k)
+    late_kf[k] = sp.split() ? sp.late_kf[k] : 0;
+  std::copy(ord.begin(), ord.end(), order);
+  std::copy(bp.blk_row.begin(), bp.blk_row.end(), blk_row);
+  std::copy(bp.blk_col.begin(), bp.blk_col.end(), blk_col);
+  std::copy(bp.blk_src.begin(), bp.blk_src.end(), blk_src);
+  return SAGE_OK;
+}
diff --git a/sage_slam_amd/csrc/photo_kernels.hip b/sage_slam_amd/csrc/photo_kernels.hip
--- a/sage_slam_amd/csrc/photo_kernels.hip
+++ b/sage_slam_amd/csrc/photo_kernels.hip
@@ -1407,6 +1407,24 @@
   });
 }
 
+hipError_t photo_linearize_resident_workgroups(int CS, int FS, bool merged, int *slots)
+{
+  return dispatch_cs_fs(CS, FS, [&](auto cs, auto fs) {
+    constexpr int C = decltype(cs)::value, F = decltype(fs)::value;
+    int dev = 0, cus = 0, per_cu = 0;
+    hipError_t e;
+    if ((e = hipGetDevice(&dev)) != hipSuccess ||
+        (e = hipDeviceGetAttribute(&cus, hipDeviceAttributeMultiprocessorCount, dev)) != hipSuccess)
+      return e;
+    if (merged)
+      e = hipOccupancyMaxActiveBlocksPerMultiprocessor(&per_cu, photo_kernel<C, F, true, 2>, kBlock, 0);
+    else
+      e = hipOccupancyMaxActiveBlocksPerMultiprocessor(&per_cu, photo_kernel<C, F, true, 1>, kBlock, 0);
+    *slots = per_cu * cus;
+    return e;
+  });
+}
+
 hipError_t launch_photo_error(hipStream_t s, int CS, int FS, const PhotoEdge *single, const PhotoEdge *table,
                               const LaunchCommon &lc, const SagePyramid &pyr, const float *weights_host,
                               float eps, float *stats)
diff --git a/sage_slam_amd/csrc/runtime_internal.h b/sage_slam_amd/csrc/runtime_internal.h
--- a/sage_slam_amd/csrc/runtime_internal.h
+++ b/sage_slam_amd/csrc/runtime_internal.h
@@ -296,6 +296,7 @@
     int psd_mode = -1;
   } fc;
   WindowProfiler prof;
+  EarlySolvePlan early;
 
   bool kernels_mirror_totals() const { return world == 1 && !dist.allreduce && mirror.h; }
 };
@@ -318,6 +319,8 @@
 std::vector<int32_t> window_link_pairs(const SageWindow *w);
 int window_linearize_set(SageWindow *w, int set, double *dst = nullptr, bool local_blocks = false, bool merge = false);
 int window_error_pass(SageWindow *w, int which, bool speculate_gradients);
+bool window_early_solve_ready(const SageWindow *w);
+int window_linearize_solve(SageWindow *w, double damp);
 int window_collective(SageWindow *w, double *buf, size_t n);
 int window_allreduce(SageWindow *w, double *buf, size_t n, int iterate);
 int window_allreduce_into(SageWindow *w, const double *send, double *recv, size_t n, int iterate);
@@ -332,5 +335,6 @@
 double window_prior_error(const SageWindow *w, int set, bool owned_only = false);
 int window_sync_candidate(SageWindow *w, bool stream_idle = false);
 int window_schur_solve(SageWindow *w, double damp, double *lin_error);
-void prof_attach(SageWindow *w, int which, LaunchCommon &lc);
+sage::SolvePriors window_solve_priors(const SageWindow *w);
+void prof_attach(SageWindow *w, int which, LaunchCommon &lc, bool more = false);
 void window_phase_mark(SageWindow *w, int which);
diff --git a/sage_slam_amd/csrc/sage_internal.h b/sage_slam_amd/csrc/sage_internal.h
--- a/sage_slam_amd/csrc/sage_internal.h
+++ b/sage_slam_amd/csrc/sage_internal.h
@@ -4,6 +4,7 @@
 #include <stdint.h>
 
 #include <cmath>
+#include <functional>
 #include <utility>
 #include <vector>
 
@@ -137,6 +138,7 @@
   double *wide = nullptr;
 };
 
+hipError_t photo_linearize_resident_workgroups(int CS, int FS, bool merged, int *slots);
 hipError_t launch_photo_linearize(hipStream_t s, int CS, int FS, const PhotoEdge *single, const PhotoEdge *table,
                                   const LaunchCommon &lc, const SagePyramid &pyr, const float *weights_host,
                                   float eps, const EdgeOut &out);
@@ -223,6 +225,11 @@
 int solver_set_holds(DeviceSolver *S, const std::vector<uint8_t> &hold, hipStream_t stream);
 int solver_run(DeviceSolver *S, hipStream_t stream, const double *packed_dev, const float *vars0, float *vars1, int CS,
                double damp, const SolvePriors &pri);
+int solver_run_split(DeviceSolver *S, hipStream_t stream, hipStream_t side, hipEvent_t ev_early, hipEvent_t ev_side,
+                     const double *packed_dev, const float *vars0, float *vars1, int CS, double damp, const SolvePriors &pri,
+                     int early_rows, const std::function<int()> &enqueue_rest);
+struct BlockPlan;
+const BlockPlan &solver_block_plan(const DeviceSolver *S);
 const float *solver_host_vars(const DeviceSolver *S);
 const double *solver_host_delta(const DeviceSolver *S);
 double solver_host_step_norm2(const DeviceSolver *S);
diff --git a/sage_slam_amd/csrc/solve_kernels.hip b/sage_slam_amd/csrc/solve_kernels.hip
--- a/sage_slam_amd/csrc/solve_kernels.hip
+++ b/sage_slam_amd/csrc/solve_kernels.hip
@@ -3,6 +3,7 @@
 #include <chrono>
 #include <cstdio>
 #include <cstring>
+#include <functional>
 #include <memory>
 #include <vector>
 
@@ -42,8 +43,8 @@
                                                             const float *__restrict__ vars0, int VS, int CS,
                                                             const SolvePriors pri, double damp,
                                                             double *__restrict__ L, double *__restrict__ y,
-                                                            const int32_t *__restrict__ order, unsigned *flags,
-                                                            unsigned epoch)
+                                                            const int32_t *__restrict__ order, int first, int count,
+                                                            unsigned *flags, unsigned epoch)
 {
   const int tid = threadIdx.x;
   const int B = P.B, Bs = P.Bs, Bp = P.Bp, BB = B * B;
@@ -52,7 +53,7 @@
   if (tid < Bs)
     s_row[tid] = P.to_block[tid];
   __syncthreads();
-  for (int it = blockIdx.x; it < P.nblk; it += gridDim.x)
+  for (int it = first + blockIdx.x; it < first + count; it += gridDim.x)
   {
     const int b = order[it];
     const int i = P.blk_row[b], j = P.blk_col[b], srcf = P.blk_src[b];
@@ -261,28 +262,8 @@
   };
   const size_t o_rf = put(row_first), o_ro = put(row_off), o_br = put(blk_row), o_bc = put(blk_col),
                o_bs = put(blk_src), o_pm = put(perm), o_ps = put(pos);
-  std::vector<int32_t> order;
-  auto push_row = [&](int i) {
-    for (int q = 0; q < a_cnt[i]; ++q)
-      order.push_back(a_off[i] + q);
-    for (int q = 0; q <= i - row_first[i]; ++q)
-      order.push_back(row_off[i] + q);
-  };
-  if (n1 > 0)
-  {
-    for (int t = 0; t < std::max(n1, n2); ++t)
-    {
-      if (t < n1)
-        push_row(t);
-      if (t < n2)
-        push_row(n1 + t);
-    }
-    for (int i = n1 + n2; i < K; ++i)
-      push_row(i);
-  }
-  else
-    for (int i = 0; i < K; ++i)
-      push_row(i);
+  const std::vector<int32_t> order =
+      plan::scatter_order(K, n1, n2, row_first.data(), row_off.data(), a_cnt.data(), a_off.data());
   const size_t o_ord = put(order);
   const size_t o_tb = put(rows.to_block), o_ts = put(rows.to_solver);
   if (hipMalloc(&S->d_int, all.size() * sizeof(int32_t)) != hipSuccess)
@@ -334,23 +315,35 @@
   return SAGE_OK;
 }
 
-int solver_run(DeviceSolver *S, hipStream_t stream, const double *packed_dev, const float *vars0, float *vars1,
-               int CS, double damp, const SolvePriors &pri)
+struct SolveInFlight
+{
+  SolveLease lease;
+  BlockEnvelope env;
+  explicit SolveInFlight(DeviceSolver *S) : env(envelope_of(S->host_plan, S->Bp))
+  {
+    if (env.n1 > 0)
+      env.no_lookahead = block_chol_arm(block_plan_has_arrow_rows(env), block_plan_long_arrow_chains(env));
+    S->epoch += 1;
+    if (S->epoch == 0)
+      S->epoch = 1;
+  }
+};
+
+static hipError_t solver_launch_scatter(DeviceSolver *S, hipStream_t stream, const double *packed_dev, const float *vars0,
+                                        int CS, double damp, const SolvePriors &pri, int first, int count)
+{
+  hipLaunchKernelGGL(solve_scatter_kernel, dim3(std::max(1, std::min(kScatterWorkgroups, count))), dim3(256), 0, stream,
+                     S->plan, packed_dev, vars0, S->VS, CS, pri, damp, reinterpret_cast<double *>(S->h_T), S->h_y, S->d_order,
+                     first, count, S->h_flags, S->epoch);
+  return hipGetLastError();
+}
+
+static int solver_retract_and_factorise(DeviceSolver *S, SolveInFlight &run, hipStream_t stream, const float *vars0,
+                                        float *vars1, int CS)
 {
   static const bool dbgt = sage::env_flag("SAGE_DEBUG_TIMING");
   hipError_t eh;
-  SolveLease lease;
-  BlockEnvelope env = envelope_of(S->host_plan, S->Bp);
-  if (env.n1 > 0)
-    env.no_lookahead = block_chol_arm(block_plan_has_arrow_rows(env), block_plan_long_arrow_chains(env));
-  S->epoch += 1;
-  if (S->epoch == 0)
-    S->epoch = 1;
-  hipLaunchKernelGGL(solve_scatter_kernel, dim3(std::min(kScatterWorkgroups, S->nblk)), dim3(256), 0, stream, S->plan,
-                     packed_dev, vars0, S->VS, CS, pri, damp, reinterpret_cast<double *>(S->h_T), S->h_y, S->d_order,
-                     S->h_flags, S->epoch);
-  if ((eh = hipGetLastError()) != hipSuccess)
-    return (int)eh;
+  BlockEnvelope &env = run.env;
   volatile unsigned *go = &S->result()->go;
   S->go_epoch = (S->go_epoch + 1) & 0x7fffffffu;
   if (S->go_epoch == 0)
@@ -386,6 +379,42 @@
   return SAGE_OK;
 }
 
+int solver_run(DeviceSolver *S, hipStream_t stream, const double *packed_dev, const float *vars0, float *vars1,
+               int CS, double damp, const SolvePriors &pri)
+{
+  SolveInFlight run(S);
+  hipError_t eh;
+  if ((eh = solver_launch_scatter(S, stream, packed_dev, vars0, CS, damp, pri, 0, S->nblk)) != hipSuccess)
+    return (int)eh;
+  return solver_retract_and_factorise(S, run, stream, vars0, vars1, CS);
+}
+
+int solver_run_split(DeviceSolver *S, hipStream_t stream, hipStream_t side, hipEvent_t ev_early, hipEvent_t ev_side,
+                     const double *packed_dev, const float *vars0, float *vars1, int CS, double damp, const SolvePriors &pri,
+                     int early_rows, const std::function<int()> &enqueue_rest)
+{
+  const BlockPlan &bp = S->host_plan;
+  if (early_rows < 1 || early_rows > std::min(bp.n1, bp.n2))
+    return SAGE_E_INVALID;
+  const int n_early = plan::scatter_order_prefix(early_rows, bp.n1, bp.row_first.data(), bp.a_cnt.data());
+  SolveInFlight run(S);
+  hipError_t eh;
+  if ((eh = hipEventRecord(ev_early, stream)) != hipSuccess || (eh = hipStreamWaitEvent(side, ev_early, 0)) != hipSuccess ||
+      (eh = solver_launch_scatter(S, side, packed_dev, vars0, CS, damp, pri, 0, n_early)) != hipSuccess ||
+      (eh = hipEventRecord(ev_side, side)) != hipSuccess)
+    return (int)eh;
+  const int rc = enqueue_rest();
+  if ((eh = hipStreamWaitEvent(stream, ev_side, 0)) != hipSuccess)
+    return (int)eh;
+  if (rc)
+    return rc;
+  if ((eh = solver_launch_scatter(S, stream, packed_dev, vars0, CS, damp, pri, n_early, S->nblk - n_early)) != hipSuccess)
+    return (int)eh;
+  return solver_retract_and_factorise(S, run, stream, vars0, vars1, CS);
+}
+
+const BlockPlan &solver_block_plan(const DeviceSolver *S) { return S->host_plan; }
+
 const float *solver_host_vars(const DeviceSolver *S) { return S->host_vars(); }
 const double *solver_host_delta(const DeviceSolver *S) { return S->host_delta(); }
 double solver_host_step_norm2(const DeviceSolver *S) { return S->result()->step_norm2; }
diff --git a/sage_slam_amd/csrc/window.hip b/sage_slam_amd/csrc/window.hip
--- a/sage_slam_amd/csrc/window.hip
+++ b/sage_slam_amd/csrc/window.hip
@@ -86,3 +86,14 @@
   }
   return SAGE_OK;
 }
+
+extern "C" int sage_window_early_solve_info(const SageWindow *w, long long *info8)
+{
+  if (!w || !info8 || !w->finalized)
+    return SAGE_E_STATE;
+  const EarlySolvePlan &ep = w->early;
+  const long long v[8] = {ep.on ? 1 : 0, ep.on ? ep.early_rows : 0, ep.on ? ep.zone_lo : 0, ep.on ? ep.zone_hi : 0,
+                          ep.on ? ep.n_work[0] : 0, ep.on ? ep.n_work[1] : 0, ep.fused_evals, ep.photo_launches};
+  std::copy(v, v + 8, info8);
+  return SAGE_OK;
+}
diff --git a/sage_slam_amd/csrc/window_build.hip b/sage_slam_amd/csrc/window_build.hip
--- a/sage_slam_amd/csrc/window_build.hip
+++ b/sage_slam_amd/csrc/window_build.hip
@@ -1,4 +1,5 @@
 #include "runtime_internal.h"
+#include "block_solver.h"
 #include "window_plan.h"
 
 static std::atomic<int> g_live_windows{0};
@@ -315,6 +316,71 @@
   return SAGE_OK;
 }
 
+static int window_plan_early_solve(SageWindow *w)
+{
+  static const bool off = sage::env_flag("SAGE_SOLVE_NO_EARLY");
+  EarlySolvePlan &ep = w->early;
+  ep.on = false;
+  const SageWindowConfig &c = w->cfg;
+  const int K = w->K, nl = (int)w->links.size();
+  if (off || !w->solver || w->world != 1 || w->n_terms() > 0 || w->n_edges == 0 || w->n_edges != 2 * nl || !c.use_photo ||
+      w->photo_rec.flush <= 0 || std::find(w->link_dense.begin(), w->link_dense.end(), (char)0) != w->link_dense.end())
+    return SAGE_OK;
+  const sage::BlockPlan &bp = sage::solver_block_plan(w->solver);
+  if (bp.n1 < 1 || sage::block_plan_has_arrow_rows(sage::envelope_of(bp, sage::padded_block(w->rows.Bs))))
+    return SAGE_OK;
+  int slots = 0;
+  SAGE_HIP(photo_linearize_resident_workgroups(c.CS, c.FS, w->merge_ok, &slots));
+  const int tpb = w->dense[kPhoto].tpb;
+  std::vector<int> runs(w->n_edges);
+  for (int e = 0; e < w->n_edges; ++e)
+    runs[e] = ((w->Nedge[e] + kTile - 1) / kTile + tpb - 1) / tpb;
+  const plan::SolveSplit sp = plan::solve_split(K, w->links, bp.perm.data(), bp.n1, bp.n2, runs, slots);
+  if (!sp.split())
+    return SAGE_OK;
+  std::vector<WorkItem> work;
+  std::vector<int32_t> edges, blocks;
+  for (int part = 0; part < 2; ++part)
+  {
+    for (int e = 0; e < w->n_edges; ++e)
+      if (sp.late_edge[e] == part)
+      {
+        edges.push_back(e);
+        for (int t = 0; t < (w->Nedge[e] + kTile - 1) / kTile; t += tpb)
+          work.push_back(WorkItem{(int32_t)e, t});
+      }
+    for (int k = 0; k < K; ++k)
+      if (sp.late_kf[k] == part)
+        blocks.push_back(k);
+    for (int l = 0; l < nl; ++l)
+      if (sp.late_link[l] == part)
+        blocks.push_back(K + l);
+    if (part == 1)
+      blocks.push_back(K + nl);
+    ep.n_work[part] = (int)work.size() - (part ? ep.n_work[0] : 0);
+    ep.n_edges[part] = (int)edges.size() - (part ? ep.n_edges[0] : 0);
+    ep.n_blocks[part] = (int)blocks.size() - (part ? ep.n_blocks[0] : 0);
+  }
+  if ((int)work.size() != w->dense[kPhoto].n_work || ep.n_work[0] < 1 || ep.n_work[1] < 1)
+    return SAGE_OK;
+  int rc;
+  if ((rc = upload(ep.work, work, w->stream)) || (rc = upload(ep.edges, edges, w->stream)) ||
+      (rc = upload(ep.blocks, blocks, w->stream)))
+    return rc;
+  SAGE_HIP(hipStreamSynchronize(w->stream));
+  if (!ep.side)
+    SAGE_HIP(hipStreamCreateWithFlags(&ep.side, hipStreamNonBlocking));
+  if (!ep.ev_early)
+    SAGE_HIP(hipEventCreateWithFlags(&ep.ev_early, hipEventDisableTiming));
+  if (!ep.ev_side)
+    SAGE_HIP(hipEventCreateWithFlags(&ep.ev_side, hipEventDisableTiming));
+  ep.early_rows = sp.early_rows;
+  ep.zone_lo = sp.zone_lo;
+  ep.zone_hi = sp.zone_hi;
+  ep.on = true;
+  return SAGE_OK;
+}
+
 static int window_plan_photo_runs(SageWindow *w, int tpb, int flush)
 {
   WorkList wp;
@@ -327,7 +393,9 @@
       (rc = upload(w->photo_rec.count, wp.rec_count, w->stream)))
     return rc;
   SAGE_HIP(hipStreamSynchronize(w->stream));
-  return ph.part.reserve(std::max<size_t>(1, std::max(ph.n_work, w->photo_rec.n)) * photo_partial_floats(w->cfg.CS) * sizeof(float));
+  if ((rc = ph.part.reserve(std::max<size_t>(1, std::max(ph.n_work, w->photo_rec.n)) * photo_partial_floats(w->cfg.CS) * sizeof(float))))
+    return rc;
+  return window_plan_early_solve(w);
 }
 
 static std::vector<int> edge_tiles(const std::vector<int> &Nedge)
@@ -740,7 +808,8 @@
     return rc;
   w->residuals_per_lin = fs.residuals;
   w->bytes_per_lin = fs.bytes;
-  if ((rc = finalize_work_lists(w, fs)) || (rc = finalize_results(w, fs)) || (rc = finalize_solver(w, fs)))
+  if ((rc = finalize_work_lists(w, fs)) || (rc = finalize_results(w, fs)) || (rc = finalize_solver(w, fs)) ||
+      (rc = window_plan_early_solve(w)))
     return rc;
   w->finalized = true;
   if (const char *e = getenv("SAGE_AUTOTUNE"))
diff --git a/sage_slam_amd/csrc/window_eval.hip b/sage_slam_amd/csrc/window_eval.hip
--- a/sage_slam_amd/csrc/window_eval.hip
+++ b/sage_slam_amd/csrc/window_eval.hip
@@ -1,3 +1,4 @@
+#include "damped_system.h"
 #include "runtime_internal.h"
 #include "finalize_bodies.h"
 
@@ -170,6 +171,7 @@
   PhotoFinalizeParams ph;
   GeoFinalizeParams ge;
   int n_p, n_g;
+  const int32_t *edges;
 };
 
 template <int CS>
@@ -180,9 +182,9 @@
   __shared__ double s[LDS];
   const int bid = (int)blockIdx.x;
   if (bid < prm.n_g)
-    geo_finalize_body<CS>(prm.ge, bid, s);
+    geo_finalize_body<CS>(prm.ge, prm.edges ? prm.edges[bid] : bid, s);
   else
-    photo_finalize_body<CS>(prm.ph, bid - prm.n_g, s);
+    photo_finalize_body<CS>(prm.ph, prm.edges ? prm.edges[bid - prm.n_g] : bid - prm.n_g, s);
 }
 
 template <bool KP>
@@ -342,6 +344,51 @@
   return ap;
 }
 
+static int window_launch_finalize(SageWindow *w, int set, const LaunchCommon &lcp, const LaunchCommon &lcg, bool merge,
+                                  const int32_t *edges, int n)
+{
+  const SageWindowConfig &c = w->cfg;
+  WindowFinalizeParams fp{};
+  fp.n_p = c.use_photo ? n : 0;
+  fp.n_g = c.use_geo ? n : 0;
+  fp.edges = edges;
+  finalize_side<PhotoEdge>(fp.ph, w->dense[kPhoto], set, lcp);
+  fp.ph.wsum = photo_weight_sum(c);
+  finalize_side<GeoEdge>(fp.ge, w->dense[kGeo], set, lcg);
+  fp.ge.weight = c.geo_weight;
+  if (merge)
+  {
+    fp.ge.photo_partials = lcp.partials;
+    fp.ge.photo_rec_first = lcp.edge_first;
+    fp.ge.photo_rec_count = lcp.edge_tiles;
+  }
+  if (fp.n_p + fp.n_g == 0)
+    return SAGE_OK;
+  if (c.CS == 32)
+    hipLaunchKernelGGL((window_finalize_kernel<32>), dim3(fp.n_p + fp.n_g), dim3(kFinalizeBlock), 0, w->stream, fp);
+  else
+    hipLaunchKernelGGL((window_finalize_kernel<16>), dim3(fp.n_p + fp.n_g), dim3(kFinalizeBlock), 0, w->stream, fp);
+  SAGE_HIP(hipGetLastError());
+  return SAGE_OK;
+}
+
+static int window_launch_assemble(SageWindow *w, double *dst, const int32_t *blocks, int nblocks)
+{
+  AssembleParams ap = window_assemble_params(w);
+  if (dst)
+    ap.packed = dst;
+  ap.split = 4;
+  ap.blocks = blocks;
+  if (nblocks < 1)
+    return SAGE_OK;
+  if (w->n_terms() > 0)
+    hipLaunchKernelGGL(assemble_kernel<true>, dim3(nblocks * ap.split), dim3(512), 0, w->stream, ap);
+  else
+    hipLaunchKernelGGL(assemble_kernel<false>, dim3(nblocks * ap.split), dim3(512), 0, w->stream, ap);
+  SAGE_HIP(hipGetLastError());
+  return SAGE_OK;
+}
+
 static int window_launch_keypoints(SageWindow *w, int set, bool jac)
 {
   const int nloc = w->n_terms();
@@ -377,6 +424,7 @@
   const int H = (int)c.pyr.cam[0].h, W = (int)c.pyr.cam[0].w;
   const bool dense = w->n_edges > 0;
   LaunchCommon lcg{}, lcp{};
+  int rc;
   merge = merge && w->merge_ok;
   if (dense)
   {
@@ -401,6 +449,7 @@
       prof_attach(w, 0, lcp);
       SAGE_HIP(launch_photo_linearize(w->stream, c.CS, c.FS, nullptr, w->dense[kPhoto].tab[set].as<PhotoEdge>(), lcp, c.pyr,
                                       c.photo_weights, c.eps, w->dense[kPhoto].out()));
+      w->early.photo_launches += 1;
     }
   }
   {
@@ -408,50 +457,92 @@
     if (rck)
       return rck;
   }
-  if (dense)
-  {
-    WindowFinalizeParams fp{};
-    fp.n_p = c.use_photo ? w->n_edges : 0;
-    fp.n_g = c.use_geo ? w->n_edges : 0;
-    finalize_side<PhotoEdge>(fp.ph, w->dense[kPhoto], set, lcp);
-    fp.ph.wsum = photo_weight_sum(c);
-    finalize_side<GeoEdge>(fp.ge, w->dense[kGeo], set, lcg);
-    fp.ge.weight = c.geo_weight;
-    if (merge)
-    {
-      fp.ge.photo_partials = lcp.partials;
-      fp.ge.photo_rec_first = lcp.edge_first;
-      fp.ge.photo_rec_count = lcp.edge_tiles;
-    }
-    if (c.CS == 32)
-      hipLaunchKernelGGL((window_finalize_kernel<32>), dim3(fp.n_p + fp.n_g), dim3(kFinalizeBlock), 0, w->stream, fp);
-    else
-      hipLaunchKernelGGL((window_finalize_kernel<16>), dim3(fp.n_p + fp.n_g), dim3(kFinalizeBlock), 0, w->stream, fp);
-    SAGE_HIP(hipGetLastError());
-  }
-  AssembleParams ap = window_assemble_params(w);
-  if (dst)
-    ap.packed = dst;
-  ap.split = 4;
-  int nblocks = w->K + ap.nlinks + 1;
-  if (local_blocks && w->dist.n_asm_blocks > 0)
-  {
-    ap.blocks = w->dist.asm_blocks.as<int32_t>();
-    nblocks = w->dist.n_asm_blocks;
-  }
-  if (w->n_terms() > 0)
-    hipLaunchKernelGGL(assemble_kernel<true>, dim3(nblocks * ap.split), dim3(512), 0, w->stream, ap);
-  else
-    hipLaunchKernelGGL(assemble_kernel<false>, dim3(nblocks * ap.split), dim3(512), 0, w->stream, ap);
-  SAGE_HIP(hipGetLastError());
+  if (dense && (rc = window_launch_finalize(w, set, lcp, lcg, merge, nullptr, w->n_edges)))
+    return rc;
+  const bool part = local_blocks && w->dist.n_asm_blocks > 0;
+  if ((rc = window_launch_assemble(w, dst, part ? w->dist.asm_blocks.as<int32_t>() : nullptr,
+                                   part ? w->dist.n_asm_blocks : w->K + (int)w->links.size() + 1)))
+    return rc;
   window_phase_mark(w, 1);
-  if (ap.packed == w->packed.as<double>())
+  if (!dst || dst == w->packed.as<double>())
   {
     w->have_lin = true;
     w->lin_epoch = set == 0 ? w->vars_epoch : 0;
     w->spec_err_valid = false;
     w->dist.packed_reduced = false;
   }
+  return SAGE_OK;
+}
+
+bool window_early_solve_ready(const SageWindow *w)
+{
+  return w->finalized && w->early.on && w->solver && w->world == 1 && !w->dist.allreduce && w->n_terms() == 0 &&
+         w->n_edges > 0 && w->cfg.use_photo;
+}
+
+int window_linearize_solve(SageWindow *w, double damp)
+{
+  if (!w || !window_early_solve_ready(w))
+    return SAGE_E_STATE;
+  const SageWindowConfig &c = w->cfg;
+  EarlySolvePlan &ep = w->early;
+  const int H = (int)c.pyr.cam[0].h, W = (int)c.pyr.cam[0].w, set = 0;
+  int rc = window_sync_candidate(w);
+  if (rc && rc != SAGE_E_NOT_PSD)
+    return rc;
+  w->have_lin = false;
+  const bool merge = w->merge_ok;
+  const bool have_depth = w->dpt_set == set;
+  SAGE_HIP(launch_depth_batch(w->stream, c.CS, w->depth_items[set].as<DepthItem>(), w->n_depth, H, W, !have_depth,
+                              !(have_depth && w->dgrad_valid)));
+  w->dpt_set = set;
+  w->dgrad_valid = true;
+  LaunchCommon lcg = window_lc(w, kGeo), lcp = window_lc(w, kPhoto, true);
+  lcg.stage = 1;
+  lcp.stage = 1;
+  lcg.merge_geo_weight = lcp.merge_geo_weight = merge ? c.geo_weight : 0.f;
+  if (c.use_geo)
+  {
+    prof_attach(w, 1, lcg);
+    SAGE_HIP(launch_geo_linearize(w->stream, c.CS, nullptr, w->dense[kGeo].tab[set].as<GeoEdge>(), lcg, c.pyr.cam[0], c.eps,
+                                  c.geo_loss_param, c.geo_weight, w->dense[kGeo].out()));
+  }
+  auto enqueue_part = [&](int part) -> int {
+    LaunchCommon lc = lcp;
+    lc.ev_start = lc.ev_stop = nullptr;
+    lc.work = ep.work.as<WorkItem>() + (part ? ep.n_work[0] : 0);
+    lc.n_work = ep.n_work[part];
+    prof_attach(w, 0, lc, part == 1);
+    SAGE_HIP(launch_photo_linearize(w->stream, c.CS, c.FS, nullptr, w->dense[kPhoto].tab[set].as<PhotoEdge>(), lc, c.pyr,
+                                    c.photo_weights, c.eps, w->dense[kPhoto].out()));
+    ep.photo_launches += 1;
+    int r;
+    if ((r = window_launch_finalize(w, set, lcp, lcg, merge, ep.edges.as<int32_t>() + (part ? ep.n_edges[0] : 0),
+                                    ep.n_edges[part])))
+      return r;
+    return window_launch_assemble(w, nullptr, ep.blocks.as<int32_t>() + (part ? ep.n_blocks[0] : 0), ep.n_blocks[part]);
+  };
+  if ((rc = enqueue_part(0)))
+    return rc;
+  rc = solver_run_split(w->solver, w->stream, ep.side, ep.ev_early, ep.ev_side, w->packed.as<double>(),
+                        w->vars[0].as<float>(), w->vars[1].as<float>(), c.CS, damp, window_solve_priors(w), ep.early_rows,
+                        [&]() -> int {
+                          const int r = enqueue_part(1);
+                          if (r)
+                            return r;
+                          window_phase_mark(w, 1);
+                          w->have_lin = true;
+                          w->lin_epoch = w->vars_epoch;
+                          w->spec_err_valid = false;
+                          w->dist.packed_reduced = false;
+                          window_phase_mark(w, 2);
+                          return SAGE_OK;
+                        });
+  ep.fused_evals += 1;
+  if (rc)
+    return rc;
+  window_phase_mark(w, 3);
+  w->cand_pending = true;
   return SAGE_OK;
 }
 
diff --git a/sage_slam_amd/csrc/window_lm.hip b/sage_slam_amd/csrc/window_lm.hip
--- a/sage_slam_amd/csrc/window_lm.hip
+++ b/sage_slam_amd/csrc/window_lm.hip
@@ -29,11 +29,18 @@
   return window_mirror_totals(w, false, dst);
 }
 
-static int lm_prepare(LmSeq seq, SageWindow *w, SageLmState *st)
+static int lm_prepare(LmSeq seq, SageWindow *w, SageLmState *st, bool *solved, int *solve_rc)
 {
   int rc;
   const bool sharded = w->dist.allreduce != nullptr;
   const size_t np = sage_window_packed_count(w);
+  *solved = false;
+  if (seq == LmSeq::classic && !sharded && window_early_solve_ready(w))
+  {
+    *solve_rc = window_linearize_solve(w, st->damp);
+    *solved = *solve_rc == SAGE_OK || *solve_rc == SAGE_E_NOT_PSD;
+    return *solved ? SAGE_OK : *solve_rc;
+  }
   if (seq != LmSeq::at_candidate)
   {
     if ((rc = window_linearize_set(w, 0, nullptr, false, true)) ||
@@ -136,11 +143,11 @@
   return SAGE_OK;
 }
 
-static int lm_evaluate(LmSeq seq, SageWindow *w, SageLmState *st, bool first, LmEval &ev)
+static int lm_evaluate(LmSeq seq, SageWindow *w, SageLmState *st, bool first, LmEval &ev, bool solved, int solve_rc)
 {
   if (seq == LmSeq::schur)
     return evaluate_schur(w, st, first);
-  const int rc = sage_window_solve(w, st->damp, nullptr);
+  const int rc = solved ? solve_rc : sage_window_solve(w, st->damp, nullptr);
   if (rc == SAGE_E_NOT_PSD)
   {
     st->candidate_error = INFINITY;
@@ -180,14 +187,16 @@
   if (st->iters == 0 && st->damp <= 0)
     st->damp = cfg->init_damp;
   window_phase_mark(w, 0);
-  int rc = lm_prepare(seq, w, st);
+  bool solved = false;
+  int solve_rc = SAGE_OK;
+  int rc = lm_prepare(seq, w, st, &solved, &solve_rc);
   if (rc)
     return rc;
   st->accepted = 0;
   for (int evals = 1;; ++evals)
   {
     LmEval ev{};
-    if ((rc = lm_evaluate(seq, w, st, evals == 1, ev)))
+    if ((rc = lm_evaluate(seq, w, st, evals == 1, ev, solved && evals == 1, solve_rc)))
       return rc;
     if (st->candidate_error < st->error)
     {
diff --git a/sage_slam_amd/csrc/window_plan.h b/sage_slam_amd/csrc/window_plan.h
--- a/sage_slam_amd/csrc/window_plan.h
+++ b/sage_slam_amd/csrc/window_plan.h
@@ -1,6 +1,7 @@
 #pragma once
 
 #include <algorithm>
+#include <utility>
 #include <vector>
 
 namespace sage
@@ -83,6 +84,106 @@
   return s;
 }
 
+inline int row_blocks(int i, const int *row_first, const int *a_cnt) { return a_cnt[i] + i - row_first[i] + 1; }
+
+inline std::vector<int> scatter_order(int K, int n1, int n2, const int *row_first, const int *row_off, const int *a_cnt,
+                                      const int *a_off)
+{
+  std::vector<int> order;
+  auto push_row = [&](int i) {
+    for (int q = 0; q < a_cnt[i]; ++q)
+      order.push_back(a_off[i] + q);
+    for (int q = 0; q <= i - row_first[i]; ++q)
+      order.push_back(row_off[i] + q);
+  };
+  if (n1 > 0)
+  {
+    for (int t = 0; t < std::max(n1, n2); ++t)
+    {
+      if (t < n1)
+        push_row(t);
+      if (t < n2)
+        push_row(n1 + t);
+    }
+    for (int i = n1 + n2; i < K; ++i)
+      push_row(i);
+  }
+  else
+    for (int i = 0; i < K; ++i)
+      push_row(i);
+  return order;
+}
+
+inline int scatter_order_prefix(int rows, int n1, const int *row_first, const int *a_cnt)
+{
+  int n = 0;
+  for (int t = 0; t < rows; ++t)
+    n += row_blocks(t, row_first, a_cnt) + row_blocks(n1 + t, row_first, a_cnt);
+  return n;
+}
+
+constexpr int kMinEarlyRows = 8;
+
+struct SolveSplit
+{
+  int early_rows = 0;
+  int zone_lo = 0, zone_hi = 0;
+  std::vector<char> late_edge;
+  std::vector<char> late_link;
+  std::vector<char> late_kf;
+  bool split() const { return early_rows > 0; }
+};
+
+inline SolveSplit solve_split(int K, const std::vector<std::pair<int, int>> &links, const int *perm, int n1, int n2,
+                              const std::vector<int> &runs, long long slots, int rounds = 1)
+{
+  SolveSplit none, s;
+  const int w = K - n1 - n2, nl = (int)links.size();
+  if (n1 < 1 || n2 < 1 || w < 1 || slots < 1 || rounds < 1 || (int)runs.size() != 2 * nl)
+    return none;
+  for (int i = 0; i < K; ++i)
+    if (perm[i] != (i < n1 ? i : (i < n1 + n2 ? K - 1 - (i - n1) : n1 + (i - n1 - n2))))
+      return none;
+  auto late_items = [&](int g) {
+    const int lo = n1 - g, hi = n1 + w + g;
+    long long late = 0;
+    for (int l = 0; l < nl; ++l)
+      if ((links[l].first >= lo && links[l].first < hi) || (links[l].second >= lo && links[l].second < hi))
+        late += runs[2 * l] + runs[2 * l + 1];
+    return late;
+  };
+  if (late_items(0) > slots * rounds)
+    return none;
+  int g = 0;
+  while (g + 1 <= std::min(n1, n2) && late_items(g + 1) <= slots * rounds)
+    ++g;
+  long long total = 0;
+  for (int r : runs)
+    total += r;
+  if ((total - late_items(g) + slots - 1) / slots + rounds > (total + slots - 1) / slots)
+    return none;
+  s.zone_lo = n1 - g;
+  s.zone_hi = n1 + w + g;
+  s.late_edge.assign((size_t)2 * nl, 0);
+  s.late_link.assign(nl, 0);
+  s.late_kf.assign(K, 0);
+  for (int k = s.zone_lo; k < s.zone_hi; ++k)
+    s.late_kf[k] = 1;
+  for (int l = 0; l < nl; ++l)
+  {
+    const int a = links[l].first, b = links[l].second;
+    if ((a >= s.zone_lo && a < s.zone_hi) || (b >= s.zone_lo && b < s.zone_hi))
+      s.late_link[l] = s.late_edge[2 * l] = s.late_edge[2 * l + 1] = s.late_kf[a] = s.late_kf[b] = 1;
+  }
+  int r = 0;
+  while (r < std::min(n1, n2) && !s.late_kf[perm[r]] && !s.late_kf[perm[n1 + r]])
+    ++r;
+  if (r < kMinEarlyRows)
+    return none;
+  s.early_rows = r;
+  return s;
+}
+
 inline long long total_tiles(const std::vector<int> &tiles)
 {
   long long total = 0;
diff --git a/sage_slam_amd/csrc/window_profile.hip b/sage_slam_amd/csrc/window_profile.hip
--- a/sage_slam_amd/csrc/window_profile.hip
+++ b/sage_slam_amd/csrc/window_profile.hip
@@ -13,6 +13,11 @@
       (void)hipEventDestroy(pr.first);
       (void)hipEventDestroy(pr.second);
     }
+  for (auto &pr : pending_more)
+  {
+    (void)hipEventDestroy(pr.first);
+    (void)hipEventDestroy(pr.second);
+  }
   for (hipEvent_t e : ev_free)
     (void)hipEventDestroy(e);
 }
@@ -33,7 +38,7 @@
     pf.ev_free.push_back(e);
 }
 
-void prof_attach(SageWindow *w, int which, LaunchCommon &lc)
+void prof_attach(SageWindow *w, int which, LaunchCommon &lc, bool more)
 {
   WindowProfiler &pf = w->prof;
   if (!pf.profiling || (pf.prof_level == 2 && which != 0))
@@ -48,7 +53,7 @@
   }
   lc.ev_start = a;
   lc.ev_stop = b;
-  pf.pending[which].emplace_back(a, b);
+  (more && which == 0 ? pf.pending_more : pf.pending[which]).emplace_back(a, b);
 }
 
 void window_phase_mark(SageWindow *w, int which)
@@ -160,6 +165,18 @@
     ev_put(pf, pr.second);
   }
   pf.pending[which].clear();
+  if (which == 0)
+  {
+    for (auto &pr : pf.pending_more)
+    {
+      float ms = 0.f;
+      if (hipEventElapsedTime(&ms, pr.first, pr.second) == hipSuccess)
+        pf.prof_ms[0] += ms;
+      ev_put(pf, pr.first);
+      ev_put(pf, pr.second);
+    }
+    pf.pending_more.clear();
+  }
   if (total_ms)
     *total_ms = pf.prof_ms[which];
   if (launches)
diff --git a/sage_slam_amd/csrc/window_solve.hip b/sage_slam_amd/csrc/window_solve.hip
--- a/sage_slam_amd/csrc/window_solve.hip
+++ b/sage_slam_amd/csrc/window_solve.hip
@@ -35,7 +35,7 @@
   return e;
 }
 
-static sage::SolvePriors window_solve_priors(const SageWindow *w)
+sage::SolvePriors window_solve_priors(const SageWindow *w)
 {
   const SageWindowConfig &c = w->cfg;
   sage::SolvePriors pri{};
diff --git a/sage_slam_amd/csrc/window_state.h b/sage_slam_amd/csrc/window_state.h
--- a/sage_slam_amd/csrc/window_state.h
+++ b/sage_slam_amd/csrc/window_state.h
@@ -58,6 +58,34 @@
 {
   DevBuf first, count;
   int flush = 0, n = 0;
+};
+
+struct EarlySolvePlan
+{
+  bool on = false;
+  int early_rows = 0;
+  int zone_lo = 0, zone_hi = 0;
+  DevBuf work;
+  int n_work[2] = {0, 0};
+  DevBuf edges;
+  int n_edges[2] = {0, 0};
+  DevBuf blocks;
+  int n_blocks[2] = {0, 0};
+  hipStream_t side = nullptr;
+  hipEvent_t ev_early = nullptr, ev_side = nullptr;
+  long long fused_evals = 0, photo_launches = 0;
+  EarlySolvePlan() = default;
+  EarlySolvePlan(const EarlySolvePlan &) = delete;
+  EarlySolvePlan &operator=(const EarlySolvePlan &) = delete;
+  ~EarlySolvePlan()
+  {
+    if (ev_early)
+      (void)hipEventDestroy(ev_early);
+    if (ev_side)
+      (void)hipEventDestroy(ev_side);
+    if (side)
+      (void)hipStreamDestroy(side);
+  }
 };
 
 struct TotalsMirror
@@ -127,6 +155,7 @@
   bool profiling = false;
   int prof_level = 0;
   std::vector<std::pair<hipEvent_t, hipEvent_t>> pending[6];
+  std::vector<std::pair<hipEvent_t, hipEvent_t>> pending_more;
   std::vector<hipEvent_t> ev_free;
   double prof_ms[6] = {0, 0, 0, 0, 0, 0};
   int prof_n[6] = {0, 0, 0, 0, 0, 0};
```

New measurement: 267,700 Mresiduals/s (median of 6 runs). 2.2% higher.
